# gdonninelli/Navier-Stokes_equations

Hardware: NVIDIA B200
Metric: time-steps/s (higher is better)
Workload: dtype f64 (fp16 operator copy inside the velocity preconditioner)

## Files before the change

navier-stokes_equations_b200/csrc/nsb200.cu:

```cuda
#include "../../include/nsb200.h"

#include <cuda_runtime.h>
#include <dlfcn.h>
#include <nccl.h>

#include <algorithm>
#include <cmath>
#include <cstdlib>
#include <cstring>
#include <map>
#include <memory>
#include <string>
#include <vector>

#include "amg.hpp"
#include "small_eig.hpp"
#include "assemble.cuh"
#include "device.cuh"
#include "linalg.cuh"
#include "structure.hpp"
#include "twolevel.cuh"
#include "velstream.cuh"

using namespace nsb;

namespace {

struct CudaErr {
  std::string msg;
};
#define CK(call)                                                                                   \
  do {                                                                                             \
    cudaError_t e_ = (call);                                                                       \
    if (e_ != cudaSuccess)                                                                         \
      throw CudaErr{std::string(#call) + " failed: " + cudaGetErrorString(e_) + " (" __FILE__ ":" + \
                    std::to_string(__LINE__) + ")"};                                               \
  } while (0)
#define CKN(call)                                                                        \
  do {                                                                                   \
    ncclResult_t r_ = (call);                                                            \
    if (r_ != ncclSuccess)                                                               \
      throw CudaErr{std::string(#call) + " failed: " + g_nccl.GetErrorString(r_)};       \
  } while (0)

struct NcclApi {
  void* handle = nullptr;
  ncclResult_t (*GetUniqueId)(ncclUniqueId*) = nullptr;
  ncclResult_t (*CommInitRank)(ncclComm_t*, int, ncclUniqueId, int) = nullptr;
  ncclResult_t (*CommDestroy)(ncclComm_t) = nullptr;
  ncclResult_t (*AllReduce)(const void*, void*, size_t, ncclDataType_t, ncclRedOp_t, ncclComm_t, cudaStream_t) = nullptr;
  ncclResult_t (*AllGather)(const void*, void*, size_t, ncclDataType_t, ncclComm_t, cudaStream_t) = nullptr;
  ncclResult_t (*Send)(const void*, size_t, ncclDataType_t, int, ncclComm_t, cudaStream_t) = nullptr;
  ncclResult_t (*Recv)(void*, size_t, ncclDataType_t, int, ncclComm_t, cudaStream_t) = nullptr;
  ncclResult_t (*GroupStart)() = nullptr;
  ncclResult_t (*GroupEnd)() = nullptr;
  const char* (*GetErrorString)(ncclResult_t) = nullptr;
  bool load(std::string& err) {
    if (handle) return true;
    for (const char* name : {"libnccl.so.2", "libnccl.so"}) {
      handle = dlopen(name, RTLD_NOW | RTLD_GLOBAL);
      if (handle) break;
    }
    if (!handle) { err = std::string("cannot load NCCL: ") + dlerror(); return false; }
    auto sym = [&](const char* n) { void* p = dlsym(handle, n); if (!p) err = std::string("NCCL symbol missing: ") + n; return p; };
    GetUniqueId = (decltype(GetUniqueId))sym("ncclGetUniqueId");
    CommInitRank = (decltype(CommInitRank))sym("ncclCommInitRank");
    CommDestroy = (decltype(CommDestroy))sym("ncclCommDestroy");
    AllReduce = (decltype(AllReduce))sym("ncclAllReduce");
    AllGather = (decltype(AllGather))sym("ncclAllGather");
    Send = (decltype(Send))sym("ncclSend");
    Recv = (decltype(Recv))sym("ncclRecv");
    GroupStart = (decltype(GroupStart))sym("ncclGroupStart");
    GroupEnd = (decltype(GroupEnd))sym("ncclGroupEnd");
    GetErrorString = (decltype(GetErrorString))sym("ncclGetErrorString");
    return GetUniqueId && CommInitRank && CommDestroy && AllReduce && AllGather && Send && Recv && GroupStart && GroupEnd && GetErrorString;
  }
};
NcclApi g_nccl;

template <typename T> struct DBuf {
  T* p = nullptr;
  size_t n = 0;
  bool owned = true;
  DBuf() = default;
  DBuf(const DBuf&) = delete;
  DBuf& operator=(const DBuf&) = delete;
  ~DBuf() { if (p && owned) cudaFree(p); }
  void alloc(size_t count) {
    if (p && owned) cudaFree(p);
    p = nullptr; owned = true;
    n = count;
    if (count) CK(cudaMalloc(&p, count * sizeof(T)));
  }
  void view(T* ptr, size_t count) {
    if (p && owned) cudaFree(p);
    p = ptr; n = count; owned = false;
  }
  void zero(cudaStream_t s) { if (n) CK(cudaMemsetAsync(p, 0, n * sizeof(T), s)); }
  void upload(const std::vector<T>& v, cudaStream_t s) {
    alloc(v.size());
    if (n) CK(cudaMemcpyAsync(p, v.data(), n * sizeof(T), cudaMemcpyHostToDevice, s));
  }
};

enum ProfCat { PC_ASM_CTX = 0, PC_ASM_ROWS, PC_SPMV, PC_SPMV_VEL, PC_SCHUR, PC_AMG, PC_ORTH, PC_OTHER, PC_ASM_PACK, PC_COARSE, PC_ASM_COARSE, PC_N };
const char* kProfNames[PC_N] = {"asm_context", "asm_rows", "spmv", "spmv_vel", "schur", "amg", "orth", "other", "asm_pack", "coarse", "asm_coarse"};

struct Prof {
  bool on = false;
  std::vector<cudaEvent_t> pool;
  size_t used = 0;
  struct Rec { int cat; size_t e0, e1; };
  std::vector<Rec> recs;
  double ms[PC_N] = {0};
  int64_t cnt[PC_N] = {0};
  cudaEvent_t get() {
    if (used == pool.size()) { cudaEvent_t e; cudaEventCreate(&e); pool.push_back(e); }
    return pool[used++];
  }
  size_t begin(int cat, cudaStream_t s) {
    if (!on) return 0;
    Rec r{cat, used, 0};
    cudaEventRecord(get(), s);
    recs.push_back(r);
    return recs.size() - 1;
  }
  void end(size_t id, cudaStream_t s) {
    if (!on) return;
    recs[id].e1 = used;
    cudaEventRecord(get(), s);
  }
  void collect(cudaStream_t s) {
    if (recs.empty()) return;
    cudaStreamSynchronize(s);
    for (auto& r : recs) {
      float t = 0;
      cudaEventElapsedTime(&t, pool[r.e0], pool[r.e1]);
      ms[r.cat] += t;
      cnt[r.cat]++;
    }
    recs.clear();
    used = 0;
  }
  void reset() { for (int i = 0; i < PC_N; ++i) { ms[i] = 0; cnt[i] = 0; } recs.clear(); used = 0; }
  ~Prof() { for (auto e : pool) cudaEventDestroy(e); }
};

struct DevLevel {
  DevCsr A, P, R;
  DBuf<int> Aptr, Acol, Pptr, Pcol, Rptr, Rcol;
  DBuf<double> Aval, Pval, Rval, dinv;
  DBuf<double> x, x2, b, d, r;
  double lmax = 1.0;
  int n = 0;
};

struct HaloBuf {
  DBuf<double> u, p;
  DBuf<int> uoff, poff;
};

void upload_csr(const HostCsr& H, DBuf<int>& ptr, DBuf<int>& col, DBuf<double>& val, DevCsr& D, cudaStream_t s) {
  ptr.upload(H.ptr, s); col.upload(H.col, s); val.upload(H.val, s);
  D.n = H.n; D.m = H.m; D.ptr = ptr.p; D.col = col.p; D.val = val.p;
}

struct PeerHalo {
  bool on = false;
  DBuf<double> arena;
  size_t stride_f = 0, stride_c = 0, coarse_base = 0;
  int slots_f = 0, slots_c = 0;
  DBuf<unsigned long long> flags;
  DBuf<unsigned int> counter;
  std::vector<void*> opened;
  std::vector<double*> peer_arena;
  std::vector<unsigned long long*> peer_flags;
  DBuf<double*> d_peer_arena;
  DBuf<unsigned long long*> d_peer_flags;
  DBuf<int> d_peer_rank;
  DBuf<int> seg_ptr_f, src_f, seg_ptr_c, src_c;
  DBuf<long long> land_f, land_c;
  unsigned long long seq = 0;
  const double* last_vec = nullptr;
  int total_f_vel = 0, total_f_all = 0, total_c = 0;
  DBuf<int> send_ptr_f, send_ptr_c, list_f, list_c;
  DBuf<int2> send_dst_f, send_dst_c;
  int n_int_f = 0, n_int_c = 0;
  const double* fresh_vec = nullptr;
  unsigned long long fresh_seq = 0;
};

struct VsDev {
  const VsTile* tiles;
  const uint32_t* meta;
  const int* uniq_xoff;
  const unsigned char* vals;
  int n_tiles;
};

struct PolyLevel {
  bool coarse = false;
  int nn = 0;
  long long n = 0, n_tot = 0;
  const double* dinv = nullptr;
  const int64_t* gid = nullptr;
  double *z0 = nullptr, *z1 = nullptr, *zd = nullptr, *poly = nullptr, *pin = nullptr;
  DBuf<double> probe;
  bool probe_init = false;
  std::vector<double> wr, wi;
  double ritz_lo = 0, ritz_hi = 0, ritz_im = 0, ritz_top = 0, probe_res = 1.0;
  std::vector<std::pair<double, double>> roots;
};

struct Coarse {
  DBuf<VsTile> tiles;
  DBuf<uint32_t> meta;
  DBuf<int> uniq_xoff;
  DBuf<unsigned char> vals;
  int n_tiles = 0;
  int64_t total_nq = 0;
  DBuf<long long> nbr_ptr, vedge_ptr;
  DBuf<int> nbr_vxoff, vedge_xoff, ends_xoff, send_xoff;
  DBuf<double> cvals, dinv, rc, z0, z1, zd, poly, pin, send_buf;
  std::vector<int> h_tiles_int, h_tiles_bnd, h_tile_node_ptr;
  std::vector<int64_t> gid, h_nbr_ptr, h_nbr_gid;
  bool built = false, valid = false;
};

}

struct nsb_ctx {
  int dim = 0, device = 0;
  int rank = 0, nranks = 1;
  ncclComm_t comm = nullptr;
  cudaStream_t stream = nullptr;
  std::string err;
  bool have_mesh = false, have_matrix = false, have_pressure = false;
  int64_t launches = 0;
  Prof prof;
  cudaEvent_t t0 = nullptr, t1 = nullptr;

  int64_t n_vertices = 0, n_cells = 0, n_u = 0, n_p = 0;
  std::vector<double> coords;
  std::vector<uint32_t> cell_vertices;
  std::vector<int> g_cell_pid;
  Structure S;
  DevMesh M{};
  DBuf<int> d_cell_xoff, d_cell_poff, d_nbr_xoff, d_pnbr_xoff, d_selfrank, d_node_pid, d_pid_node, d_pselfrank, d_tile_ptr;
  DBuf<double> d_cell_geom;
  DBuf<uint16_t> d_rank_uu, d_rank_up;
  DBuf<long long> d_nbr_ptr, d_pnbr_ptr, d_rowbase, d_prowbase, d_n2c_ptr;
  DBuf<uint32_t> d_n2c;
  DBuf<NodeDesc> d_nd;
  DBuf<FeTables> d_fe;
  int num_sms = 148;
  int n_tiles = 0, tile_smem_bytes = 0;
  DBuf<int> d_stile_ptr, d_suniq_ptr, d_suniq_xoff, d_spuniq_ptr, d_spuniq_xoff;
  DBuf<unsigned short> d_nbr_loc, d_pnbr_loc;
  SpmvTiles stiles{};
  int n_stiles = 0;
  std::vector<int> g2x;
  DBuf<int> d_pid_gid;
  DBuf<int> d_own_gdof;
  DBuf<double> w_tg, w_gather;
  DBuf<double> v_old, v_oldold, v_cur, v_sol, v_rhs;
  DBuf<unsigned char> cflag;
  DBuf<double> cval;
  DBuf<int> c_idx;
  DBuf<double> c_val;
  int n_con = 0;
  nsb_params par{};
  nsb_solver_opts opt{};
  DBuf<double> vals, dinv, ctx, cell_rhs;
  DBuf<double> forcing[2];
  bool forcing_set[2] = {false, false};
  DBuf<unsigned char> vs_vals;
  DBuf<VsTile> d_vs_tiles;
  DBuf<uint32_t> d_vs_meta;
  int64_t vs_total_nq = 0;
  bool vs_valid = false;
  int ctx_stride = 0;
  HostCsr h_Mp, h_Kp;
  DevCsr Mp{};
  DBuf<int> Mp_ptr, Mp_col;
  DBuf<double> Mp_val, Mp_dinv;
  double Mp_lmax = 1.0;
  std::vector<std::unique_ptr<DevLevel>> amg;
  std::vector<std::unique_ptr<HaloBuf>> halo;
  int n_tiles_int = 0, n_tiles_bnd = 0;
  std::vector<int> h_tiles_int, h_tiles_bnd, h_tile_node_ptr;
  bool fused_halo = false;
  double* pin = nullptr;
  DBuf<double> coarse_inv;
  int coarse_n = 0;
  DBuf<double> w_z0, w_z1, w_d, w_t, w_y1, w_m0, w_m1, w_md, w_in, w_tmp, w_pin, w_poly, w_y0, w_u;
  Coarse cg;
  PeerHalo ph;
  PolyLevel lvF, lvC;
  bool two_level = false;
  bool cycle_disabled = false;
  DBuf<double> V;
  int V_cap = 0;
  DBuf<double> partial, d_h, d_nrm;
  int solves = 0;

  void launch_check() {
    ++launches;
#ifdef NSB_DEBUG_SYNC
    CK(cudaStreamSynchronize(stream));
#endif
    CK(cudaGetLastError());
  }
};

namespace {

int fail(nsb_ctx* c, const std::string& m, int code = -1) {
  if (c) c->err = m;
  return code;
}

#define NSB_TRY try {
#define NSB_CATCH(c)                                               \
  }                                                                \
  catch (const CudaErr& e) { return fail(c, e.msg); }              \
  catch (const std::exception& e) { return fail(c, e.what()); }

inline int nblk(long long n, int t) { return (int)((n + t - 1) / t); }

#ifndef NSB_DEFAULT_PRECOND_PRECISION
#define NSB_DEFAULT_PRECOND_PRECISION 16
#endif

size_t vs_vals_bytes(const nsb_ctx* c) {
  if (c->opt.precond_precision == 64) return 0;
  return (size_t)c->vs_total_nq * 4 * c->dim * c->dim * (c->opt.precond_precision == 16 ? 2 : 4);
}

void peer_wait(nsb_ctx* c) {
  PeerHalo& H = c->ph;
  const int np = (int)c->S.peer.size();
  if (np == 0) return;
  k_halo_wait<<<1, 32, 0, c->stream>>>(np, H.d_peer_rank.p, H.flags.p, H.seq);
  c->launch_check();
}

void peer_exchange(nsb_ctx* c, const double* v, int nseg, const DBuf<int>& seg_ptr, const DBuf<int>& src, const DBuf<long long>& land,
                   int total_entries, bool wait = true) {
  PeerHalo& H = c->ph;
  const int np = (int)c->S.peer.size();
  if (np == 0) return;
  const long long vec_off = v - H.arena.p;
  if (vec_off < 0 || (size_t)vec_off >= H.arena.n) throw CudaErr{"halo exchange of a vector outside the symmetric arena"};
  if (v == H.last_vec) {
    k_halo_ack<<<1, 32, 0, c->stream>>>(np, H.d_peer_flags.p, c->nranks, c->rank, H.seq);
    c->launch_check();
    k_halo_wait<<<1, 32, 0, c->stream>>>(np, H.d_peer_rank.p, H.flags.p + c->nranks, H.seq);
    c->launch_check();
  }
  H.last_vec = v;
  H.fresh_vec = nullptr;
  ++H.seq;
  const int grid = std::max(1, std::min(nblk(total_entries, 256), 64));
  k_halo_push<<<grid, 256, 0, c->stream>>>(nseg, np, seg_ptr.p, src.p, land.p, H.d_peer_arena.p, vec_off, v, H.d_peer_flags.p, c->rank,
                                            H.seq, H.counter.p);
  c->launch_check();
  if (wait) peer_wait(c);
}

void halo_exchange(nsb_ctx* c, double* v, bool with_pressure = true) {
  if (c->nranks == 1) return;
  const Structure& S = c->S;
  if (c->ph.on) {
    const int np = (int)S.peer.size();
    const int nseg = with_pressure ? 2 * np : np;
    peer_exchange(c, v, nseg, c->ph.seg_ptr_f, c->ph.src_f, c->ph.land_f, with_pressure ? c->ph.total_f_all : c->ph.total_f_vel);
    return;
  }
  auto& B = c->halo;
  if (B.empty()) {
    auto b = std::make_unique<HaloBuf>();
    std::vector<int> uo, po;
    for (size_t k = 0; k < S.peer.size(); ++k) {
      for (int n : S.send_nodes[k]) uo.push_back((int)S.node_xoff(n));
      for (int q : S.send_pids[k]) po.push_back((int)S.pid_xoff(q));
    }
    b->uoff.upload(uo, c->stream); b->poff.upload(po, c->stream);
    CK(cudaStreamSynchronize(c->stream));
    b->u.alloc(uo.size() * S.dim); b->p.alloc(po.size());
    B.push_back(std::move(b));
  }
  HaloBuf& H = *B[0];
  const long long tu = (long long)H.uoff.n, tp = (long long)H.poff.n;
  if (tu) { k_gather_nodes<<<nblk(tu * S.dim, 256), 256, 0, c->stream>>>((int)tu, S.dim, H.uoff.p, v, H.u.p); c->launch_check(); }
  if (with_pressure && tp) { k_gather<<<nblk(tp, 256), 256, 0, c->stream>>>((int)tp, H.poff.p, v, H.p.p); c->launch_check(); }
  CKN(g_nccl.GroupStart());
  long long uoff = S.n_own_dofs(), poff = S.n_own_dofs() + (long long)S.dim * S.nn_ghost;
  size_t su = 0, sp = 0;
  for (size_t k = 0; k < S.peer.size(); ++k) {
    const int peer = S.peer[k];
    const size_t nu = S.send_nodes[k].size() * S.dim, np = S.send_pids[k].size();
    if (nu) CKN(g_nccl.Send(H.u.p + su, nu, ncclDouble, peer, c->comm, c->stream));
    if (with_pressure && np) CKN(g_nccl.Send(H.p.p + sp, np, ncclDouble, peer, c->comm, c->stream));
    const size_t ru = (size_t)S.recv_node_count[k] * S.dim, rp = (size_t)S.recv_pid_count[k];
    if (ru) CKN(g_nccl.Recv(v + uoff, ru, ncclDouble, peer, c->comm, c->stream));
    if (with_pressure && rp) CKN(g_nccl.Recv(v + poff, rp, ncclDouble, peer, c->comm, c->stream));
    uoff += ru; poff += rp;
    su += nu; sp += np;
  }
  CKN(g_nccl.GroupEnd());
}

void allreduce_sum(nsb_ctx* c, double* dbuf, int n) {
  if (c->nranks == 1) return;
  CKN(g_nccl.AllReduce(dbuf, dbuf, n, ncclDouble, ncclSum, c->comm, c->stream));
}

template <int DIM> void launch_coarse_assemble(nsb_ctx* c);

template <int DIM> void launch_assemble(nsb_ctx* c, bool newton) {
  AsmParams P;
  P.dt = c->par.dt; P.inv_dt = 1.0 / c->par.dt; P.theta = c->par.theta; P.nu = c->par.nu; P.rho = c->par.rho;
  P.use_supg = c->par.use_supg;
  P.gamma = c->par.use_supg ? c->par.gamma : 0.0;
  P.first_order_ustar = c->par.first_order_ustar;
  const int stride = newton ? Ctx<DIM>::N_NEWTON : CtxL<DIM>::N;
  if ((int)c->ctx_stride < stride) {
    c->ctx.alloc((size_t)c->S.nc * stride);
    c->ctx_stride = stride;
  }
  const double* vecA = newton ? c->v_cur.p : c->v_old.p;
  const double* vecB = newton ? c->v_old.p : c->v_oldold.p;
  size_t id = c->prof.begin(PC_ASM_CTX, c->stream);
  const int cgrid = std::min(nblk(c->S.nc, ASM_WARPS), c->num_sms * 8);
  const double *fn = c->forcing[NSB_FORCING_NEW].p, *fo = c->forcing[NSB_FORCING_OLD].p;
  const bool forced = fn != nullptr;
  if (newton && forced)
    k_cell_context<DIM, true, true><<<cgrid, ASM_WARPS * 32, 0, c->stream>>>(c->M, P, c->d_fe.p, vecA, vecB, c->ctx.p, c->cell_rhs.p, fn, fo);
  else if (newton)
    k_cell_context<DIM, true, false><<<cgrid, ASM_WARPS * 32, 0, c->stream>>>(c->M, P, c->d_fe.p, vecA, vecB, c->ctx.p, c->cell_rhs.p, nullptr, nullptr);
  else if (forced)
    k_cell_context<DIM, false, true><<<cgrid, ASM_WARPS * 32, 0, c->stream>>>(c->M, P, c->d_fe.p, vecA, vecB, c->ctx.p, c->cell_rhs.p, fn, fo);
  else
    k_cell_context<DIM, false, false><<<cgrid, ASM_WARPS * 32, 0, c->stream>>>(c->M, P, c->d_fe.p, vecA, vecB, c->ctx.p, c->cell_rhs.p, nullptr, nullptr);
  c->launch_check();
  c->prof.end(id, c->stream);
  RowOut out{c->vals.p, c->v_rhs.p, c->dinv.p};
  id = c->prof.begin(PC_ASM_ROWS, c->stream);
  if (newton)
    k_node_rows<DIM, true><<<c->n_tiles, ASM_WARPS * 32, c->tile_smem_bytes, c->stream>>>(c->M, P, c->ctx.p, c->cell_rhs.p, c->cflag.p, c->cval.p, out, c->d_tile_ptr.p, c->d_fe.p);
  else
    k_node_rows<DIM, false><<<c->n_tiles, ASM_WARPS * 32, c->tile_smem_bytes, c->stream>>>(c->M, P, c->ctx.p, c->cell_rhs.p, c->cflag.p, c->cval.p, out, c->d_tile_ptr.p, c->d_fe.p);
  c->launch_check();
  c->prof.end(id, c->stream);
  c->vs_valid = false;
  if (c->vs_vals.p) {
    id = c->prof.begin(PC_ASM_PACK, c->stream);
    if (c->opt.precond_precision == 16)
      k_vel_pack<DIM, __half><<<c->n_stiles, 256, 0, c->stream>>>(c->M, c->d_vs_tiles.p, c->d_vs_meta.p, c->vals.p, c->dinv.p, reinterpret_cast<__half*>(c->vs_vals.p));
    else
      k_vel_pack<DIM, float><<<c->n_stiles, 256, 0, c->stream>>>(c->M, c->d_vs_tiles.p, c->d_vs_meta.p, c->vals.p, c->dinv.p, reinterpret_cast<float*>(c->vs_vals.p));
    c->launch_check();
    c->prof.end(id, c->stream);
    c->vs_valid = true;
  }
  c->cg.valid = false;
  if (!newton && c->vs_valid && c->cg.built && c->opt.velocity_cycle != 1) launch_coarse_assemble<DIM>(c);
}

template <int DIM> void set_smem_attr(int bytes) {
  CK(cudaFuncSetAttribute(k_node_rows<DIM, false>, cudaFuncAttributeMaxDynamicSharedMemorySize, bytes));
  CK(cudaFuncSetAttribute(k_node_rows<DIM, true>, cudaFuncAttributeMaxDynamicSharedMemorySize, bytes));
}

template <int DIM, typename VT> void set_vs_attr() {
  const int bytes = VsLayout<DIM, VT>::SMEM_BYTES;
  CK(cudaFuncSetAttribute(k_vel_stream<DIM, VT, 2, false>, cudaFuncAttributeMaxDynamicSharedMemorySize, bytes));
  CK(cudaFuncSetAttribute(k_vel_stream<DIM, VT, 3, false>, cudaFuncAttributeMaxDynamicSharedMemorySize, bytes));
  CK(cudaFuncSetAttribute(k_vel_stream<DIM, VT, 3, true>, cudaFuncAttributeMaxDynamicSharedMemorySize, bytes));
  CK(cudaFuncSetAttribute(k_vel_stream<DIM, VT, 4, false>, cudaFuncAttributeMaxDynamicSharedMemorySize, bytes));
  CK(cudaFuncSetAttribute(k_vel_stream<DIM, VT, 4, true>, cudaFuncAttributeMaxDynamicSharedMemorySize, bytes));
}

template <int DIM, typename VT, int MODE, bool HALO>
void launch_vel_stream(nsb_ctx* c, const VsDev& D, int ntiles, const int* list, const double* x, double* y, const double* u, double* poly,
                       PolyCoef pc, const VsHalo& hx) {
  if (ntiles <= 0) return;
  const int grid = std::min(ntiles, c->num_sms);
  k_vel_stream<DIM, VT, MODE, HALO><<<grid, VS_THREADS, VsLayout<DIM, VT>::SMEM_BYTES, c->stream>>>(
      D.tiles, ntiles, list, reinterpret_cast<const VT*>(D.vals), D.meta, D.uniq_xoff, x, y, u, poly, pc, hx);
  c->launch_check();
}
template <int MODE, bool HALO>
void vel_stream(nsb_ctx* c, const VsDev& D, int ntiles, const int* list, const double* x, double* y, const double* u, double* poly, PolyCoef pc,
                const VsHalo& hx = VsHalo{}) {
  const bool h = c->opt.precond_precision == 16;
  if (c->dim == 2) {
    if (h) launch_vel_stream<2, __half, MODE, HALO>(c, D, ntiles, list, x, y, u, poly, pc, hx);
    else launch_vel_stream<2, float, MODE, HALO>(c, D, ntiles, list, x, y, u, poly, pc, hx);
  } else {
    if (h) launch_vel_stream<3, __half, MODE, HALO>(c, D, ntiles, list, x, y, u, poly, pc, hx);
    else launch_vel_stream<3, float, MODE, HALO>(c, D, ntiles, list, x, y, u, poly, pc, hx);
  }
}
VsDev fine_dev(const nsb_ctx* c);

void spmv_full(nsb_ctx* c, const double* x, double* y) {
  size_t id = c->prof.begin(PC_SPMV, c->stream);
  if (c->dim == 2) k_spmv_full<2, double><<<c->n_stiles, SPMV_WARPS * 32, 0, c->stream>>>(c->M, c->stiles, c->vals.p, x, y);
  else k_spmv_full<3, double><<<c->n_stiles, SPMV_WARPS * 32, 0, c->stream>>>(c->M, c->stiles, c->vals.p, x, y);
  c->launch_check();
  c->prof.end(id, c->stream);
}

template <int MODE>
void spmv_vel(nsb_ctx* c, const double* x, double* y, const double* u, double* poly, PolyCoef pc) {
  size_t id = c->prof.begin(PC_SPMV_VEL, c->stream);
  const int g = c->n_stiles;
  if (c->vs_valid && MODE != 0) {
    vel_stream<MODE == 0 ? 2 : MODE, false>(c, fine_dev(c), g, nullptr, x, y, u, poly, pc);
  } else {
    if (c->dim == 2) k_spmv_vel<2, MODE, double><<<g, SPMV_WARPS * 32, 0, c->stream>>>(c->M, c->stiles, c->vals.p, x, y, u, poly, c->dinv.p, pc);
    else k_spmv_vel<3, MODE, double><<<g, SPMV_WARPS * 32, 0, c->stream>>>(c->M, c->stiles, c->vals.p, x, y, u, poly, c->dinv.p, pc);
    c->launch_check();
  }
  c->prof.end(id, c->stream);
}

template <int MODE>
void fused_apply(nsb_ctx* c, bool coarse, const VsDev& D, double* x, double* y, const double* u, double* poly, PolyCoef pc) {
  PeerHalo& H = c->ph;
  const int np = (int)c->S.peer.size();
  VsHalo hx{};
  hx.flags = H.flags.p; hx.peer_rank = H.d_peer_rank.p; hx.npeers = np;
  hx.n_int = coarse ? H.n_int_c : H.n_int_f;
  hx.ghost_start = coarse ? c->dim * c->S.np_own : (int)c->S.n_own_dofs();
  if (x == H.fresh_vec) hx.wait_seq = H.fresh_seq;
  else {
    if (coarse) peer_exchange(c, x, np, H.seg_ptr_c, H.src_c, H.land_c, H.total_c);
    else peer_exchange(c, x, np, H.seg_ptr_f, H.src_f, H.land_f, H.total_f_vel);
    hx.wait_seq = 0;
  }
  hx.send_ptr = coarse ? H.send_ptr_c.p : H.send_ptr_f.p;
  hx.send_dst = coarse ? H.send_dst_c.p : H.send_dst_f.p;
  hx.peer_arena = H.d_peer_arena.p;
  hx.y_off = y - H.arena.p;
  if (hx.y_off < 0 || (size_t)hx.y_off >= H.arena.n) throw CudaErr{"fused halo delivery into a vector outside the symmetric arena"};
  hx.peer_flags = H.d_peer_flags.p; hx.my_rank = c->rank;
  hx.push_seq = ++H.seq;
  hx.counter = H.counter.p;
  const int* list = coarse ? H.list_c.p : H.list_f.p;
  vel_stream<MODE, true>(c, D, D.n_tiles, list, x, y, u, poly, pc, hx);
  H.fresh_vec = y; H.fresh_seq = hx.push_seq;
  H.last_vec = nullptr;
}

void halo_spmv_vel3(nsb_ctx* c, double* x, double* y, const double* u, double* poly, PolyCoef pc) {
  if (c->nranks > 1 && c->ph.on && c->vs_valid && c->fused_halo) {
    size_t id = c->prof.begin(PC_SPMV_VEL, c->stream);
    fused_apply<3>(c, false, fine_dev(c), x, y, u, poly, pc);
    c->prof.end(id, c->stream);
    return;
  }
  halo_exchange(c, x, false);
  spmv_vel<3>(c, x, y, u, poly, pc);
}

void block_scale(nsb_ctx* c, const double* x, double* y) {
  if (c->dim == 2) k_block_scale<2><<<nblk(c->S.nn_own, 256), 256, 0, c->stream>>>(c->S.nn_own, c->dinv.p, x, y);
  else k_block_scale<3><<<nblk(c->S.nn_own, 256), 256, 0, c->stream>>>(c->S.nn_own, c->dinv.p, x, y);
  c->launch_check();
}

double device_norm2(nsb_ctx* c, const double* x, long long n) {
  const int nb = nblk(n, RED_CHUNK);
  k_norm2_partial<<<nb, RED_THREADS, 0, c->stream>>>(x, n, c->partial.p);
  c->launch_check();
  k_reduce_partials<<<1, RED_THREADS, 0, c->stream>>>(nb, c->partial.p, c->d_nrm.p, 0);
  c->launch_check();
  allreduce_sum(c, c->d_nrm.p, 1);
  double v = 0;
  CK(cudaMemcpyAsync(&v, c->d_nrm.p, sizeof(double), cudaMemcpyDeviceToHost, c->stream));
  CK(cudaStreamSynchronize(c->stream));
  return std::sqrt(v);
}

struct Cheb {
  double theta, delta, sigma, rho;
  Cheb(double lmax, double lmin) : theta(0.5 * (lmax + lmin)), delta(0.5 * (lmax - lmin)) {
    sigma = theta / delta;
    rho = 1.0 / sigma;
  }
  void next(double& c1, double& c2) {
    const double rho_new = 1.0 / (2.0 * sigma - rho);
    c1 = rho_new * rho;
    c2 = 2.0 * rho_new / delta;
    rho = rho_new;
  }
};


VsDev fine_dev(const nsb_ctx* c) {
  return VsDev{c->d_vs_tiles.p, c->d_vs_meta.p, c->d_suniq_xoff.p, c->vs_vals.p, c->n_stiles};
}
VsDev coarse_dev(const nsb_ctx* c) {
  return VsDev{c->cg.tiles.p, c->cg.meta.p, c->cg.uniq_xoff.p, c->cg.vals.p, c->cg.n_tiles};
}

void halo_exchange_coarse(nsb_ctx* c, double* v) {
  if (c->nranks == 1) return;
  const Structure& S = c->S;
  if (c->ph.on) {
    peer_exchange(c, v, (int)S.peer.size(), c->ph.seg_ptr_c, c->ph.src_c, c->ph.land_c, c->ph.total_c);
    return;
  }
  Coarse& G = c->cg;
  const int dim = c->dim;
  const long long tp = (long long)G.send_xoff.n;
  if (tp) { k_gather_nodes<<<nblk(tp * dim, 256), 256, 0, c->stream>>>((int)tp, dim, G.send_xoff.p, v, G.send_buf.p); c->launch_check(); }
  CKN(g_nccl.GroupStart());
  long long roff = (long long)dim * S.np_own;
  size_t so = 0;
  for (size_t k = 0; k < S.peer.size(); ++k) {
    const int peer = S.peer[k];
    const size_t ns = S.send_pids[k].size() * dim, nr = (size_t)S.recv_pid_count[k] * dim;
    if (ns) CKN(g_nccl.Send(G.send_buf.p + so, ns, ncclDouble, peer, c->comm, c->stream));
    if (nr) CKN(g_nccl.Recv(v + roff, nr, ncclDouble, peer, c->comm, c->stream));
    so += ns; roff += nr;
  }
  CKN(g_nccl.GroupEnd());
}

void level_halo(nsb_ctx* c, PolyLevel& lv, double* v) {
  if (lv.coarse) halo_exchange_coarse(c, v);
  else halo_exchange(c, v, false);
}

template <int MODE>
void level_apply(nsb_ctx* c, PolyLevel& lv, const double* x, double* y, const double* u, double* poly, PolyCoef pc) {
  if (!lv.coarse) { spmv_vel<MODE>(c, x, y, u, poly, pc); return; }
  size_t id = c->prof.begin(PC_COARSE, c->stream);
  vel_stream<MODE, false>(c, coarse_dev(c), c->cg.n_tiles, nullptr, x, y, u, poly, pc);
  c->prof.end(id, c->stream);
}

void level_root(nsb_ctx* c, PolyLevel& lv, double* x, double* y, const double* u, double* poly, PolyCoef pc) {
  if (!lv.coarse) { halo_spmv_vel3(c, x, y, u, poly, pc); return; }
  if (c->nranks > 1 && c->ph.on && c->fused_halo) {
    size_t id = c->prof.begin(PC_COARSE, c->stream);
    fused_apply<3>(c, true, coarse_dev(c), x, y, u, poly, pc);
    c->prof.end(id, c->stream);
    return;
  }
  halo_exchange_coarse(c, x);
  level_apply<3>(c, lv, x, y, u, poly, pc);
}

void level_block_scale(nsb_ctx* c, PolyLevel& lv, const double* x, double* y) {
  if (c->dim == 2) k_block_scale<2><<<nblk(lv.nn, 256), 256, 0, c->stream>>>(lv.nn, lv.dinv, x, y);
  else k_block_scale<3><<<nblk(lv.nn, 256), 256, 0, c->stream>>>(lv.nn, lv.dinv, x, y);
  c->launch_check();
}

void level_arnoldi(nsb_ctx* c, PolyLevel& lv, int dmax, double target) {
  const long long nl = lv.n;
  const long long ld = c->S.n_own_dofs();
  int d = std::max(1, std::min(dmax, 64));
  if (c->V_cap < d + 1) { c->V.alloc((size_t)(std::max(d + 1, c->V_cap)) * ld); c->V_cap = std::max(d + 1, c->V_cap); }
  const int nb = nblk(nl, RED_CHUNK);
  if (c->partial.n < (size_t)nb * (d + 2)) c->partial.alloc((size_t)nb * (d + 2));
  if (c->d_h.n < (size_t)2 * (d + 2)) c->d_h.alloc(2 * (d + 2));
  if (!lv.probe_init) {
    std::vector<double> h(nl);
    for (int A = 0; A < lv.nn; ++A)
      for (int k = 0; k < c->dim; ++k) {
        uint64_t z = (uint64_t)(lv.gid[A] * c->dim + k) + 0x9E3779B97F4A7C15ull;
        z = (z ^ (z >> 30)) * 0xBF58476D1CE4E5B9ull;
        z = (z ^ (z >> 27)) * 0x94D049BB133111EBull;
        z ^= z >> 31;
        h[(size_t)c->dim * A + k] = (double)(z >> 11) / 9007199254740992.0 - 0.5;
      }
    lv.probe.upload(h, c->stream);
    CK(cudaStreamSynchronize(c->stream));
    lv.probe_init = true;
  }
  const int ldh = d;
  std::vector<double> H((size_t)(d + 1) * d, 0.0), hh(2 * (d + 2)), gcs(d + 1), gsn(d + 1);
  double gres = 1.0;
  double beta = device_norm2(c, lv.probe.p, nl);
  k_axpby<<<nblk(nl, 256), 256, 0, c->stream>>>(nl, 1.0 / beta, lv.probe.p, 0.0, c->V.p);
  c->launch_check();
  int dd = d;
  for (int k = 0; k < d; ++k) {
    double* vk = c->V.p + (size_t)k * ld;
    double* w = c->V.p + (size_t)(k + 1) * ld;
    const double* xin = vk;
    if (c->nranks > 1) {
      double* buf = (k & 1) ? lv.z1 : lv.pin;
      CK(cudaMemcpyAsync(buf, vk, nl * sizeof(double), cudaMemcpyDeviceToDevice, c->stream));
      level_halo(c, lv, buf);
      xin = buf;
    }
    level_apply<2>(c, lv, xin, w, nullptr, nullptr, PolyCoef{});
    for (int pass = 0; pass < 2; ++pass) {
      k_multi_dot<<<nb, RED_THREADS, 0, c->stream>>>(k + 1, c->V.p, ld, w, nl, c->partial.p);
      c->launch_check();
      double* hp = c->d_h.p + pass * (d + 2);
      k_reduce_partials<<<k + 1, RED_THREADS, 0, c->stream>>>(nb, c->partial.p, hp, 0);
      c->launch_check();
      allreduce_sum(c, hp, k + 1);
      k_multi_axpy<<<nb, RED_THREADS, 0, c->stream>>>(k + 1, c->V.p, ld, hp, -1.0, w, nl, pass == 1 ? c->partial.p : nullptr);
      c->launch_check();
    }
    k_reduce_partials<<<1, RED_THREADS, 0, c->stream>>>(nb, c->partial.p, c->d_nrm.p, 0);
    c->launch_check();
    allreduce_sum(c, c->d_nrm.p, 1);
    k_scale_by_inv_norm<<<nblk(nl, 256), 256, 0, c->stream>>>(nl, w, c->d_nrm.p, w);
    c->launch_check();
    double nrm2 = 0;
    CK(cudaMemcpyAsync(hh.data(), c->d_h.p, sizeof(double) * 2 * (d + 2), cudaMemcpyDeviceToHost, c->stream));
    CK(cudaMemcpyAsync(&nrm2, c->d_nrm.p, sizeof(double), cudaMemcpyDeviceToHost, c->stream));
    CK(cudaStreamSynchronize(c->stream));
    for (int i = 0; i <= k; ++i) H[(size_t)i * ldh + k] = hh[i] + hh[(d + 2) + i];
    H[(size_t)(k + 1) * ldh + k] = std::sqrt(nrm2);
    if (!(nrm2 > 1e-28)) { dd = k + 1; break; }
    {
      std::vector<double> col(k + 2);
      for (int i = 0; i <= k + 1; ++i) col[i] = H[(size_t)i * ldh + k];
      for (int i = 0; i < k; ++i) {
        const double t = gcs[i] * col[i] + gsn[i] * col[i + 1];
        col[i + 1] = -gsn[i] * col[i] + gcs[i] * col[i + 1];
        col[i] = t;
      }
      const double r = std::hypot(col[k], col[k + 1]);
      gcs[k] = col[k] / r; gsn[k] = col[k + 1] / r;
      gres *= std::fabs(gsn[k]);
      if (target > 0 && gres <= target && k + 1 >= 2) { dd = k + 1; break; }
    }
  }
  lv.probe_res = gres;
  d = dd;
  std::vector<double> Hd((size_t)d * d), At((size_t)d * d), f(d, 0.0);
  for (int i = 0; i < d; ++i)
    for (int j = 0; j < d; ++j) { Hd[(size_t)i * d + j] = H[(size_t)i * ldh + j]; At[(size_t)j * d + i] = H[(size_t)i * ldh + j]; }
  f[d - 1] = 1.0;
  {
    for (int col = 0; col < d; ++col) {
      int p = col;
      for (int r = col + 1; r < d; ++r) if (std::fabs(At[(size_t)r * d + col]) > std::fabs(At[(size_t)p * d + col])) p = r;
      if (p != col) { for (int k = 0; k < d; ++k) std::swap(At[(size_t)col * d + k], At[(size_t)p * d + k]); std::swap(f[col], f[p]); }
      const double dg = At[(size_t)col * d + col];
      for (int r = col + 1; r < d; ++r) {
        const double m = At[(size_t)r * d + col] / dg;
        if (m == 0.0) continue;
        for (int k = col; k < d; ++k) At[(size_t)r * d + k] -= m * At[(size_t)col * d + k];
        f[r] -= m * f[col];
      }
    }
    for (int r = d - 1; r >= 0; --r) {
      double sum = f[r];
      for (int k = r + 1; k < d; ++k) sum -= At[(size_t)r * d + k] * f[k];
      f[r] = sum / At[(size_t)r * d + r];
    }
  }
  const double hl = H[(size_t)d * ldh + (d - 1)];
  for (int i = 0; i < d; ++i) Hd[(size_t)i * d + (d - 1)] += hl * hl * f[i];
  std::vector<double> H0((size_t)d * d), sr, si;
  for (int i = 0; i < d; ++i)
    for (int j = 0; j < d; ++j) H0[(size_t)i * d + j] = H[(size_t)i * ldh + j];
  if (!hessenberg_eigs(d, Hd, lv.wr, lv.wi)) throw CudaErr{"harmonic Ritz eigenvalue iteration did not converge"};
  if (!hessenberg_eigs(d, H0, sr, si)) throw CudaErr{"Ritz eigenvalue iteration did not converge"};
  lv.ritz_lo = 1e300; lv.ritz_hi = -1e300; lv.ritz_im = 0; lv.ritz_top = -1e300;
  for (int i = 0; i < d; ++i) {
    lv.ritz_lo = std::min(lv.ritz_lo, lv.wr[i]); lv.ritz_hi = std::max(lv.ritz_hi, lv.wr[i]);
    lv.ritz_im = std::max(lv.ritz_im, std::fabs(lv.wi[i]));
    lv.ritz_top = std::max(lv.ritz_top, std::hypot(sr[i], si[i]));
  }
  lv.ritz_top = std::max(lv.ritz_top, lv.ritz_hi);
}

bool level_spectrum_is_real(const PolyLevel& lv, double tol = 0.05) { return lv.ritz_lo > 0 && lv.ritz_im < tol * lv.ritz_hi; }

void set_roots(PolyLevel& lv, std::vector<double> wr, std::vector<double> wi) {
  const int d = (int)wr.size();
  std::vector<std::pair<double, double>> th, out;
  for (int i = 0; i < d; ++i) if (wi[i] >= 0) th.emplace_back(wr[i], wi[i]);
  auto mag = [](const std::pair<double, double>& z) { return std::hypot(z.first, z.second); };
  while (!th.empty()) {
    size_t best = 0;
    double bv = -1e300;
    for (size_t i = 0; i < th.size(); ++i) {
      double v;
      if (out.empty()) v = mag(th[i]);
      else {
        v = 0;
        for (auto& o : out) {
          v += std::log(std::hypot(th[i].first - o.first, th[i].second - o.second) + 1e-300);
          if (o.second != 0) v += std::log(std::hypot(th[i].first - o.first, th[i].second + o.second) + 1e-300);
        }
      }
      if (v > bv) { bv = v; best = i; }
    }
    out.push_back(th[best]);
    th.erase(th.begin() + best);
  }
  lv.roots = out;
}
void set_chebyshev_roots(PolyLevel& lv, int d, double lo, double hi) {
  std::vector<double> wr(d), wi(d, 0.0);
  for (int j = 1; j <= d; ++j) wr[j - 1] = 0.5 * (hi + lo) + 0.5 * (hi - lo) * std::cos(M_PI * (2 * j - 1) / (2.0 * d));
  set_roots(lv, wr, wi);
}

void apply_poly(nsb_ctx* c, PolyLevel& lv) {
  double* prod = lv.z0;
  double* other = lv.z1;
  double* tmp = lv.zd;
  double* poly = lv.poly;
  CK(cudaMemsetAsync(poly, 0, lv.n * sizeof(double), c->stream));
  const auto& R = lv.roots;
  for (size_t k = 0; k < R.size(); ++k) {
    const bool last = (k + 1 == R.size());
    const double a = R[k].first, b = R[k].second;
    if (b == 0.0) {
      if (last) {
        k_axpby<<<nblk(lv.n, 256), 256, 0, c->stream>>>(lv.n, 1.0 / a, prod, 1.0, poly);
        c->launch_check();
      } else {
        level_root(c, lv, prod, other, prod, poly, PolyCoef{1.0, -1.0 / a, 1.0 / a, 0.0});
        std::swap(prod, other);
      }
    } else {
      const double m2 = a * a + b * b;
      level_root(c, lv, prod, tmp, prod, poly, PolyCoef{2.0 * a, -1.0, 0.0, 1.0 / m2});
      if (!last) {
        level_root(c, lv, tmp, other, prod, poly, PolyCoef{1.0, -1.0 / m2, 0.0, 0.0});
        std::swap(prod, other);
      }
    }
  }
}

template <int DIM> void launch_coarse_assemble(nsb_ctx* c) {
  Coarse& G = c->cg;
  FeTables T;
  fill_tables(DIM, T);
  double wsum = 0;
  for (int q = 0; q < T.nq; ++q) wsum += T.w[q];
  const double gamma = c->par.use_supg ? c->par.gamma : 0.0;
  size_t id = c->prof.begin(PC_ASM_COARSE, c->stream);
  k_coarse_rows<DIM><<<nblk(c->S.np_own, CG_WARPS), CG_WARPS * 32, 0, c->stream>>>(c->M, c->ctx.p, gamma, wsum, G.nbr_ptr.p, G.nbr_vxoff.p,
                                                                                     c->cflag.p, G.cvals.p, G.dinv.p);
  c->launch_check();
  if (c->opt.precond_precision == 16)
    k_coarse_pack<DIM, __half><<<G.n_tiles, 256, 0, c->stream>>>(G.tiles.p, G.meta.p, G.nbr_ptr.p, G.cvals.p, G.dinv.p, reinterpret_cast<__half*>(G.vals.p));
  else
    k_coarse_pack<DIM, float><<<G.n_tiles, 256, 0, c->stream>>>(G.tiles.p, G.meta.p, G.nbr_ptr.p, G.cvals.p, G.dinv.p, reinterpret_cast<float*>(G.vals.p));
  c->launch_check();
  c->prof.end(id, c->stream);
  G.valid = true;
}

void setup_velocity_pc(nsb_ctx* c) {
  PolyLevel& F = c->lvF;
  bool two = c->opt.velocity_cycle != 1 && c->cg.valid && c->vs_valid && !c->cycle_disabled;
  if (two) {
    level_arnoldi(c, F, 24, 0.0);
    two = level_spectrum_is_real(F, 0.02);
  }
  c->two_level = two;
  if (!two) {
    level_arnoldi(c, F, c->opt.poly_degree_F, c->opt.poly_target);
    if (c->opt.poly_kind == 1 && level_spectrum_is_real(F)) set_chebyshev_roots(F, (int)F.wr.size(), 0.9 * F.ritz_lo, 1.05 * F.ritz_hi);
    else set_roots(F, F.wr, F.wi);
    return;
  }
  const double hi = c->opt.smoother_hi_factor * F.ritz_top;
  set_chebyshev_roots(F, std::max(1, c->opt.smoother_degree), c->opt.smoother_lo_frac * hi, hi);
  PolyLevel& C = c->lvC;
  level_arnoldi(c, C, std::max(4, std::min(64, c->opt.coarse_degree + 5)), 0.05);
  if (level_spectrum_is_real(C)) set_chebyshev_roots(C, std::max(1, c->opt.coarse_degree), 0.9 * C.ritz_lo, c->opt.smoother_hi_factor * C.ritz_top);
  else set_roots(C, C.wr, C.wi);
}

void apply_velocity_pc(nsb_ctx* c, const double* x) {
  PolyLevel& F = c->lvF;
  const long long nu = F.n;
  if (!c->two_level) {
    level_block_scale(c, F, x, F.z0);
    apply_poly(c, F);
    return;
  }
  PolyLevel& C = c->lvC;
  Coarse& G = c->cg;
  const double* xr = x;
  if (c->nranks > 1) {
    CK(cudaMemcpyAsync(c->w_u.p, x, nu * sizeof(double), cudaMemcpyDeviceToDevice, c->stream));
    halo_exchange(c, c->w_u.p, false);
    xr = c->w_u.p;
  }
  size_t id = c->prof.begin(PC_COARSE, c->stream);
  if (c->dim == 2) k_restrict<2><<<nblk(c->S.np_own, 128), 128, 0, c->stream>>>(c->S.np_own, c->M.pid_node, G.vedge_ptr.p, G.vedge_xoff.p, c->cflag.p, xr, G.rc.p);
  else k_restrict<3><<<nblk(c->S.np_own, 128), 128, 0, c->stream>>>(c->S.np_own, c->M.pid_node, G.vedge_ptr.p, G.vedge_xoff.p, c->cflag.p, xr, G.rc.p);
  c->launch_check();
  c->prof.end(id, c->stream);
  level_block_scale(c, C, G.rc.p, C.z0);
  apply_poly(c, C);
  halo_exchange_coarse(c, C.poly);
  double* y0 = c->w_y0.p;
  id = c->prof.begin(PC_COARSE, c->stream);
  if (c->dim == 2) k_prolong<2><<<nblk(nu, 256), 256, 0, c->stream>>>(c->S.nn_own, G.ends_xoff.p, c->cflag.p, C.poly, y0);
  else k_prolong<3><<<nblk(nu, 256), 256, 0, c->stream>>>(c->S.nn_own, G.ends_xoff.p, c->cflag.p, C.poly, y0);
  c->launch_check();
  c->prof.end(id, c->stream);
  level_block_scale(c, F, x, c->w_u.p);
  if (c->nranks > 1 && c->ph.on && c->fused_halo) {
    size_t idf = c->prof.begin(PC_SPMV_VEL, c->stream);
    fused_apply<4>(c, false, fine_dev(c), y0, F.z0, c->w_u.p, nullptr, PolyCoef{1.0, -1.0, 0.0, 0.0});
    c->prof.end(idf, c->stream);
  } else {
    halo_exchange(c, y0, false);
    level_apply<4>(c, F, y0, F.z0, c->w_u.p, nullptr, PolyCoef{1.0, -1.0, 0.0, 0.0});
  }
  apply_poly(c, F);
  k_axpby<<<nblk(nu, 256), 256, 0, c->stream>>>(nu, 1.0, y0, 1.0, F.poly);
  c->launch_check();
}

void csr_cheb(nsb_ctx* c, const DevCsr& A, const double* dinv, double lmax, double ratio, int degree,
              const double* b, double* x, double* x2, double* d, bool zero_guess, double** result) {
  Cheb ch(1.1 * lmax, 1.1 * lmax / ratio);
  double* cur = x;
  double* oth = x2;
  int k0 = 0;
  const int g8 = nblk((long long)A.n * 8, 256);
  if (zero_guess) {
    k_cheb_first<<<nblk(A.n, 256), 256, 0, c->stream>>>(A.n, dinv, b, d, cur, 1.0 / ch.theta);
    c->launch_check();
    k0 = 1;
  }
  for (int k = k0; k < degree; ++k) {
    double c1, c2;
    if (k == 0) { c1 = 0.0; c2 = 1.0 / ch.theta; }
    else ch.next(c1, c2);
    k_csr<3><<<g8, 256, 0, c->stream>>>(A, cur, oth, b, d, dinv, c1, c2);
    c->launch_check();
    std::swap(cur, oth);
  }
  *result = cur;
}

void amg_vcycle(nsb_ctx* c, int lev) {
  DevLevel& L = *c->amg[lev];
  const int deg = c->opt.amg_smoother_degree;
  if (lev + 1 == (int)c->amg.size()) {
    if (c->coarse_n > 0) {
      k_dense_mv<<<nblk((long long)L.n * 32, 256), 256, 0, c->stream>>>(L.n, c->coarse_inv.p, L.b.p, L.x.p);
      c->launch_check();
    } else {
      double* res;
      csr_cheb(c, L.A, L.dinv.p, L.lmax, 30.0, 12, L.b.p, L.x.p, L.x2.p, L.d.p, true, &res);
      if (res != L.x.p) std::swap(L.x.p, L.x2.p);
    }
    return;
  }
  double* res;
  csr_cheb(c, L.A, L.dinv.p, L.lmax, 20.0, deg, L.b.p, L.x.p, L.x2.p, L.d.p, true, &res);
  if (res != L.x.p) std::swap(L.x.p, L.x2.p);
  const int g8 = nblk((long long)L.n * 8, 256);
  k_csr<1><<<g8, 256, 0, c->stream>>>(L.A, L.x.p, L.r.p, L.b.p, nullptr, nullptr, 0, 0);
  c->launch_check();
  DevLevel& N = *c->amg[lev + 1];
  k_csr<0><<<nblk((long long)N.n * 8, 256), 256, 0, c->stream>>>(L.R, L.r.p, N.b.p, nullptr, nullptr, nullptr, 0, 0);
  c->launch_check();
  amg_vcycle(c, lev + 1);
  k_csr<2><<<g8, 256, 0, c->stream>>>(L.P, N.x.p, L.x.p, nullptr, nullptr, nullptr, 0, 0);
  c->launch_check();
  csr_cheb(c, L.A, L.dinv.p, L.lmax, 20.0, deg, L.b.p, L.x.p, L.x2.p, L.d.p, false, &res);
  if (res != L.x.p) std::swap(L.x.p, L.x2.p);
}

double schur_mass_coeff(const nsb_ctx* c) {
  const double cm = c->opt.schur_mass_coeff;
  return cm >= 0 ? cm : c->par.theta * c->par.nu + (c->par.use_supg ? c->par.gamma : 0.0);
}

void precond_apply(nsb_ctx* c, const double* x, double* y) {
  const Structure& S = c->S;
  const int dim = c->dim;
  const long long nu = (long long)dim * S.nn_own;
  apply_velocity_pc(c, x);
  double* z = c->w_poly.p;
  CK(cudaMemcpyAsync(y, z, nu * sizeof(double), cudaMemcpyDeviceToDevice, c->stream));
  halo_exchange(c, z);
  size_t id = c->prof.begin(PC_SCHUR, c->stream);
  if (dim == 2) k_schur_rhs<2, double><<<nblk(S.np_own, SPMV_WARPS), SPMV_WARPS * 32, 0, c->stream>>>(c->M, c->vals.p, z, x, c->w_t.p);
  else k_schur_rhs<3, double><<<nblk(S.np_own, SPMV_WARPS), SPMV_WARPS * 32, 0, c->stream>>>(c->M, c->vals.p, z, x, c->w_t.p);
  c->launch_check();
  c->prof.end(id, c->stream);
  const double* tg = c->w_t.p;
  if (c->nranks > 1) {
    CK(cudaMemsetAsync(c->w_tg.p, 0, (size_t)c->n_p * sizeof(double), c->stream));
    k_scatter_vals<<<nblk(S.np_own, 256), 256, 0, c->stream>>>(S.np_own, c->d_pid_gid.p, c->w_t.p, c->w_tg.p);
    c->launch_check();
    allreduce_sum(c, c->w_tg.p, (int)c->n_p);
    tg = c->w_tg.p;
  }
  id = c->prof.begin(PC_AMG, c->stream);
  DevLevel& L0 = *c->amg[0];
  CK(cudaMemcpyAsync(L0.b.p, tg, (size_t)L0.n * sizeof(double), cudaMemcpyDeviceToDevice, c->stream));
// ... 15 lines not shown
  const int m = std::max(1, n_tmp - 2);
  if (c->V_cap < m + 1) {
    c->V.alloc((size_t)(m + 1) * n);
    c->V_cap = m + 1;
  }
  const int nb = nblk(n, RED_CHUNK);
  if (c->partial.n < (size_t)nb * (m + 2)) c->partial.alloc((size_t)nb * (m + 2));
  if (c->d_h.n < (size_t)2 * (m + 2)) c->d_h.alloc(2 * (m + 2));
  double* x = c->v_sol.p;
  CK(cudaMemsetAsync(x, 0, S.n_tot_dofs() * sizeof(double), c->stream));
  std::vector<double> H((size_t)(m + 1) * m, 0.0), cs(m), sn(m), g(m + 1), hcol(2 * (m + 2));
  int it = 0;
  double res = 0;
  bool first = true;
  for (;;) {
    double* V0 = c->V.p;
    if (first) {
      precond_apply(c, c->v_rhs.p, c->w_in.p);
    } else {
      halo_exchange(c, x);
      spmv_full(c, x, c->w_tmp.p);
      k_lincomb<<<nblk(n, 256), 256, 0, c->stream>>>(n, 1.0, c->v_rhs.p, -1.0, c->w_tmp.p, c->w_tmp.p);
      c->launch_check();
      precond_apply(c, c->w_tmp.p, c->w_in.p);
    }
    const double beta = device_norm2(c, c->w_in.p, n);
    res = beta;
    if (first && beta <= tol_abs) { *iterations = 0; *residual = beta; return 0; }
    first = false;
    if (!(beta > 0)) { *iterations = it; *residual = beta; return 0; }
    k_axpby<<<nblk(n, 256), 256, 0, c->stream>>>(n, 1.0 / beta, c->w_in.p, 0.0, V0);
    c->launch_check();
    std::fill(g.begin(), g.end(), 0.0);
    g[0] = beta;
    int kused = 0;
    bool converged = false;
    for (int k = 0; k < m; ++k) {
      double* vk = c->V.p + (size_t)k * n;
      double* w = c->V.p + (size_t)(k + 1) * n;
      const double* xin = vk;
      if (c->nranks > 1) {
        CK(cudaMemcpyAsync(c->w_pin.p, vk, n * sizeof(double), cudaMemcpyDeviceToDevice, c->stream));
        halo_exchange(c, c->w_pin.p);
        xin = c->w_pin.p;
      }
      spmv_full(c, xin, c->w_tmp.p);
      precond_apply(c, c->w_tmp.p, w);
      size_t id = c->prof.begin(PC_ORTH, c->stream);
      const int mode = c->opt.reorthogonalize;
      int passes = 1;
      double nrm2 = 0, nrm2_before = 0;
      for (int pass = 0; pass < 2; ++pass) {
        const int nv = k + 1 + (pass == 0 ? 1 : 0);
        k_multi_dot<<<nb, RED_THREADS, 0, c->stream>>>(nv, c->V.p, n, w, n, c->partial.p);
        c->launch_check();
        double* hp = c->d_h.p + pass * (m + 2);
        k_reduce_partials<<<nv, RED_THREADS, 0, c->stream>>>(nb, c->partial.p, hp, 0);
        c->launch_check();
        allreduce_sum(c, hp, nv);
        k_multi_axpy<<<nb, RED_THREADS, 0, c->stream>>>(k + 1, c->V.p, n, hp, -1.0, w, n, c->partial.p);
        c->launch_check();
        k_reduce_partials<<<1, RED_THREADS, 0, c->stream>>>(nb, c->partial.p, c->d_nrm.p, 0);
        c->launch_check();
        allreduce_sum(c, c->d_nrm.p, 1);
        passes = pass + 1;
        if (pass == 1 || mode < 0) break;
        if (mode != 2) {
          CK(cudaMemcpyAsync(&nrm2_before, hp + k + 1, sizeof(double), cudaMemcpyDeviceToHost, c->stream));
          CK(cudaMemcpyAsync(&nrm2, c->d_nrm.p, sizeof(double), cudaMemcpyDeviceToHost, c->stream));
          CK(cudaStreamSynchronize(c->stream));
          if (nrm2 > 0.5 * nrm2_before) break;
        }
      }
      k_scale_by_inv_norm<<<nblk(n, 256), 256, 0, c->stream>>>(n, w, c->d_nrm.p, w);
      c->launch_check();
      c->prof.end(id, c->stream);
      CK(cudaMemcpyAsync(hcol.data(), c->d_h.p, sizeof(double) * 2 * (m + 2), cudaMemcpyDeviceToHost, c->stream));
      CK(cudaMemcpyAsync(&nrm2, c->d_nrm.p, sizeof(double), cudaMemcpyDeviceToHost, c->stream));
      CK(cudaStreamSynchronize(c->stream));
      for (int i = 0; i <= k; ++i) H[(size_t)i * m + k] = hcol[i] + (passes == 2 ? hcol[(m + 2) + i] : 0.0);
      H[(size_t)(k + 1) * m + k] = std::sqrt(nrm2);
      for (int i = 0; i < k; ++i) {
        const double t = cs[i] * H[(size_t)i * m + k] + sn[i] * H[(size_t)(i + 1) * m + k];
        H[(size_t)(i + 1) * m + k] = -sn[i] * H[(size_t)i * m + k] + cs[i] * H[(size_t)(i + 1) * m + k];
        H[(size_t)i * m + k] = t;
      }
      const double a = H[(size_t)k * m + k], b = H[(size_t)(k + 1) * m + k];
      const double dd = std::hypot(a, b);
      cs[k] = a / dd; sn[k] = b / dd;
      H[(size_t)k * m + k] = dd;
      H[(size_t)(k + 1) * m + k] = 0.0;
      g[k + 1] = -sn[k] * g[k];
      g[k] = cs[k] * g[k];
      res = std::fabs(g[k + 1]);
      ++it;
      kused = k + 1;
      if (res <= tol_abs) { converged = true; break; }
      if (it >= max_it) break;
      if (!(nrm2 > 0)) break;
    }
    std::vector<double> yv(kused);
    for (int i = kused - 1; i >= 0; --i) {
      double s = g[i];
      for (int j = i + 1; j < kused; ++j) s -= H[(size_t)i * m + j] * yv[j];
      yv[i] = s / H[(size_t)i * m + i];
    }
    CK(cudaMemcpyAsync(c->d_h.p, yv.data(), sizeof(double) * kused, cudaMemcpyHostToDevice, c->stream));
    k_multi_axpy<<<nb, RED_THREADS, 0, c->stream>>>(kused, c->V.p, n, c->d_h.p, 1.0, x, n, nullptr);
    c->launch_check();
    CK(cudaStreamSynchronize(c->stream));
    if (converged || it >= max_it) {
      *iterations = it;
      *residual = res;
      return converged ? 0 : 1;
    }
  }
}

void build_tiles(nsb_ctx* c) {
  const Structure& S = c->S;
  int dev_max = 0;
  CK(cudaDeviceGetAttribute(&dev_max, cudaDevAttrMaxSharedMemoryPerBlockOptin, c->device));
  const int stat = 24 * 1024;
  int budget = std::max(S.max_node_smem_doubles, 5 * 1024);
  if ((long long)budget * 8 + stat > dev_max)
    throw CudaErr{"a node's rows do not fit in shared memory (valence too high)"};
  std::vector<int> tp;
  tp.push_back(0);
  int sum = 0, cnt = 0;
  for (int A = 0; A < S.nn_own; ++A) {
    const int need = (S.dim + (S.node_pid[A] >= 0 ? 1 : 0)) * S.row_len(A);
    if (cnt > 0 && (sum + need > budget || cnt >= 64)) { tp.push_back(A); sum = 0; cnt = 0; }
    sum += need; ++cnt;
  }
  tp.push_back(S.nn_own);
  c->n_tiles = (int)tp.size() - 1;
  c->tile_smem_bytes = budget * 8;
  c->d_tile_ptr.upload(tp, c->stream);
  {
    TilePlan P;
    const TileLimits L{TILE_MAX_NODES, TILE_MAX_IDX, TILE_MAX_UNIQ, TILE_MAX_PUNIQ, VS_MAX_BLOCKS};
    const std::string err = build_tile_plan(S, L, P);
    if (!err.empty()) throw CudaErr{err};
    VsPlan V;
    const std::string err2 = build_vel_stream(S, P, V);
    if (!err2.empty()) throw CudaErr{err2};
    c->n_stiles = P.n_tiles();
    c->d_stile_ptr.upload(P.node_ptr, c->stream);
    c->n_tiles_int = (int)P.tiles_int.size(); c->n_tiles_bnd = (int)P.tiles_bnd.size();
    c->h_tiles_int = P.tiles_int; c->h_tiles_bnd = P.tiles_bnd; c->h_tile_node_ptr = P.node_ptr;
    c->d_suniq_ptr.upload(P.uniq_ptr, c->stream); c->d_suniq_xoff.upload(P.uniq_xoff, c->stream);
    c->d_spuniq_ptr.upload(P.puniq_ptr, c->stream); c->d_spuniq_xoff.upload(P.puniq_xoff, c->stream);
    c->d_nbr_loc.upload(P.nbr_loc, c->stream); c->d_pnbr_loc.upload(P.pnbr_loc, c->stream);
    c->d_vs_tiles.upload(V.tiles, c->stream); c->d_vs_meta.upload(V.meta, c->stream);
    c->vs_total_nq = V.total_nq;
    CK(cudaStreamSynchronize(c->stream));
    c->stiles.node_ptr = c->d_stile_ptr.p;
    c->stiles.uniq_ptr = c->d_suniq_ptr.p; c->stiles.uniq_xoff = c->d_suniq_xoff.p;
    c->stiles.puniq_ptr = c->d_spuniq_ptr.p; c->stiles.puniq_xoff = c->d_spuniq_xoff.p;
    c->stiles.nbr_loc = c->d_nbr_loc.p; c->stiles.pnbr_loc = c->d_pnbr_loc.p;
  }
  c->vs_vals.alloc(vs_vals_bytes(c));
  c->vs_valid = false;
  CK(cudaStreamSynchronize(c->stream));
  if (c->dim == 2) { set_smem_attr<2>(c->tile_smem_bytes); set_vs_attr<2, float>(); set_vs_attr<2, __half>(); }
  else { set_smem_attr<3>(c->tile_smem_bytes); set_vs_attr<3, float>(); set_vs_attr<3, __half>(); }
}

void close_peer_halo(nsb_ctx* c) {
  PeerHalo& H = c->ph;
  for (void* q : H.opened) cudaIpcCloseMemHandle(q);
  H.opened.clear(); H.peer_arena.clear(); H.peer_flags.clear();
  H.on = false;
}

void nccl_barrier(nsb_ctx* c) {
  if (c->nranks == 1 || !c->comm) return;
  CKN(g_nccl.AllReduce(c->d_nrm.p + 2, c->d_nrm.p + 2, 1, ncclDouble, ncclSum, c->comm, c->stream));
  CK(cudaStreamSynchronize(c->stream));
}

void setup_peer_halo(nsb_ctx* c, std::vector<DBuf<double>*> fine, std::vector<DBuf<double>*> coarse, size_t nt, size_t nct) {
  PeerHalo& H = c->ph;
  const Structure& S = c->S;
  const int R = c->nranks, dim = c->dim, np = (int)S.peer.size();
  cudaStream_t st = c->stream;
  close_peer_halo(c);
  nccl_barrier(c);
  long long hs[2] = {(long long)nt, (long long)nct};
  DBuf<long long> ds;
  ds.alloc(2);
  CK(cudaMemcpyAsync(ds.p, hs, sizeof(hs), cudaMemcpyHostToDevice, st));
  CKN(g_nccl.AllReduce(ds.p, ds.p, 2, ncclInt64, ncclMax, c->comm, st));
  CK(cudaMemcpyAsync(hs, ds.p, sizeof(hs), cudaMemcpyDeviceToHost, st));
  CK(cudaStreamSynchronize(st));
  H.stride_f = ((size_t)hs[0] + 31) / 32 * 32;
  H.stride_c = ((size_t)hs[1] + 31) / 32 * 32;
  H.slots_f = (int)fine.size(); H.slots_c = (int)coarse.size();
  H.coarse_base = H.stride_f * H.slots_f;
  H.arena.alloc(H.coarse_base + H.stride_c * H.slots_c);
  H.arena.zero(st);
  for (size_t i = 0; i < fine.size(); ++i) fine[i]->view(H.arena.p + i * H.stride_f, nt);
  for (size_t i = 0; i < coarse.size(); ++i) coarse[i]->view(H.arena.p + H.coarse_base + i * H.stride_c, nct);
  H.flags.alloc(2 * (size_t)R); H.flags.zero(st);
  H.counter.alloc(1); H.counter.zero(st);
  H.seq = 0; H.last_vec = nullptr;
  const char* mode = std::getenv("NSB200_HALO");
  const bool want = !(mode && std::string(mode) == "nccl");
  std::vector<long long> mine((size_t)R * 3, -1), all((size_t)R * R * 3, -1);
  {
    long long uoff = S.n_own_dofs(), poff = S.n_own_dofs() + (long long)dim * S.nn_ghost, coff = (long long)dim * S.np_own;
    for (int k = 0; k < np; ++k) {
      mine[(size_t)S.peer[k] * 3 + 0] = uoff; mine[(size_t)S.peer[k] * 3 + 1] = poff; mine[(size_t)S.peer[k] * 3 + 2] = coff;
      uoff += (long long)S.recv_node_count[k] * dim; poff += S.recv_pid_count[k]; coff += (long long)S.recv_pid_count[k] * dim;
    }
  }
  struct Handles { cudaIpcMemHandle_t arena, flags; };
  Handles hm;
  std::vector<Handles> hall(R);
  bool ok = want;
  if (ok) ok = cudaIpcGetMemHandle(&hm.arena, H.arena.p) == cudaSuccess && cudaIpcGetMemHandle(&hm.flags, H.flags.p) == cudaSuccess;
  if (!ok) { std::memset(&hm, 0, sizeof(hm)); cudaGetLastError(); }
  {
    DBuf<unsigned char> g0, g1;
    DBuf<long long> t0, t1;
    g0.alloc(sizeof(Handles) + 8); g1.alloc((sizeof(Handles) + 8) * R);
    t0.alloc(mine.size()); t1.alloc(all.size());
    unsigned char pack[sizeof(Handles) + 8] = {0};
    std::memcpy(pack, &hm, sizeof(hm));
    pack[sizeof(Handles)] = ok ? 1 : 0;
    CK(cudaMemcpyAsync(g0.p, pack, sizeof(pack), cudaMemcpyHostToDevice, st));
    CK(cudaMemcpyAsync(t0.p, mine.data(), mine.size() * sizeof(long long), cudaMemcpyHostToDevice, st));
    CKN(g_nccl.AllGather(g0.p, g1.p, sizeof(pack), ncclChar, c->comm, st));
    CKN(g_nccl.AllGather(t0.p, t1.p, mine.size(), ncclInt64, c->comm, st));
    std::vector<unsigned char> back((sizeof(Handles) + 8) * R);
    CK(cudaMemcpyAsync(back.data(), g1.p, back.size(), cudaMemcpyDeviceToHost, st));
    CK(cudaMemcpyAsync(all.data(), t1.p, all.size() * sizeof(long long), cudaMemcpyDeviceToHost, st));
    CK(cudaStreamSynchronize(st));
    for (int r = 0; r < R; ++r) {
      std::memcpy(&hall[r], back.data() + (sizeof(Handles) + 8) * r, sizeof(Handles));
      ok = ok && back[(sizeof(Handles) + 8) * r + sizeof(Handles)] == 1;
    }
  }
  if (ok) {
    for (int k = 0; k < np && ok; ++k) {
      void *pa = nullptr, *pf = nullptr;
      ok = cudaIpcOpenMemHandle(&pa, hall[S.peer[k]].arena, cudaIpcMemLazyEnablePeerAccess) == cudaSuccess;
      if (ok) { H.opened.push_back(pa); ok = cudaIpcOpenMemHandle(&pf, hall[S.peer[k]].flags, cudaIpcMemLazyEnablePeerAccess) == cudaSuccess; }
      if (ok) H.opened.push_back(pf);
      H.peer_arena.push_back((double*)pa); H.peer_flags.push_back((unsigned long long*)pf);
    }
    if (!ok) cudaGetLastError();
  }
  {
    DBuf<long long> d;
    d.alloc(1);
    long long v = ok ? 1 : 0;
    CK(cudaMemcpyAsync(d.p, &v, sizeof(v), cudaMemcpyHostToDevice, st));
    CKN(g_nccl.AllReduce(d.p, d.p, 1, ncclInt64, ncclMin, c->comm, st));
    CK(cudaMemcpyAsync(&v, d.p, sizeof(v), cudaMemcpyDeviceToHost, st));
    CK(cudaStreamSynchronize(st));
    ok = v == 1;
  }
  if (!ok) {
    if (want && c->rank == 0) std::fprintf(stderr, "nsb200: peer-store halo unavailable (CUDA IPC), using NCCL send/recv\n");
    close_peer_halo(c);
    return;
  }
  std::vector<int> sp(1, 0), src, spc(1, 0), srcc, pr(np);
  std::vector<long long> land(2 * (size_t)np), landc(np);
  for (int k = 0; k < np; ++k) {
    pr[k] = S.peer[k];
    for (int n : S.send_nodes[k]) for (int cc = 0; cc < dim; ++cc) src.push_back((int)S.node_xoff(n) + cc);
    sp.push_back((int)src.size());
    land[k] = all[((size_t)S.peer[k] * R + c->rank) * 3 + 0];
  }
  H.total_f_vel = (int)src.size();
  for (int k = 0; k < np; ++k) {
    for (int q : S.send_pids[k]) src.push_back((int)S.pid_xoff(q));
    sp.push_back((int)src.size());
    land[np + k] = all[((size_t)S.peer[k] * R + c->rank) * 3 + 1];
    for (int q : S.send_pids[k]) for (int cc = 0; cc < dim; ++cc) srcc.push_back(dim * q + cc);
    spc.push_back((int)srcc.size());
    landc[k] = all[((size_t)S.peer[k] * R + c->rank) * 3 + 2];
  }
  H.total_f_all = (int)src.size(); H.total_c = (int)srcc.size();
  for (int k = 0; k < np; ++k)
    if (land[k] < 0 || land[np + k] < 0 || landc[k] < 0) throw CudaErr{"halo plan mismatch: a peer does not expect data from this rank"};
  H.seg_ptr_f.upload(sp, st); H.src_f.upload(src, st); H.land_f.upload(land, st);
  H.seg_ptr_c.upload(spc, st); H.src_c.upload(srcc, st); H.land_c.upload(landc, st);
  H.d_peer_arena.upload(H.peer_arena, st); H.d_peer_flags.upload(H.peer_flags, st); H.d_peer_rank.upload(pr, st);
  auto fused_tables = [&](int n_own, const std::vector<std::vector<int>>& send, const std::vector<long long>& landing, const std::vector<int>& ,
                          const std::vector<int>& t_bnd, const std::vector<int>& node_ptr, DBuf<int>& d_ptr, DBuf<int2>& d_dst, DBuf<int>& d_list,
                          int& n_int) {
    std::vector<int> cnt(n_own + 1, 0);
    for (int k = 0; k < np; ++k) for (int n : send[k]) cnt[n + 1]++;
    for (int n = 0; n < n_own; ++n) cnt[n + 1] += cnt[n];
    std::vector<int2> dst(cnt[n_own]);
    std::vector<int> fill(cnt.begin(), cnt.end() - 1);
    for (int k = 0; k < np; ++k)
      for (size_t i = 0; i < send[k].size(); ++i) dst[fill[send[k][i]]++] = make_int2(k, (int)(landing[k] + (long long)i * dim));
    std::vector<char> back(node_ptr.size() - 1, 0);
    for (int t : t_bnd) back[t] = 1;
    for (size_t t = 0; t + 1 < node_ptr.size(); ++t)
      for (int n = node_ptr[t]; n < node_ptr[t + 1] && !back[t]; ++n)
        if (cnt[n + 1] != cnt[n]) back[t] = 1;
    std::vector<int> list;
    for (size_t t = 0; t + 1 < node_ptr.size(); ++t) if (!back[t]) list.push_back((int)t);
    n_int = (int)list.size();
    for (size_t t = 0; t + 1 < node_ptr.size(); ++t) if (back[t]) list.push_back((int)t);
    for (auto& d : dst) if (d.y < 0) throw CudaErr{"halo plan: negative landing offset"};
    d_ptr.upload(cnt, st); d_dst.upload(dst, st); d_list.upload(list, st);
    CK(cudaStreamSynchronize(st));
  };
  {
    std::vector<long long> lf(land.begin(), land.begin() + np);
    fused_tables(S.nn_own, S.send_nodes, lf, c->h_tiles_int, c->h_tiles_bnd, c->h_tile_node_ptr, H.send_ptr_f, H.send_dst_f, H.list_f, H.n_int_f);
    fused_tables(S.np_own, S.send_pids, landc, c->cg.h_tiles_int, c->cg.h_tiles_bnd, c->cg.h_tile_node_ptr, H.send_ptr_c, H.send_dst_c, H.list_c, H.n_int_c);
  }
  H.fresh_vec = nullptr; H.fresh_seq = 0;
  CK(cudaStreamSynchronize(st));
  nccl_barrier(c);
  H.on = true;
}

void build_coarse_level(nsb_ctx* c) {
  const Structure& S = c->S;
  Coarse& G = c->cg;
  G.built = false; G.valid = false;
  CoarseLevel CL;
  const std::string e = build_coarse(S, CL);
  if (!e.empty()) throw CudaErr{e};
  const Structure& Sc = CL.Sc;
  for (int P = 0; P < S.np_own; ++P)
    if (Sc.nbr_ptr[P + 1] - Sc.nbr_ptr[P] > CG_MAX_NB) throw CudaErr{"a vertex has more P1 neighbours than the coarse row kernel can accumulate"};
  TilePlan P;
  const TileLimits L{TILE_MAX_NODES, TILE_MAX_IDX, TILE_MAX_UNIQ, TILE_MAX_PUNIQ, VS_MAX_BLOCKS};
  const std::string e1 = build_tile_plan(Sc, L, P);
  if (!e1.empty()) throw CudaErr{e1};
  VsPlan V;
  const std::string e2 = build_vel_stream(Sc, P, V);
  if (!e2.empty()) throw CudaErr{e2};
  cudaStream_t st = c->stream;
  const int dim = c->dim;
  G.n_tiles = P.n_tiles();
  G.total_nq = V.total_nq;
  G.h_tiles_int = P.tiles_int; G.h_tiles_bnd = P.tiles_bnd; G.h_tile_node_ptr = P.node_ptr;
  G.tiles.upload(V.tiles, st); G.meta.upload(V.meta, st); G.uniq_xoff.upload(P.uniq_xoff, st);
  std::vector<long long> t64(Sc.nbr_ptr.begin(), Sc.nbr_ptr.end()), v64(CL.vedge_ptr.begin(), CL.vedge_ptr.end());
  G.nbr_ptr.upload(t64, st); G.vedge_ptr.upload(v64, st);
  std::vector<int> vx(Sc.nbr.size()), ex(CL.vedge.size()), en(CL.node_ends.size()), sx;
  for (size_t i = 0; i < vx.size(); ++i) vx[i] = (int)S.node_xoff(S.pid_node[Sc.nbr[i]]);
  for (size_t i = 0; i < ex.size(); ++i) ex[i] = (int)S.node_xoff(CL.vedge[i]);
  for (size_t i = 0; i < en.size(); ++i) en[i] = (int)Sc.node_xoff(CL.node_ends[i]);
  for (size_t k = 0; k < S.peer.size(); ++k)
    for (int q : S.send_pids[k]) sx.push_back((int)Sc.node_xoff(q));
  G.nbr_vxoff.upload(vx, st); G.vedge_xoff.upload(ex, st); G.ends_xoff.upload(en, st); G.send_xoff.upload(sx, st);
  G.send_buf.alloc(sx.size() * dim);
  G.gid.assign(S.pid_gid.begin(), S.pid_gid.begin() + S.np_own);
  G.h_nbr_ptr.assign(Sc.nbr_ptr.begin(), Sc.nbr_ptr.end());
  G.h_nbr_gid.resize(Sc.nbr.size());
  for (size_t i = 0; i < Sc.nbr.size(); ++i) G.h_nbr_gid[i] = S.pid_gid[Sc.nbr[i]];
  CK(cudaStreamSynchronize(st));
  const size_t nct = (size_t)Sc.n_tot_dofs();
  G.cvals.alloc(Sc.nbr.size() * dim * dim);
  G.dinv.alloc((size_t)S.np_own * dim * dim);
  if (c->nranks == 1) {
    for (DBuf<double>* v : {&G.rc, &G.z0, &G.z1, &G.zd, &G.poly, &G.pin}) { v->alloc(nct); v->zero(st); }
  } else {
    setup_peer_halo(c, {&c->v_old, &c->v_oldold, &c->v_cur, &c->v_sol, &c->v_rhs, &c->cval, &c->w_z0, &c->w_z1, &c->w_d, &c->w_in, &c->w_tmp,
                        &c->w_pin, &c->w_poly, &c->w_y0, &c->w_u},
                    {&G.rc, &G.z0, &G.z1, &G.zd, &G.poly, &G.pin}, (size_t)S.n_tot_dofs(), nct);
  }
  CK(cudaStreamSynchronize(st));
  PolyLevel& C = c->lvC;
  C.coarse = true; C.nn = S.np_own; C.n = (long long)dim * S.np_own; C.n_tot = (long long)nct;
  C.dinv = G.dinv.p; C.gid = G.gid.data();
  C.z0 = G.z0.p; C.z1 = G.z1.p; C.zd = G.zd.p; C.poly = G.poly.p; C.pin = G.pin.p;
  C.probe_init = false; C.roots.clear();
  G.built = true;
}

size_t coarse_vals_bytes(const nsb_ctx* c) {
  if (c->opt.precond_precision == 64) return 0;
  return (size_t)c->cg.total_nq * 4 * c->dim * c->dim * (c->opt.precond_precision == 16 ? 2 : 4);
}

void bind_fine_level(nsb_ctx* c) {
  PolyLevel& F = c->lvF;
  F.coarse = false; F.nn = c->S.nn_own; F.n = (long long)c->dim * c->S.nn_own; F.n_tot = c->S.n_tot_dofs();
  F.dinv = c->dinv.p; F.gid = c->S.node_gid.data();
  F.z0 = c->w_z0.p; F.z1 = c->w_z1.p; F.zd = c->w_d.p; F.poly = c->w_poly.p; F.pin = c->w_pin.p;
}

void host_pressure_matrices(nsb_ctx* c, const std::vector<unsigned char>& pflag) {
  const int dim = c->dim, NV = dim + 1;
  const int64_t np = c->n_p, C = c->n_cells;
  FeTables T;
  fill_tables(dim, T);
  double wsum = 0;
  for (int q = 0; q < T.nq; ++q) wsum += T.w[q];
  std::vector<std::vector<int>> adj(np);
  for (int64_t cc = 0; cc < C; ++cc)
    for (int i = 0; i < NV; ++i)
      for (int j = 0; j < NV; ++j) adj[c->g_cell_pid[cc * NV + i]].push_back(c->g_cell_pid[cc * NV + j]);
  HostCsr Mp, Kp;
  Mp.n = Mp.m = (int)np;
  Mp.ptr.assign(np + 1, 0);
  for (int64_t i = 0; i < np; ++i) {
    auto& a = adj[i];
    std::sort(a.begin(), a.end());
    a.erase(std::unique(a.begin(), a.end()), a.end());
    Mp.ptr[i + 1] = Mp.ptr[i] + (int)a.size();
  }
  Mp.col.resize(Mp.ptr[np]);
  for (int64_t i = 0; i < np; ++i) std::copy(adj[i].begin(), adj[i].end(), Mp.col.begin() + Mp.ptr[i]);
  Mp.val.assign(Mp.col.size(), 0.0);
  Kp = Mp;
  auto find = [&](int r, int col) {
    const int* b = Mp.col.data() + Mp.ptr[r];
    const int* e = Mp.col.data() + Mp.ptr[r + 1];
    return (int)(std::lower_bound(b, e, col) - Mp.col.data());
  };
  for (int64_t cc = 0; cc < C; ++cc) {
    const uint32_t* cv = c->cell_vertices.data() + cc * NV;
    double X[4][3] = {{0}};
    for (int v = 0; v < NV; ++v)
      for (int k = 0; k < dim; ++k) X[v][k] = c->coords[(size_t)cv[v] * dim + k];
    double gl[4][3] = {{0}}, det;
    if (dim == 2) {
      const double a = X[1][0] - X[0][0], b = X[2][0] - X[0][0], cq = X[1][1] - X[0][1], d = X[2][1] - X[0][1];
      det = a * d - b * cq;
      gl[1][0] = d / det; gl[1][1] = -b / det; gl[2][0] = -cq / det; gl[2][1] = a / det;
      for (int k = 0; k < 2; ++k) gl[0][k] = -(gl[1][k] + gl[2][k]);
    } else {
      double J[3][3];
      for (int r = 0; r < 3; ++r)
        for (int k = 0; k < 3; ++k) J[r][k] = X[k + 1][r] - X[0][r];
      const double c00 = J[1][1] * J[2][2] - J[1][2] * J[2][1], c01 = J[1][2] * J[2][0] - J[1][0] * J[2][2],
                   c02 = J[1][0] * J[2][1] - J[1][1] * J[2][0];
      det = J[0][0] * c00 + J[0][1] * c01 + J[0][2] * c02;
      const double id = 1.0 / det;
      gl[1][0] = c00 * id; gl[1][1] = (J[0][2] * J[2][1] - J[0][1] * J[2][2]) * id; gl[1][2] = (J[0][1] * J[1][2] - J[0][2] * J[1][1]) * id;
      gl[2][0] = c01 * id; gl[2][1] = (J[0][0] * J[2][2] - J[0][2] * J[2][0]) * id; gl[2][2] = (J[0][2] * J[1][0] - J[0][0] * J[1][2]) * id;
      gl[3][0] = c02 * id; gl[3][1] = (J[0][1] * J[2][0] - J[0][0] * J[2][1]) * id; gl[3][2] = (J[0][0] * J[1][1] - J[0][1] * J[1][0]) * id;
      for (int k = 0; k < 3; ++k) gl[0][k] = -((gl[1][k] + gl[2][k]) + gl[3][k]);
    }
    const double absJ = std::fabs(det);
    const int* pid = c->g_cell_pid.data() + cc * NV;
    for (int i = 0; i < NV; ++i) {
      const bool ci = pflag[pid[i]] != 0;
      for (int j = 0; j < NV; ++j) {
        const bool cj = pflag[pid[j]] != 0;
        double gg = 0;
        for (int k = 0; k < dim; ++k) gg += gl[i][k] * gl[j][k];
        double m = absJ * T.MPhat[i][j], kk = absJ * wsum * gg;
        if (ci || cj) {
          if (i == j) { m = std::fabs(m); kk = std::fabs(kk); }
          else { m = 0; kk = 0; }
        }
        const int p = find(pid[i], pid[j]);
        Mp.val[p] += m;
        Kp.val[p] += kk;
      }
    }
  }
  for (size_t k = 0; k < Kp.val.size(); ++k) Kp.val[k] += 1e-6 * Mp.val[k];
  c->h_Mp = std::move(Mp);
  c->h_Kp = std::move(Kp);
}

double* vec_ptr(nsb_ctx* c, int which) {
  switch (which) {
    case NSB_SOLUTION_OLD: return c->v_old.p;
    case NSB_SOLUTION_OLD_OLD: return c->v_oldold.p;
    case NSB_CURRENT_SOLUTION: return c->v_cur.p;
    case NSB_SOLUTION: return c->v_sol.p;
    case NSB_RHS: return c->v_rhs.p;
  }
  return nullptr;
}

PolyLevel& level_of(nsb_ctx* c, int level) { return level == 0 ? c->lvF : c->lvC; }

void level_upload(nsb_ctx* c, int level, const double* g, double* d) {
  const Structure& S = c->S;
  const int dim = c->dim;
  const int nn = level == 0 ? S.nn_own + S.nn_ghost : S.np_own;
  std::vector<double> loc(level == 0 ? (size_t)S.n_tot_dofs() : (size_t)dim * nn, 0.0);
  for (int A = 0; A < nn; ++A) {
    const int64_t off = level == 0 ? S.node_xoff(A) : (int64_t)dim * A;
    const int64_t gid = level == 0 ? S.node_gid[A] : S.pid_gid[A];
    for (int k = 0; k < dim; ++k) loc[off + k] = g[gid * dim + k];
  }
  CK(cudaMemcpyAsync(d, loc.data(), loc.size() * sizeof(double), cudaMemcpyHostToDevice, c->stream));
  CK(cudaStreamSynchronize(c->stream));
}

void level_download(nsb_ctx* c, int level, const double* d, double* g) {
  const Structure& S = c->S;
  const int dim = c->dim;
  const int nn = level == 0 ? S.nn_own : S.np_own;
  std::vector<double> out((size_t)dim * nn);
  CK(cudaMemcpyAsync(out.data(), d, out.size() * sizeof(double), cudaMemcpyDeviceToHost, c->stream));
  CK(cudaStreamSynchronize(c->stream));
  for (int A = 0; A < nn; ++A) {
    const int64_t gid = level == 0 ? S.node_gid[A] : S.pid_gid[A];
    for (int k = 0; k < dim; ++k) g[gid * dim + k] = out[(size_t)dim * A + k];
  }
}

void velocity_operator_apply(nsb_ctx* c, int level, int mode, const double* coef, const double* xg, const double* ug, double* yg,
                             double* pg) {
  PolyLevel& lv = level_of(c, level);
  double* x = level == 0 ? c->w_pin.p : c->cg.pin.p;
  double* u = level == 0 ? c->w_u.p : c->cg.z0.p;
  double* y = level == 0 ? c->w_tmp.p : c->cg.z1.p;
  double* p = level == 0 ? c->w_poly.p : c->cg.poly.p;
  level_upload(c, level, xg, x);
  if (mode >= 3) level_upload(c, level, ug, u);
  if (mode == 3) level_upload(c, level, pg, p);
  const PolyCoef pc = coef ? PolyCoef{coef[0], coef[1], coef[2], coef[3]} : PolyCoef{};
  if (mode == 2) level_apply<2>(c, lv, x, y, nullptr, nullptr, pc);
  else if (mode == 3) level_apply<3>(c, lv, x, y, u, p, pc);
  else level_apply<4>(c, lv, x, y, u, nullptr, pc);
  level_download(c, level, y, yg);
  if (mode == 3) level_download(c, level, p, pg);
}

template <typename VT>
void unpack_level(nsb_ctx* c, const VsDev& D, int64_t total_nq, size_t n_uniq, std::vector<int>& node, std::vector<int>& nbr,
                  std::vector<double>& val) {
  const int dim = c->dim, PL = dim * dim;
  std::vector<VsTile> tiles(D.n_tiles);
  std::vector<uint32_t> meta((size_t)total_nq * 4);
  std::vector<int> uniq(n_uniq);
  std::vector<VT> v((size_t)total_nq * 4 * PL);
  CK(cudaMemcpyAsync(tiles.data(), D.tiles, tiles.size() * sizeof(VsTile), cudaMemcpyDeviceToHost, c->stream));
  CK(cudaMemcpyAsync(meta.data(), D.meta, meta.size() * sizeof(uint32_t), cudaMemcpyDeviceToHost, c->stream));
  CK(cudaMemcpyAsync(uniq.data(), D.uniq_xoff, uniq.size() * sizeof(int), cudaMemcpyDeviceToHost, c->stream));
  CK(cudaMemcpyAsync(v.data(), D.vals, v.size() * sizeof(VT), cudaMemcpyDeviceToHost, c->stream));
  CK(cudaStreamSynchronize(c->stream));
  for (const VsTile& T : tiles) {
    const uint32_t* m = meta.data() + (size_t)T.nq_off * 4;
    const VT* tv = v.data() + (size_t)T.nq_off * 4 * PL;
    for (int q = 0; q < T.nquad; ++q) {
      const uint32_t* mq = m + 4 * q;
      if (mq[2] == 0xffffu) continue;
      const int cnt = (int)(mq[3] >> 16);
      for (int e = 0; e < cnt; ++e) {
        const int loc = (int)(((e < 2 ? mq[0] : mq[1]) >> (16 * (e & 1))) & 0xffffu);
        node.push_back(T.n0 + (int)mq[2]);
        nbr.push_back(uniq[T.u0 + loc] / dim);
        for (int rc = 0; rc < PL; ++rc) val.push_back((double)(float)tv[((size_t)rc * T.NQ + q) * 4 + e]);
      }
    }
  }
}

}

extern "C" {

int nsb_create(int dim, int device, nsb_handle* out) {
  if (!out) return -1;
  *out = nullptr;
  if (dim != 2 && dim != 3) return -1;
  nsb_ctx* c = new nsb_ctx();
  c->dim = dim; c->device = device;
  *out = c;
  NSB_TRY
  int ndev = 0;
  CK(cudaGetDeviceCount(&ndev));
  if (device < 0 || device >= ndev) throw CudaErr{"no such CUDA device (the product path has no CPU fallback)"};
  CK(cudaSetDevice(device));
  cudaDeviceProp prop;
  CK(cudaGetDeviceProperties(&prop, device));
  if (prop.major < 10) throw CudaErr{"nsb200 is built for sm_100a (B200) only"};
  CK(cudaStreamCreateWithFlags(&c->stream, cudaStreamNonBlocking));
  CK(cudaEventCreate(&c->t0));
  CK(cudaEventCreate(&c->t1));
  FeTables T2, T3;
  fill_tables(2, T2);
  fill_tables(3, T3);
  {
    std::vector<FeTables> tv(1, dim == 2 ? T2 : T3);
    c->d_fe.upload(tv, c->stream);
    CK(cudaStreamSynchronize(c->stream));
  }
  CK(cudaDeviceGetAttribute(&c->num_sms, cudaDevAttrMultiProcessorCount, device));
  c->opt.poly_degree_F = 64; c->opt.poly_refresh = 1; c->opt.poly_target = 0.08; c->opt.poly_kind = 1; c->opt.cheb_degree_Mp = 3;
  c->opt.amg_smoother_degree = 2; c->opt.schur_mass_coeff = -1.0; c->opt.reorthogonalize = 1;
  c->opt.precond_precision = NSB_DEFAULT_PRECOND_PRECISION;
  c->opt.precond_operator = 1;
  c->opt.velocity_cycle = 2; c->opt.smoother_degree = 14; c->opt.smoother_lo_frac = 0.012; c->opt.coarse_degree = 15; c->opt.smoother_hi_factor = 1.1;
  c->par.dt = 0.01; c->par.theta = 1.0; c->par.nu = 1e-3; c->par.rho = 1.0; c->par.gamma = 0.1;
  c->d_nrm.alloc(4);
  return 0;
  NSB_CATCH(c)
}

int nsb_destroy(nsb_handle c) {
  if (!c) return 0;
  cudaSetDevice(c->device);
  if (c->stream) cudaStreamSynchronize(c->stream);
  if (c->ph.on) {
    try { close_peer_halo(c); nccl_barrier(c); } catch (...) {}
  }
  if (c->pin) cudaFreeHost(c->pin);
  if (c->comm) g_nccl.CommDestroy(c->comm);
  if (c->t0) cudaEventDestroy(c->t0);
  if (c->t1) cudaEventDestroy(c->t1);
  cudaStream_t s = c->stream;
  delete c;
  if (s) cudaStreamDestroy(s);
  return 0;
}

const char* nsb_last_error(nsb_handle c) { return c ? c->err.c_str() : "null handle"; }

int nsb_comm_unique_id(void* out128) {
  ncclUniqueId id;
  std::string err;
  if (!g_nccl.load(err)) { std::fprintf(stderr, "nsb200: %s\n", err.c_str()); return -1; }
  if (g_nccl.GetUniqueId(&id) != ncclSuccess) return -1;
  std::memcpy(out128, &id, sizeof(id));
  return 0;
}

int nsb_comm_init(nsb_handle c, int rank, int nranks, const void* uid) {
  if (!c) return -1;
  NSB_TRY
  CK(cudaSetDevice(c->device));
  if (c->have_mesh) throw CudaErr{"nsb_comm_init must precede nsb_upload_mesh"};
  if (nranks > 1) {
    std::string err;
    if (!g_nccl.load(err)) throw CudaErr{err};
    if (!uid) throw CudaErr{"nccl_unique_id is required with more than one rank"};
    ncclUniqueId id;
    std::memcpy(&id, uid, sizeof(id));
    CKN(g_nccl.CommInitRank(&c->comm, nranks, id, rank));
    const char* fh = std::getenv("NSB200_FUSED_HALO");
    c->fused_halo = fh && fh[0] == '1';
  }
  c->rank = rank; c->nranks = nranks;
  return 0;
  NSB_CATCH(c)
}

int nsb_upload_mesh(nsb_handle c, int64_t n_vertices, const double* coords, int64_t n_cells,
                    const uint32_t* cell_vertices, const uint32_t* cell_dofs, int64_t n_u, int64_t n_p,
                    const int32_t* cell_part) {
  if (!c) return -1;
  NSB_TRY
  CK(cudaSetDevice(c->device));
  for (auto& b : c->forcing) b.alloc(0);
  c->forcing_set[0] = c->forcing_set[1] = false;
  const int dim = c->dim, NV = dim + 1;
  std::string e = build_structure(dim, n_vertices, coords, n_cells, cell_vertices, cell_dofs, n_u, n_p,
                                  c->nranks > 1 ? cell_part : nullptr, c->rank, c->nranks, c->S);
  if (!e.empty()) return fail(c, e);
  if (c->nranks > 1 && !cell_part) return fail(c, "cell_part is required with more than one rank");
  Structure& S = c->S;
  c->n_vertices = n_vertices; c->n_cells = n_cells; c->n_u = n_u; c->n_p = n_p;
  c->coords.assign(coords, coords + n_vertices * dim);
  c->cell_vertices.assign(cell_vertices, cell_vertices + n_cells * NV);
  c->g_cell_pid.resize(n_cells * NV);
  const int DPC = S.DPC;
  for (int64_t cc = 0; cc < n_cells; ++cc)
    for (int v = 0; v < NV; ++v) c->g_cell_pid[cc * NV + v] = (int)(cell_dofs[cc * DPC + v * (dim + 1) + dim] - n_u);
  if (S.n_tot_dofs() >= (int64_t)INT32_MAX) return fail(c, "local vector too long for 32-bit offsets");
  c->g2x.assign(n_u + n_p, -1);
  for (int A = 0; A < S.nn_own + S.nn_ghost; ++A)
    for (int k = 0; k < dim; ++k) c->g2x[S.node_gid[A] * dim + k] = (int)S.node_xoff(A) + k;
  for (int P = 0; P < S.np_own + S.np_ghost; ++P) c->g2x[n_u + S.pid_gid[P]] = (int)S.pid_xoff(P);
  cudaStream_t st = c->stream;
  std::vector<int> cx(S.cell_nodes.size()), cp(S.cell_pids.size());
  for (size_t i = 0; i < cx.size(); ++i) cx[i] = (int)S.node_xoff(S.cell_nodes[i]);
  for (size_t i = 0; i < cp.size(); ++i) cp[i] = (int)S.pid_xoff(S.cell_pids[i]);
  c->d_cell_xoff.upload(cx, st); c->d_cell_poff.upload(cp, st);
  c->d_cell_geom.upload(S.cell_geom, st);
  c->d_rank_uu.upload(S.rank_uu, st); c->d_rank_up.upload(S.rank_up, st);
  std::vector<int> nx(S.nbr.size()), px(S.pnbr.size());
  for (size_t i = 0; i < nx.size(); ++i) nx[i] = (int)S.node_xoff(S.nbr[i]);
  for (size_t i = 0; i < px.size(); ++i) px[i] = (int)S.pid_xoff(S.pnbr[i]);
  c->d_nbr_xoff.upload(nx, st); c->d_pnbr_xoff.upload(px, st);
  std::vector<long long> t64;
  auto up64 = [&](const std::vector<int64_t>& v, DBuf<long long>& d) {
    t64.assign(v.begin(), v.end());
    d.upload(t64, st);
    CK(cudaStreamSynchronize(st));
  };
  up64(S.nbr_ptr, c->d_nbr_ptr); up64(S.pnbr_ptr, c->d_pnbr_ptr);
  up64(S.rowbase, c->d_rowbase); up64(S.prowbase, c->d_prowbase); up64(S.n2c_ptr, c->d_n2c_ptr);
  c->d_selfrank.upload(S.selfrank, st);
  std::vector<int> npid(S.node_pid.begin(), S.node_pid.begin() + S.nn_own);
  c->d_node_pid.upload(npid, st);
  std::vector<int> pnode(S.pid_node.begin(), S.pid_node.begin() + S.np_own);
  c->d_pid_node.upload(pnode, st);
  c->d_pselfrank.upload(S.pselfrank, st);
  c->d_n2c.upload(S.n2c, st);
  if (S.nbr.size() >= (size_t)INT32_MAX) return fail(c, "neighbour lists too long for 32-bit offsets");
  std::vector<NodeDesc> nd(S.nn_own);
  for (int A = 0; A < S.nn_own; ++A) {
    NodeDesc& d = nd[A];
    d.rowbase = S.rowbase[A];
// ... 552 lines not shown
  apply_velocity_pc(c, c->w_tmp.p);
  CK(cudaMemcpyAsync(yg, c->w_poly.p, nu * sizeof(double), cudaMemcpyDeviceToHost, c->stream));
  CK(cudaStreamSynchronize(c->stream));
  return 0;
  NSB_CATCH(c)
}

int nsb_apply_preconditioner(nsb_handle c, const double* xg, double* yg) {
  if (int rc = pc_entry_check(c, "nsb_apply_preconditioner")) return rc;
  NSB_TRY
  CK(cudaSetDevice(c->device));
  const size_t n = (size_t)c->S.n_own_dofs();
  CK(cudaMemcpyAsync(c->w_tmp.p, xg, n * sizeof(double), cudaMemcpyHostToDevice, c->stream));
  precond_apply(c, c->w_tmp.p, c->w_in.p);
  CK(cudaMemcpyAsync(yg, c->w_in.p, n * sizeof(double), cudaMemcpyDeviceToHost, c->stream));
  CK(cudaStreamSynchronize(c->stream));
  return 0;
  NSB_CATCH(c)
}

int nsb_pressure_pc_info(nsb_handle c, double* mp_lambda_max, double* mass_coeff) {
  if (!c || !c->have_pressure) return fail(c, "pressure matrices not assembled");
  if (mp_lambda_max) *mp_lambda_max = c->Mp_lmax;
  if (mass_coeff) *mass_coeff = schur_mass_coeff(c);
  return 0;
}

int nsb_timer_start(nsb_handle c) {
  if (!c) return -1;
  cudaSetDevice(c->device);
  return cudaEventRecord(c->t0, c->stream) == cudaSuccess ? 0 : -1;
}
int nsb_timer_stop(nsb_handle c, double* ms) {
  if (!c) return -1;
  cudaSetDevice(c->device);
  cudaEventRecord(c->t1, c->stream);
  cudaEventSynchronize(c->t1);
  float t = 0;
  cudaEventElapsedTime(&t, c->t0, c->t1);
  if (ms) *ms = t;
  return 0;
}
int nsb_synchronize(nsb_handle c) {
  if (!c) return -1;
  cudaSetDevice(c->device);
  return cudaStreamSynchronize(c->stream) == cudaSuccess ? 0 : fail(c, "stream synchronize failed");
}
int nsb_profile_enable(nsb_handle c, int on) {
  if (!c) return -1;
  c->prof.collect(c->stream);
  c->prof.on = on != 0;
  return 0;
}
int nsb_profile_reset(nsb_handle c) {
  if (!c) return -1;
  c->prof.collect(c->stream);
  c->prof.reset();
  return 0;
}
int nsb_profile_get(nsb_handle c, const char* name, double* total_ms, int64_t* launches) {
  if (!c) return -1;
  c->prof.collect(c->stream);
  for (int i = 0; i < PC_N; ++i)
    if (std::strcmp(name, kProfNames[i]) == 0) {
      if (total_ms) *total_ms = c->prof.ms[i];
      if (launches) *launches = c->prof.cnt[i];
      return 0;
    }
  return fail(c, "unknown profile class");
}
int nsb_test_build_pattern(int dim, int64_t n_vertices, const double* coords, int64_t n_cells,
                           const uint32_t* cell_vertices, const uint32_t* cell_dofs, int64_t n_u, int64_t n_p,
                           const int32_t* cell_part, int rank, int nranks, int64_t* n_rows, int64_t* nnz,
                           int64_t* rowptr, uint32_t* col, int64_t* row_gids, int64_t* n_ghost_dofs,
                           int64_t* n_send_dofs, int64_t* n_local_cells) {
  Structure S;
  const std::string e = build_structure(dim, n_vertices, coords, n_cells, cell_vertices, cell_dofs, n_u, n_p, cell_part, rank, nranks, S);
  if (!e.empty()) { std::fprintf(stderr, "nsb_test_build_pattern: %s\n", e.c_str()); return -1; }
  if (n_rows) *n_rows = S.n_own_dofs();
  if (nnz) *nnz = S.nnz_local;
  if (n_ghost_dofs) *n_ghost_dofs = S.n_tot_dofs() - S.n_own_dofs();
  if (n_local_cells) *n_local_cells = S.nc;
  if (n_send_dofs) {
    int64_t t = 0;
    for (size_t k = 0; k < S.peer.size(); ++k) t += (int64_t)S.send_nodes[k].size() * dim + (int64_t)S.send_pids[k].size();
    *n_send_dofs = t;
  }
  if (rowptr && col) {
    std::vector<int64_t> rp;
    std::vector<uint32_t> cl;
    export_pattern(S, rp, cl);
    std::copy(rp.begin(), rp.end(), rowptr);
    std::copy(cl.begin(), cl.end(), col);
  }
  if (row_gids) {
    std::vector<int64_t> g;
    export_row_gids(S, g);
    std::copy(g.begin(), g.end(), row_gids);
  }
  return 0;
}

int nsb_test_halo_plan(int dim, int64_t n_vertices, const double* coords, int64_t n_cells, const uint32_t* cell_vertices,
                       const uint32_t* cell_dofs, int64_t n_u, int64_t n_p, const int32_t* cell_part, int rank, int nranks,
                       int64_t* n_ghost, int64_t* ghost_gdof, int32_t* n_peers, int32_t* peers, int64_t* send_u_ptr,
                       int64_t* send_u_gdof, int64_t* send_p_ptr, int64_t* send_p_gdof, int64_t* recv_u_count,
                       int64_t* recv_p_count) {
  Structure S;
  const std::string e = build_structure(dim, n_vertices, coords, n_cells, cell_vertices, cell_dofs, n_u, n_p, cell_part, rank, nranks, S);
  if (!e.empty()) { std::fprintf(stderr, "nsb_test_halo_plan: %s\n", e.c_str()); return -1; }
  if (n_ghost) *n_ghost = S.n_tot_dofs() - S.n_own_dofs();
  if (n_peers) *n_peers = (int32_t)S.peer.size();
  if (ghost_gdof) {
    int64_t k = 0;
    for (int A = S.nn_own; A < S.nn_own + S.nn_ghost; ++A)
      for (int c = 0; c < dim; ++c) ghost_gdof[k++] = S.node_gid[A] * dim + c;
    for (int P = S.np_own; P < S.np_own + S.np_ghost; ++P) ghost_gdof[k++] = n_u + S.pid_gid[P];
  }
  int64_t su = 0, sp = 0;
  for (size_t k = 0; k < S.peer.size(); ++k) {
    if (peers) peers[k] = S.peer[k];
    if (send_u_ptr) send_u_ptr[k] = su;
    if (send_p_ptr) send_p_ptr[k] = sp;
    for (int A : S.send_nodes[k])
      for (int c = 0; c < dim; ++c) { if (send_u_gdof) send_u_gdof[su] = S.node_gid[A] * dim + c; ++su; }
    for (int P : S.send_pids[k]) { if (send_p_gdof) send_p_gdof[sp] = n_u + S.pid_gid[P]; ++sp; }
    if (recv_u_count) recv_u_count[k] = (int64_t)S.recv_node_count[k] * dim;
    if (recv_p_count) recv_p_count[k] = S.recv_pid_count[k];
  }
  if (send_u_ptr) send_u_ptr[S.peer.size()] = su;
  if (send_p_ptr) send_p_ptr[S.peer.size()] = sp;
  return 0;
}

int nsb_test_tile_plan(int dim, int64_t n_vertices, const double* coords, int64_t n_cells, const uint32_t* cell_vertices,
                       const uint32_t* cell_dofs, int64_t n_u, int64_t n_p, const int32_t* cell_part, int rank, int nranks,
                       int64_t* out5) {
  Structure S;
  const std::string e = build_structure(dim, n_vertices, coords, n_cells, cell_vertices, cell_dofs, n_u, n_p,
                                        nranks > 1 ? cell_part : nullptr, rank, nranks, S);
  if (!e.empty()) { std::fprintf(stderr, "nsb_test_tile_plan: %s\n", e.c_str()); return -1; }
  TilePlan P;
  const TileLimits L{TILE_MAX_NODES, TILE_MAX_IDX, TILE_MAX_UNIQ, TILE_MAX_PUNIQ, VS_MAX_BLOCKS};
  const std::string e2 = build_tile_plan(S, L, P);
  if (!e2.empty()) { std::fprintf(stderr, "nsb_test_tile_plan: %s\n", e2.c_str()); return -1; }
  VsPlan V;
  const std::string e3 = build_vel_stream(S, P, V);
  if (!e3.empty()) { std::fprintf(stderr, "nsb_test_tile_plan: %s\n", e3.c_str()); return -1; }
  out5[0] = P.n_tiles(); out5[1] = (int64_t)P.tiles_int.size(); out5[2] = (int64_t)P.tiles_bnd.size();
  out5[3] = 4 * V.total_nq; out5[4] = verify_tile_plan(S, L, P) + verify_vel_stream(S, P, V);
  return 0;
}

int nsb_test_coarse_level(int dim, int64_t n_vertices, const double* coords, int64_t n_cells, const uint32_t* cell_vertices,
                          const uint32_t* cell_dofs, int64_t n_u, int64_t n_p, const int32_t* cell_part, int rank, int nranks,
                          int64_t* sizes4, int64_t* node_gid, int64_t* ends_gid, int64_t* vedge_pairs, int64_t* vertex_gid,
                          int64_t* cnbr_ptr, int64_t* cnbr_gid) {
  Structure S;
  const std::string e = build_structure(dim, n_vertices, coords, n_cells, cell_vertices, cell_dofs, n_u, n_p,
                                        nranks > 1 ? cell_part : nullptr, rank, nranks, S);
  if (!e.empty()) { std::fprintf(stderr, "nsb_test_coarse_level: %s\n", e.c_str()); return -1; }
  CoarseLevel C;
  const std::string e2 = build_coarse(S, C);
  if (!e2.empty()) { std::fprintf(stderr, "nsb_test_coarse_level: %s\n", e2.c_str()); return -1; }
  sizes4[0] = S.nn_own; sizes4[1] = (int64_t)C.vedge.size(); sizes4[2] = S.np_own; sizes4[3] = (int64_t)C.Sc.nbr.size();
  if (node_gid) for (int A = 0; A < S.nn_own; ++A) node_gid[A] = S.node_gid[A];
  if (ends_gid) for (size_t i = 0; i < C.node_ends.size(); ++i) ends_gid[i] = S.pid_gid[C.node_ends[i]];
  if (vedge_pairs)
    for (int P = 0; P < S.np_own; ++P)
      for (int64_t k = C.vedge_ptr[P]; k < C.vedge_ptr[P + 1]; ++k) { vedge_pairs[2 * k] = S.pid_gid[P]; vedge_pairs[2 * k + 1] = S.node_gid[C.vedge[k]]; }
  if (vertex_gid) for (int P = 0; P < S.np_own; ++P) vertex_gid[P] = S.pid_gid[P];
  if (cnbr_ptr) std::copy(C.Sc.nbr_ptr.begin(), C.Sc.nbr_ptr.end(), cnbr_ptr);
  if (cnbr_gid) for (size_t i = 0; i < C.Sc.nbr.size(); ++i) cnbr_gid[i] = S.pid_gid[C.Sc.nbr[i]];
  return 0;
}

int nsb_test_hessenberg_eigs(int n, const double* a, double* wr, double* wi) {
  std::vector<double> A(a, a + (size_t)n * n), r, i;
  if (!hessenberg_eigs(n, A, r, i)) return 1;
  std::copy(r.begin(), r.end(), wr);
  std::copy(i.begin(), i.end(), wi);
  return 0;
}

int nsb_solver_info(nsb_handle c, int* poly_degree, double* poly_probe_residual, int* amg_levels) {
  if (!c) return -1;
  if (poly_degree) {
    int d = 0;
    for (auto& r : c->lvF.roots) d += (r.second != 0.0) ? 2 : 1;
    *poly_degree = d;
  }
  if (poly_probe_residual) *poly_probe_residual = c->lvF.probe_res;
  if (amg_levels) *amg_levels = (int)c->amg.size();
  return 0;
}

int nsb_velocity_operator_info(nsb_handle c, int* precision, int64_t* value_bytes, int64_t* index_bytes, int64_t* tiles,
                               int64_t* blocks) {
  if (!c || !c->have_mesh) return fail(c, "no mesh uploaded");
  if (precision) *precision = c->opt.precond_precision;
  if (value_bytes) *value_bytes = (int64_t)vs_vals_bytes(c);
  if (index_bytes) *index_bytes = 16 * c->vs_total_nq + 64 * (int64_t)c->n_stiles + 4 * (int64_t)c->d_suniq_xoff.n;
  if (tiles) *tiles = c->n_stiles;
  if (blocks) *blocks = (int64_t)c->S.nbr.size();
  return 0;
}

int nsb_comm_info(nsb_handle c, int* nranks, int* halo_mode, int64_t* halo_doubles_per_exchange) {
  if (!c) return -1;
  if (nranks) *nranks = c->nranks;
  if (halo_mode) *halo_mode = c->nranks == 1 ? 0 : !c->ph.on ? 1 : c->fused_halo ? 3 : 2;
  if (halo_doubles_per_exchange) {
    int64_t t = 0;
    for (size_t k = 0; k < c->S.peer.size(); ++k) t += (int64_t)c->S.send_nodes[k].size() * c->dim;
    *halo_doubles_per_exchange = t;
  }
  return 0;
}

int nsb_get_coarse_operator(nsb_handle c, int64_t* n_rows, int64_t* n_blocks, int64_t* row_gid, int64_t* rowptr, int64_t* col_gid,
                            double* vals) {
  if (!c || !c->have_mesh || !c->cg.built) return fail(c, "no coarse level");
  NSB_TRY
  CK(cudaSetDevice(c->device));
  const Coarse& G = c->cg;
  if (n_rows) *n_rows = (int64_t)G.gid.size();
  if (n_blocks) *n_blocks = (int64_t)G.h_nbr_gid.size();
  if (row_gid) std::copy(G.gid.begin(), G.gid.end(), row_gid);
  if (rowptr) std::copy(G.h_nbr_ptr.begin(), G.h_nbr_ptr.end(), rowptr);
  if (col_gid) std::copy(G.h_nbr_gid.begin(), G.h_nbr_gid.end(), col_gid);
  if (vals) {
    if (!G.valid) return fail(c, "the coarse operator has not been assembled (linearised systems with velocity_cycle = 2 only)");
    CK(cudaMemcpyAsync(vals, G.cvals.p, G.cvals.n * sizeof(double), cudaMemcpyDeviceToHost, c->stream));
    CK(cudaStreamSynchronize(c->stream));
  }
  return 0;
  NSB_CATCH(c)
}

int nsb_velocity_pc_info(nsb_handle c, int* two_level, int* smoother_degree, int* coarse_degree, int64_t* coarse_rows,
                         int64_t* coarse_value_bytes, double* fine_lambda_max) {
  if (!c) return -1;
  if (two_level) *two_level = c->two_level ? 1 : 0;
  if (smoother_degree) *smoother_degree = (int)c->lvF.roots.size();
  if (coarse_degree) *coarse_degree = c->two_level ? (int)c->lvC.roots.size() : 0;
  if (coarse_rows) *coarse_rows = c->lvC.n;
  if (coarse_value_bytes) *coarse_value_bytes = (int64_t)coarse_vals_bytes(c);
  if (fine_lambda_max) *fine_lambda_max = c->lvF.ritz_top;
  return 0;
}

int nsb_get_solver_opts(nsb_handle c, nsb_solver_opts* o) {
  if (!c || !o) return -1;
  *o = c->opt;
  return 0;
}

int nsb_launch_count(nsb_handle c, int64_t* n) {
  if (!c) return -1;
  *n = c->launches;
  return 0;
}

}
```

navier-stokes_equations_b200/csrc/structure.cpp:

```cpp
#include "structure.hpp"

#include <algorithm>
#include <cstring>
#include <climits>
#include <cmath>
#include <numeric>

namespace nsb {

namespace {
struct Layout {
  int dim, NV, NN, DPC;
  int udof(int a, int c) const { return a < NV ? a * (dim + 1) + c : NV * (dim + 1) + (a - NV) * dim + c; }
  int pdof(int v) const { return v * (dim + 1) + dim; }
};
}

std::string build_structure(int dim, int64_t n_vertices, const double* coords, int64_t n_cells,
                            const uint32_t* cell_vertices, const uint32_t* cell_dofs, int64_t n_u,
                            int64_t n_p, const int32_t* cell_part, int rank, int nranks, Structure& S) {
  if (dim != 2 && dim != 3) return "dim must be 2 or 3";
  Layout L{dim, dim + 1, (dim == 2) ? 6 : 10, 0};
  L.DPC = dim * L.NN + L.NV;
  const int NV = L.NV, NN = L.NN, DPC = L.DPC;
// ... 251 lines not shown
      const double id = 1.0 / det;
      gl[1][0] = c00 * id;
      gl[1][1] = (J[0][2] * J[2][1] - J[0][1] * J[2][2]) * id;
      gl[1][2] = (J[0][1] * J[1][2] - J[0][2] * J[1][1]) * id;
      gl[2][0] = c01 * id;
      gl[2][1] = (J[0][0] * J[2][2] - J[0][2] * J[2][0]) * id;
      gl[2][2] = (J[0][2] * J[1][0] - J[0][0] * J[1][2]) * id;
      gl[3][0] = c02 * id;
      gl[3][1] = (J[0][1] * J[2][0] - J[0][0] * J[2][1]) * id;
      gl[3][2] = (J[0][0] * J[1][1] - J[0][1] * J[1][0]) * id;
      for (int k = 0; k < 3; ++k) gl[0][k] = -((gl[1][k] + gl[2][k]) + gl[3][k]);
    }
    if (!(det > 0)) ++negative;
    double h = 0;
    for (int v = 0; v < NV; ++v)
      for (int w = v + 1; w < NV; ++w) {
        double s = 0;
        for (int k = 0; k < dim; ++k) s += (X[v][k] - X[w][k]) * (X[v][k] - X[w][k]);
        h = std::max(h, std::sqrt(s));
      }
    for (int v = 0; v < NV; ++v)
      for (int k = 0; k < dim; ++k) g[v * dim + k] = gl[v][k];
    g[12] = det;
    g[13] = h;
    g[14] = 1.0 / h;
  }
  if (negative) return "mesh has cells with non-positive measure";
  (void)n_vertices;

  if (nranks > 1) {
    std::vector<std::vector<int64_t>> send_to(nranks);
    std::vector<char> seen(nranks);
    for (int64_t c = 0; c < n_cells; ++c) {
      int os[10], no = 0;
      for (int a = 0; a < NN; ++a) {
        const int o = owner[cn[(size_t)c * NN + a]];
        bool dup = false;
        for (int k = 0; k < no; ++k) dup |= (os[k] == o);
        if (!dup) os[no++] = o;
      }
      if (no == 1) continue;
      for (int a = 0; a < NN; ++a) {
        const int n = cn[(size_t)c * NN + a];
        if (owner[n] != rank) continue;
        for (int k = 0; k < no; ++k)
          if (os[k] != rank) send_to[os[k]].push_back(n);
      }
    }
    std::vector<int64_t> recv_cnt(nranks, 0), recv_pcnt(nranks, 0);
    for (int k = 0; k < nn_ghost; ++k) {
      recv_cnt[owner[ghosts[k]]]++;
      if (node_pid_glob[ghosts[k]] >= 0) recv_pcnt[owner[ghosts[k]]]++;
    }
    for (int s = 0; s < nranks; ++s) {
      auto& v = send_to[s];
      std::sort(v.begin(), v.end());
      v.erase(std::unique(v.begin(), v.end()), v.end());
      if (v.empty() && recv_cnt[s] == 0) continue;
      S.peer.push_back(s);
      std::vector<int> sn, sp;
      for (int64_t n : v) {
        sn.push_back(g2l[n]);
        if (node_pid_glob[n] >= 0) sp.push_back(pg2l[node_pid_glob[n]]);
      }
      S.send_nodes.push_back(sn);
      S.send_pids.push_back(sp);
      S.recv_node_count.push_back((int)recv_cnt[s]);
      S.recv_pid_count.push_back((int)recv_pcnt[s]);
    }
  }
  return "";
}

void export_pattern(const Structure& S, std::vector<int64_t>& rowptr, std::vector<uint32_t>& col) {
  const int dim = S.dim;
  const int64_t nrows = S.n_own_dofs();
  rowptr.assign(nrows + 1, 0);
  col.resize(S.nnz_local);
  auto fill_row = [&](int A, uint32_t* out) {
    int64_t k = 0;
    for (int64_t j = S.nbr_ptr[A]; j < S.nbr_ptr[A + 1]; ++j)
      for (int d = 0; d < dim; ++d) out[k++] = (uint32_t)(S.node_gid[S.nbr[j]] * dim + d);
    for (int64_t j = S.pnbr_ptr[A]; j < S.pnbr_ptr[A + 1]; ++j)
      out[k++] = (uint32_t)(S.n_u_glob + S.pid_gid[S.pnbr[j]]);
  };
  for (int A = 0; A < S.nn_own; ++A) {
    const int len = S.row_len(A);
    for (int c = 0; c < dim; ++c) {
      rowptr[(int64_t)dim * A + c] = S.rowbase[A] + (int64_t)c * len;
      fill_row(A, col.data() + S.rowbase[A] + (int64_t)c * len);
    }
  }
  for (int P = 0; P < S.np_own; ++P) {
    rowptr[(int64_t)dim * S.nn_own + P] = S.prowbase[P];
    fill_row(S.pid_node[P], col.data() + S.prowbase[P]);
  }
  rowptr[nrows] = S.nnz_local;
}

void export_row_gids(const Structure& S, std::vector<int64_t>& gid) {
  gid.resize(S.n_own_dofs());
  for (int A = 0; A < S.nn_own; ++A)
    for (int c = 0; c < S.dim; ++c) gid[(int64_t)S.dim * A + c] = S.node_gid[A] * S.dim + c;
  for (int P = 0; P < S.np_own; ++P) gid[(int64_t)S.dim * S.nn_own + P] = S.n_u_glob + S.pid_gid[P];
}

std::string build_tile_plan(const Structure& S, const TileLimits& L, TilePlan& P) {
  P = TilePlan();
  const int ntot = S.nn_own + S.nn_ghost, ptot = S.np_own + S.np_ghost;
  P.nbr_loc.assign(S.nbr.size(), 0);
  P.pnbr_loc.assign(S.pnbr.size(), 0);
  std::vector<int> stamp(ntot, -1), pstamp(ptot, -1), posn(ntot, 0), posp(ptot, 0);
  P.node_ptr.push_back(0); P.uniq_ptr.push_back(0); P.puniq_ptr.push_back(0);
  int A = 0, tile = 0;
  std::vector<int> U, PU;
  while (A < S.nn_own) {
    U.clear(); PU.clear();
    int idx = 0, cn = 0, vblk = 0;
    const int start = A;
    while (A < S.nn_own && cn < L.max_nodes) {
      const int nb = (int)(S.nbr_ptr[A + 1] - S.nbr_ptr[A]), np = (int)(S.pnbr_ptr[A + 1] - S.pnbr_ptr[A]);
      if (nb + np > L.max_idx || nb > L.max_uniq || np > L.max_puniq || (L.max_vel_blocks && (nb + 3) / 4 * 4 > L.max_vel_blocks))
        return "a node has more neighbours than one SpMV tile can stage";
      if (idx + nb + np > L.max_idx) break;
      if (L.max_vel_blocks && vblk + (nb + 3) / 4 * 4 > L.max_vel_blocks) break;
      vblk += (nb + 3) / 4 * 4;
      int newu = 0, newp = 0;
      for (int64_t k = S.nbr_ptr[A]; k < S.nbr_ptr[A + 1]; ++k) newu += stamp[S.nbr[k]] != tile;
      for (int64_t k = S.pnbr_ptr[A]; k < S.pnbr_ptr[A + 1]; ++k) newp += pstamp[S.pnbr[k]] != tile;
      if ((int)U.size() + newu > L.max_uniq || (int)PU.size() + newp > L.max_puniq) break;
      for (int64_t k = S.nbr_ptr[A]; k < S.nbr_ptr[A + 1]; ++k)
        if (stamp[S.nbr[k]] != tile) { stamp[S.nbr[k]] = tile; U.push_back(S.nbr[k]); }
      for (int64_t k = S.pnbr_ptr[A]; k < S.pnbr_ptr[A + 1]; ++k)
        if (pstamp[S.pnbr[k]] != tile) { pstamp[S.pnbr[k]] = tile; PU.push_back(S.pnbr[k]); }
      idx += nb + np; ++cn; ++A;
    }
    std::sort(U.begin(), U.end(), [&](int a, int b) { return S.node_xoff(a) < S.node_xoff(b); });
    std::sort(PU.begin(), PU.end(), [&](int a, int b) { return S.pid_xoff(a) < S.pid_xoff(b); });
    for (size_t i = 0; i < U.size(); ++i) { posn[U[i]] = (int)i; P.uniq_xoff.push_back((int)S.node_xoff(U[i])); }
    for (size_t i = 0; i < PU.size(); ++i) { posp[PU[i]] = (int)i; P.puniq_xoff.push_back((int)S.pid_xoff(PU[i])); }
    for (int B = start; B < A; ++B) {
      for (int64_t k = S.nbr_ptr[B]; k < S.nbr_ptr[B + 1]; ++k) P.nbr_loc[k] = (unsigned short)posn[S.nbr[k]];
      for (int64_t k = S.pnbr_ptr[B]; k < S.pnbr_ptr[B + 1]; ++k) P.pnbr_loc[k] = (unsigned short)posp[S.pnbr[k]];
    }
    bool reads_ghost = false;
    for (int n : U) reads_ghost |= (n >= S.nn_own);
    (reads_ghost ? P.tiles_bnd : P.tiles_int).push_back(tile);
    P.node_ptr.push_back(A); P.uniq_ptr.push_back((int)P.uniq_xoff.size()); P.puniq_ptr.push_back((int)P.puniq_xoff.size());
    ++tile;
  }
  return "";
}

std::string build_vel_stream(const Structure& S, const TilePlan& P, VsPlan& V) {
  V = VsPlan();
  const int nt = P.n_tiles();
  V.tiles.resize(nt);
  auto quads = [&](int A) { return (int)((S.nbr_ptr[A + 1] - S.nbr_ptr[A] + 3) / 4); };
  int64_t off = 0;
  std::vector<int> qstart;
  for (int t = 0; t < nt; ++t) {
    VsTile& T = V.tiles[t];
    std::memset(&T, 0, sizeof(T));
    T.n0 = P.node_ptr[t]; T.nn = P.node_ptr[t + 1] - T.n0;
    qstart.assign(T.nn + 1, 0);
    for (int a = 0; a < T.nn; ++a) qstart[a + 1] = qstart[a] + quads(T.n0 + a);
    if (qstart[T.nn] > VS_MAX_QUADS) return "an SpMV tile holds more velocity blocks than the streamed operator can stage";
    T.nquad = qstart[T.nn];
    T.NQ = (T.nquad + 31) / 32 * 32;
    if ((off + T.NQ) * 4 >= (int64_t)INT32_MAX) return "too many velocity blocks for 32-bit tile offsets";
    T.nq_off = (int)off;
    T.u0 = P.uniq_ptr[t]; T.nuq = P.uniq_ptr[t + 1] - T.u0;
    int a = 0;
    for (int w = 0; w <= VS_CONSUMERS; ++w) {
      const int target = (int)((int64_t)T.nquad * w / VS_CONSUMERS);
      while (a < T.nn && qstart[a] < target) ++a;
      T.split[w] = (unsigned short)qstart[a];
    }
    T.split[VS_CONSUMERS] = (unsigned short)T.nquad;
    off += T.NQ;
  }
  V.total_nq = off;
  V.meta.assign((size_t)off * 4, 0u);
#pragma omp parallel for schedule(static)
  for (int t = 0; t < nt; ++t) {
    const VsTile& T = V.tiles[t];
    uint32_t* m = V.meta.data() + (size_t)T.nq_off * 4;
    int q = 0;
    for (int a = 0; a < T.nn; ++a) {
      const int64_t k0 = S.nbr_ptr[T.n0 + a], k1 = S.nbr_ptr[T.n0 + a + 1];
      for (int64_t k = k0; k < k1; k += 4, ++q) {
        uint32_t loc[4];
        const int cnt = (int)std::min<int64_t>(4, k1 - k);
        for (int e = 0; e < 4; ++e) loc[e] = P.nbr_loc[k + (e < cnt ? e : 0)];
        m[4 * q + 0] = loc[0] | (loc[1] << 16);
        m[4 * q + 1] = loc[2] | (loc[3] << 16);
        m[4 * q + 2] = (uint32_t)a;
        m[4 * q + 3] = (uint32_t)(k - k0) | ((uint32_t)cnt << 16);
      }
    }
    for (; q < T.NQ; ++q) { m[4 * q + 0] = 0; m[4 * q + 1] = 0; m[4 * q + 2] = 0xffffu; m[4 * q + 3] = 0; }
  }
  return "";
}

int64_t verify_vel_stream(const Structure& S, const TilePlan& P, const VsPlan& V) {
  int64_t bad = 0;
  const int nt = P.n_tiles();
  if ((int)V.tiles.size() != nt) return 1;
  int64_t off = 0;
  int next_node = 0;
  for (int t = 0; t < nt; ++t) {
    const VsTile& T = V.tiles[t];
    if (T.n0 != next_node || T.nn <= 0 || T.nn > 64) ++bad;
    next_node = T.n0 + T.nn;
    if (T.nq_off != off || T.NQ % 32 || T.NQ < T.nquad || T.NQ > VS_MAX_QUADS) ++bad;
    if (T.u0 != P.uniq_ptr[t] || T.nuq != P.uniq_ptr[t + 1] - P.uniq_ptr[t]) ++bad;
    const uint32_t* m = V.meta.data() + (size_t)off * 4;
    int q = 0;
    std::vector<int> qstart(1, 0);
    for (int a = 0; a < T.nn; ++a) {
      const int64_t k0 = S.nbr_ptr[T.n0 + a], k1 = S.nbr_ptr[T.n0 + a + 1];
      for (int64_t k = k0; k < k1; k += 4, ++q) {
        const int cnt = (int)(m[4 * q + 3] >> 16), first = (int)(m[4 * q + 3] & 0xffffu);
        if ((int)m[4 * q + 2] != a || first != (int)(k - k0) || cnt != (int)std::min<int64_t>(4, k1 - k)) ++bad;
        for (int e = 0; e < 4; ++e) {
          const int loc = (int)((m[4 * q + e / 2] >> (16 * (e & 1))) & 0xffffu);
          if (loc >= T.nuq) { ++bad; continue; }
          if (e < cnt && P.uniq_xoff[T.u0 + loc] != (int)S.node_xoff(S.nbr[k + e])) ++bad;
        }
      }
      qstart.push_back(q);
    }
    if (q != T.nquad) ++bad;
    for (; q < T.NQ; ++q) if (m[4 * q + 2] != 0xffffu) ++bad;
    if (T.split[0] != 0 || T.split[VS_CONSUMERS] != T.nquad) ++bad;
    for (int w = 0; w < VS_CONSUMERS; ++w) {
      if (T.split[w] > T.split[w + 1]) ++bad;
      if (!std::binary_search(qstart.begin(), qstart.end(), (int)T.split[w])) ++bad;
    }
    off += T.NQ;
  }
  if (next_node != S.nn_own || off != V.total_nq) ++bad;
  return bad;
}

std::string build_coarse(const Structure& S, CoarseLevel& C) {
  C = CoarseLevel();
  static const int lines2[3][2] = {{0, 1}, {1, 2}, {2, 0}};
  static const int lines3[6][2] = {{0, 1}, {1, 2}, {2, 0}, {0, 3}, {1, 3}, {2, 3}};
  const int dim = S.dim, NV = S.NV, NN = S.NN, NL = NN - NV;
  Structure& Sc = C.Sc;
  Sc.dim = dim; Sc.NV = NV; Sc.NN = NN; Sc.DPC = S.DPC;
  Sc.rank = S.rank; Sc.nranks = S.nranks;
  Sc.nn_own = S.np_own; Sc.nn_ghost = S.np_ghost; Sc.np_own = 0; Sc.np_ghost = 0; Sc.nc = 0;
  Sc.node_gid = S.pid_gid;
  Sc.nbr_ptr.assign(S.np_own + 1, 0);
  for (int P = 0; P < S.np_own; ++P) {
    const int A = S.pid_node[P];
    Sc.nbr_ptr[P + 1] = Sc.nbr_ptr[P] + (S.pnbr_ptr[A + 1] - S.pnbr_ptr[A]);
  }
  Sc.nbr.resize((size_t)Sc.nbr_ptr[S.np_own]);
  Sc.selfrank.assign(S.np_own, 0);
  for (int P = 0; P < S.np_own; ++P) {
    const int A = S.pid_node[P];
    std::copy(S.pnbr.begin() + S.pnbr_ptr[A], S.pnbr.begin() + S.pnbr_ptr[A + 1], Sc.nbr.begin() + Sc.nbr_ptr[P]);
    Sc.selfrank[P] = S.pselfrank[P];
  }
  Sc.pnbr_ptr.assign(S.np_own + 1, 0);
  Sc.node_pid.assign(S.np_own + S.np_ghost, -1);
  Sc.peer = S.peer;
  Sc.send_nodes = S.send_pids;
  Sc.send_pids.assign(S.peer.size(), std::vector<int>());
  Sc.recv_node_count = S.recv_pid_count;
  Sc.recv_pid_count.assign(S.peer.size(), 0);
  std::vector<std::pair<int, int>> ve;
  C.node_ends.assign((size_t)S.nn_own * 2, -1);
  for (int c = 0; c < S.nc; ++c) {
    const int* cn = S.cell_nodes.data() + (size_t)c * NN;
    const int* cp = S.cell_pids.data() + (size_t)c * NV;
    for (int v = 0; v < NV; ++v)
      if (cn[v] < S.nn_own) { C.node_ends[2 * (size_t)cn[v]] = cp[v]; C.node_ends[2 * (size_t)cn[v] + 1] = cp[v]; }
    for (int l = 0; l < NL; ++l) {
      const int i = dim == 2 ? lines2[l][0] : lines3[l][0], j = dim == 2 ? lines2[l][1] : lines3[l][1];
      const int e = cn[NV + l];
      if (e < S.nn_own) { C.node_ends[2 * (size_t)e] = cp[i]; C.node_ends[2 * (size_t)e + 1] = cp[j]; }
      if (cp[i] < S.np_own) ve.emplace_back(cp[i], e);
      if (cp[j] < S.np_own) ve.emplace_back(cp[j], e);
    }
  }
  for (int A = 0; A < S.nn_own; ++A)
    if (C.node_ends[2 * (size_t)A] < 0) return "an owned node belongs to no local cell";
  std::sort(ve.begin(), ve.end());
  ve.erase(std::unique(ve.begin(), ve.end()), ve.end());
  C.vedge_ptr.assign(S.np_own + 1, 0);
  for (auto& pr : ve) C.vedge_ptr[pr.first + 1]++;
  for (int P = 0; P < S.np_own; ++P) C.vedge_ptr[P + 1] += C.vedge_ptr[P];
  C.vedge.resize(ve.size());
  for (size_t k = 0; k < ve.size(); ++k) C.vedge[k] = ve[k].second;
  return "";
}

int64_t verify_tile_plan(const Structure& S, const TileLimits& L, const TilePlan& P) {
  int64_t bad = 0;
  const int nt = P.n_tiles();
  if (nt < 0 || P.node_ptr.empty() || P.node_ptr.front() != 0 || P.node_ptr.back() != S.nn_own) return 1;
  if ((int)P.uniq_ptr.size() != nt + 1 || (int)P.puniq_ptr.size() != nt + 1) return 1;
  std::vector<char> seen(nt, 0);
  for (int t : P.tiles_int) { if (t < 0 || t >= nt || seen[t]) ++bad; else seen[t] = 1; }
  for (int t : P.tiles_bnd) { if (t < 0 || t >= nt || seen[t]) ++bad; else seen[t] = 2; }
  for (int t = 0; t < nt; ++t) if (!seen[t]) ++bad;
  if (bad) return bad;
  for (int t = 0; t < nt; ++t) {
    const int n0 = P.node_ptr[t], n1 = P.node_ptr[t + 1];
    const int u0 = P.uniq_ptr[t], nu = P.uniq_ptr[t + 1] - u0, q0 = P.puniq_ptr[t], nq = P.puniq_ptr[t + 1] - q0;
    if (n1 <= n0 || n1 - n0 > L.max_nodes || nu > L.max_uniq || nq > L.max_puniq) ++bad;
    int64_t idx = 0;
    bool ghost = false;
    for (int i = 1; i < nu; ++i) if (P.uniq_xoff[u0 + i] <= P.uniq_xoff[u0 + i - 1]) ++bad;
    for (int i = 1; i < nq; ++i) if (P.puniq_xoff[q0 + i] <= P.puniq_xoff[q0 + i - 1]) ++bad;
    for (int i = 0; i < nu; ++i) ghost |= P.uniq_xoff[u0 + i] >= S.n_own_dofs();
    if ((seen[t] == 2) != ghost) ++bad;
    for (int A = n0; A < n1; ++A) {
      idx += (S.nbr_ptr[A + 1] - S.nbr_ptr[A]) + (S.pnbr_ptr[A + 1] - S.pnbr_ptr[A]);
      for (int64_t k = S.nbr_ptr[A]; k < S.nbr_ptr[A + 1]; ++k) {
        const int loc = P.nbr_loc[k];
        if (loc >= nu || P.uniq_xoff[u0 + loc] != (int)S.node_xoff(S.nbr[k])) ++bad;
      }
      for (int64_t k = S.pnbr_ptr[A]; k < S.pnbr_ptr[A + 1]; ++k) {
        const int loc = P.pnbr_loc[k];
        if (loc >= nq || P.puniq_xoff[q0 + loc] != (int)S.pid_xoff(S.pnbr[k])) ++bad;
      }
    }
    if (idx > L.max_idx) ++bad;
  }
  return bad;
}

}
```

navier-stokes_equations_b200/csrc/structure.hpp:

```cpp
#pragma once
#include <cstdint>
#include <string>
#include <vector>

namespace nsb {

struct Structure {
  int dim = 0, NV = 0, NN = 0, DPC = 0;
  int rank = 0, nranks = 1;
  int64_t n_u_glob = 0, n_p_glob = 0, n_cells_glob = 0;
  int nn_own = 0, nn_ghost = 0, np_own = 0, np_ghost = 0, nc = 0;
  std::vector<int64_t> node_gid;
  std::vector<int64_t> pid_gid;
  std::vector<int> cell_gid;
  std::vector<int> cell_nodes;
  std::vector<int> cell_pids;
  std::vector<int> node_pid;
  std::vector<int> pid_node;
  std::vector<int64_t> nbr_ptr;
  std::vector<int> nbr;
  std::vector<int64_t> pnbr_ptr;
  std::vector<int> pnbr;
  std::vector<int> selfrank;
  std::vector<int> pselfrank;
  std::vector<int64_t> rowbase;
  std::vector<int64_t> prowbase;
  int64_t nnz_local = 0;
  std::vector<int64_t> n2c_ptr;
  std::vector<uint32_t> n2c;
  std::vector<uint16_t> rank_uu;
  std::vector<uint16_t> rank_up;
  std::vector<double> cell_geom;
  std::vector<int> peer;
  std::vector<std::vector<int>> send_nodes;
  std::vector<std::vector<int>> send_pids;
  std::vector<int> recv_node_count, recv_pid_count;
  int max_row_len = 0, max_node_smem_doubles = 0;

  int64_t n_own_dofs() const { return (int64_t)dim * nn_own + np_own; }
  int64_t n_tot_dofs() const { return (int64_t)dim * (nn_own + nn_ghost) + np_own + np_ghost; }
  int64_t node_xoff(int A) const {
    return A < nn_own ? (int64_t)dim * A : n_own_dofs() + (int64_t)dim * (A - nn_own);
  }
  int64_t pid_xoff(int P) const {
    return P < np_own ? (int64_t)dim * nn_own + P
                      : n_own_dofs() + (int64_t)dim * nn_ghost + (P - np_own);
  }
  int row_len(int A) const {
    return dim * (int)(nbr_ptr[A + 1] - nbr_ptr[A]) + (int)(pnbr_ptr[A + 1] - pnbr_ptr[A]);
  }
};

std::string build_structure(int dim, int64_t n_vertices, const double* coords, int64_t n_cells,
                            const uint32_t* cell_vertices, const uint32_t* cell_dofs, int64_t n_u,
                            int64_t n_p, const int32_t* cell_part, int rank, int nranks, Structure& S);

struct TileLimits {
  int max_nodes, max_idx, max_uniq, max_puniq;
  int max_vel_blocks = 0;
};
struct TilePlan {
  std::vector<int> node_ptr;
  std::vector<int> uniq_ptr, uniq_xoff;
  std::vector<int> puniq_ptr, puniq_xoff;
  std::vector<unsigned short> nbr_loc;
  std::vector<unsigned short> pnbr_loc;
  std::vector<int> tiles_int, tiles_bnd;
  int n_tiles() const { return (int)node_ptr.size() - 1; }
};
std::string build_tile_plan(const Structure& S, const TileLimits& L, TilePlan& P);
int64_t verify_tile_plan(const Structure& S, const TileLimits& L, const TilePlan& P);

constexpr int VS_CONSUMERS = 8;
constexpr int VS_MAX_BLOCKS = 2048;
constexpr int VS_MAX_QUADS = VS_MAX_BLOCKS / 4;
struct alignas(16) VsTile {
  int n0, nn;
  int nquad, NQ;
  int nq_off;
  int u0, nuq;
  int pad0;
  unsigned short split[VS_CONSUMERS + 1];
  unsigned short pad1[32 - 16 - (VS_CONSUMERS + 1)];
};
static_assert(sizeof(VsTile) == 64, "VsTile is one 64-byte TMA bulk copy");
struct VsPlan {
  std::vector<VsTile> tiles;
  std::vector<uint32_t> meta;
  int64_t total_nq = 0;
};
std::string build_vel_stream(const Structure& S, const TilePlan& P, VsPlan& V);
int64_t verify_vel_stream(const Structure& S, const TilePlan& P, const VsPlan& V);

struct CoarseLevel {
  Structure Sc;
  std::vector<int64_t> vedge_ptr;
  std::vector<int> vedge;
  std::vector<int> node_ends;
};
std::string build_coarse(const Structure& S, CoarseLevel& C);

void export_pattern(const Structure& S, std::vector<int64_t>& rowptr, std::vector<uint32_t>& col);

void export_row_gids(const Structure& S, std::vector<int64_t>& gid);

}
```

navier-stokes_equations_b200/csrc/twolevel.cuh:

```cuda
#pragma once
#include "assemble.cuh"
#include "velstream.cuh"

namespace nsb {

constexpr int CG_WARPS = 4;
constexpr int CG_MAX_NB = 64;

template <int DIM>
__global__ void __launch_bounds__(CG_WARPS * 32)
k_coarse_rows(DevMesh M, const double* __restrict__ ctx, double gamma, double wsum, const long long* __restrict__ cnbr_ptr,
              const int* __restrict__ cnbr_vxoff, const unsigned char* __restrict__ cflag, double* __restrict__ cvals,
              double* __restrict__ cdinv) {
  constexpr int NV = DIM + 1, NN = Fe<DIM>::NN, PL = DIM * DIM;
  using CL = CtxL<DIM>;
  __shared__ double sacc[CG_WARPS][CG_MAX_NB * PL];
  const int lane = threadIdx.x & 31, wid = threadIdx.x >> 5;
  const int P = blockIdx.x * CG_WARPS + wid;
  if (P >= M.np_own) return;
  double* acc = sacc[wid];
  const int A = M.pid_node[P];
  const long long q0 = cnbr_ptr[P];
  const int nbc = (int)(cnbr_ptr[P + 1] - q0);
  for (int k = lane; k < nbc * PL; k += 32) acc[k] = 0.0;
  __syncwarp();
  const long long kc0 = M.n2c_ptr[A];
  const int ncell = (int)(M.n2c_ptr[A + 1] - kc0);
  for (int ic = 0; ic < ncell; ++ic) {
    const uint32_t pk = __ldg(M.n2c + kc0 + ic);
    const size_t cell = pk >> 4;
    const int a = (int)(pk & 15u);
    const double* cx = ctx + cell * CL::N;
    double t = 0.0;
    if (lane < NN) {
      t = cx[CL::S + a * NN + lane];
#pragma unroll
      for (int e = NV; e < NN; ++e)
        if (node_i<DIM>(e) == a || node_j<DIM>(e) == a) t += 0.5 * cx[CL::S + e * NN + lane];
    }
    double s = 0.0;
#pragma unroll
    for (int f = 0; f < NN; ++f) {
      const double tf = __shfl_sync(NSB_FULL, t, f);
      if (lane < NV) {
        if (f == lane) s += tf;
        else if (f >= NV && (node_i<DIM>(f) == lane || node_j<DIM>(f) == lane)) s += 0.5 * tf;
      }
    }
    if (lane < NV) {
      const int j = lane;
      const int rp = M.rank_up[(cell * NN + a) * NV + j];
      const double vol = gamma * wsum * cx[CL::ABSJ];
      double ga[DIM], gj[DIM];
#pragma unroll
      for (int k = 0; k < DIM; ++k) { ga[k] = cx[CL::GL + a * DIM + k]; gj[k] = cx[CL::GL + j * DIM + k]; }
#pragma unroll
      for (int c = 0; c < DIM; ++c)
#pragma unroll
        for (int d = 0; d < DIM; ++d) acc[rp * PL + c * DIM + d] += ((c == d) ? s : 0.0) + vol * ga[c] * gj[d];
    }
    __syncwarp();
  }
  const int self = M.pselfrank[P];
  const int xA = DIM * A;
  for (int k = lane; k < nbc * PL; k += 32) {
    const int Q = k / PL, c = (k % PL) / DIM, d = k % DIM;
    const bool crow = cflag[xA + c] != 0;
    const bool ccol = cflag[__ldg(cnbr_vxoff + q0 + Q) + d] != 0;
    double v = acc[k];
    if (crow || ccol) v = (Q == self && c == d && crow) ? 1.0 : 0.0;
    acc[k] = v;
    cvals[(q0 + Q) * PL + k % PL] = v;
  }
  __syncwarp();
  if (lane == 0) {
    double Dm[DIM][DIM];
#pragma unroll
    for (int c = 0; c < DIM; ++c)
#pragma unroll
      for (int e = 0; e < DIM; ++e) Dm[c][e] = acc[self * PL + c * DIM + e];
    double* o = cdinv + (size_t)P * PL;
    if (DIM == 2) {
      const double id = 1.0 / (Dm[0][0] * Dm[1][1] - Dm[0][1] * Dm[1][0]);
      o[0] = Dm[1][1] * id; o[1] = -Dm[0][1] * id; o[2] = -Dm[1][0] * id; o[3] = Dm[0][0] * id;
    } else {
      const double c00 = Dm[1][1] * Dm[2][2] - Dm[1][2] * Dm[2][1];
      const double c01 = Dm[1][2] * Dm[2][0] - Dm[1][0] * Dm[2][2];
      const double c02 = Dm[1][0] * Dm[2][1] - Dm[1][1] * Dm[2][0];
      const double id = 1.0 / (Dm[0][0] * c00 + Dm[0][1] * c01 + Dm[0][2] * c02);
      o[0] = c00 * id;
      o[1] = (Dm[0][2] * Dm[2][1] - Dm[0][1] * Dm[2][2]) * id;
      o[2] = (Dm[0][1] * Dm[1][2] - Dm[0][2] * Dm[1][1]) * id;
      o[3] = c01 * id;
      o[4] = (Dm[0][0] * Dm[2][2] - Dm[0][2] * Dm[2][0]) * id;
      o[5] = (Dm[0][2] * Dm[1][0] - Dm[0][0] * Dm[1][2]) * id;
      o[6] = c02 * id;
      o[7] = (Dm[0][1] * Dm[2][0] - Dm[0][0] * Dm[2][1]) * id;
      o[8] = (Dm[0][0] * Dm[1][1] - Dm[0][1] * Dm[1][0]) * id;
    }
  }
}

template <int DIM, typename VT>
__global__ void __launch_bounds__(256)
k_coarse_pack(const VsTile* __restrict__ tiles, const uint32_t* __restrict__ meta, const long long* __restrict__ cnbr_ptr,
              const double* __restrict__ cvals, const double* __restrict__ cdinv, VT* __restrict__ out) {
  constexpr int PL = DIM * DIM;
  const VsTile hd = tiles[blockIdx.x];
  VT* o = out + (long long)PL * 4 * hd.nq_off;
  const uint4* mt = reinterpret_cast<const uint4*>(meta) + hd.nq_off;
  for (int jb = threadIdx.x; jb < 4 * hd.NQ; jb += blockDim.x) {
    const int q = jb >> 2, e = jb & 3;
    double b[DIM][DIM];
#pragma unroll
    for (int r = 0; r < DIM; ++r)
#pragma unroll
      for (int c = 0; c < DIM; ++c) b[r][c] = 0.0;
    const uint4 m = __ldg(mt + q);
    if (m.z != 0xffffu && e < (int)(m.w >> 16)) {
      const int P = hd.n0 + (int)m.z;
      const long long blk = cnbr_ptr[P] + (int)(m.w & 0xffffu) + e;
#pragma unroll
      for (int r = 0; r < DIM; ++r)
#pragma unroll
        for (int c = 0; c < DIM; ++c)
#pragma unroll
          for (int ee = 0; ee < DIM; ++ee) b[r][c] += __ldg(cdinv + (size_t)P * PL + r * DIM + ee) * __ldg(cvals + blk * PL + ee * DIM + c);
    }
#pragma unroll
    for (int r = 0; r < DIM; ++r)
#pragma unroll
      for (int c = 0; c < DIM; ++c) o[((size_t)(r * DIM + c) * hd.NQ + q) * 4 + e] = vs_from_double<DIM, VT>(b[r][c]);
  }
}

template <int DIM>
__global__ void k_restrict(int np_own, const int* __restrict__ pid_node, const long long* __restrict__ vedge_ptr,
                           const int* __restrict__ vedge_xoff, const unsigned char* __restrict__ cflag,
                           const double* __restrict__ r, double* __restrict__ rc) {
  const int P = blockIdx.x * blockDim.x + threadIdx.x;
  if (P >= np_own) return;
  const int xA = DIM * __ldg(pid_node + P);
  double s[DIM];
#pragma unroll
  for (int c = 0; c < DIM; ++c) s[c] = r[xA + c];
  for (long long k = vedge_ptr[P]; k < vedge_ptr[P + 1]; ++k) {
    const int xo = __ldg(vedge_xoff + k);
#pragma unroll
    for (int c = 0; c < DIM; ++c) s[c] += 0.5 * r[xo + c];
  }
#pragma unroll
  for (int c = 0; c < DIM; ++c) rc[DIM * P + c] = cflag[xA + c] ? 0.0 : s[c];
}

template <int DIM>
__global__ void k_prolong(int nn_own, const int* __restrict__ ends_xoff, const unsigned char* __restrict__ cflag,
                          const double* __restrict__ ec, double* __restrict__ y) {
  const int i = blockIdx.x * blockDim.x + threadIdx.x;
  if (i >= nn_own * DIM) return;
  const int A = i / DIM, c = i % DIM;
  const int e0 = __ldg(ends_xoff + 2 * A), e1 = __ldg(ends_xoff + 2 * A + 1);
  y[i] = cflag[i] ? 0.0 : 0.5 * (ec[e0 + c] + ec[e1 + c]);
}

}
```

navier-stokes_equations_b200/csrc/velstream.cuh:

```cuda
#pragma once
#include <cuda_fp16.h>

#include "device.cuh"
#include "linalg.cuh"
#include "structure.hpp"

namespace nsb {

constexpr int VS_GROUPS = 2;
constexpr int VS_THREADS = (VS_GROUPS * VS_CONSUMERS + 1) * 32;
constexpr int VS_MAX_UNIQ = TILE_MAX_UNIQ;

template <int DIM, typename VT> struct VsLayout {
  static constexpr int PL = DIM * DIM;
  static constexpr int VAL_BYTES = PL * VS_MAX_BLOCKS * (int)sizeof(VT);
  static constexpr int META_BYTES = VS_MAX_QUADS * 16;
  static constexpr int XS_BYTES = VS_MAX_UNIQ * DIM * 8;
  static constexpr int YS_BYTES = TILE_MAX_NODES * DIM * 8;
  static constexpr int HDR_BYTES = 64;
  static constexpr int OFF_VAL = 0;
  static constexpr int OFF_META = OFF_VAL + VAL_BYTES;
  static constexpr int OFF_XS = OFF_META + META_BYTES;
  static constexpr int OFF_YS = OFF_XS + XS_BYTES;
  static constexpr int OFF_HDR = OFF_YS + YS_BYTES;
  static constexpr int STAGE_BYTES = ((OFF_HDR + HDR_BYTES + 127) / 128) * 128;
  static constexpr int STAGES = (227 * 1024 - 256) / STAGE_BYTES >= 3 ? 3 : 2;
  static constexpr int SMEM_BYTES = STAGES * STAGE_BYTES + 256;
};

__device__ __forceinline__ uint32_t smem_u32(const void* p) { return (uint32_t)__cvta_generic_to_shared(p); }
__device__ __forceinline__ void mbar_init(uint64_t* bar, uint32_t count) {
  asm volatile("mbarrier.init.shared::cta.b64 [%0], %1;" ::"r"(smem_u32(bar)), "r"(count) : "memory");
}
__device__ __forceinline__ void mbar_expect_tx(uint64_t* bar, uint32_t bytes) {
  asm volatile("mbarrier.arrive.expect_tx.shared::cta.b64 _, [%0], %1;" ::"r"(smem_u32(bar)), "r"(bytes) : "memory");
}
__device__ __forceinline__ void mbar_arrive(uint64_t* bar) {
  asm volatile("mbarrier.arrive.shared::cta.b64 _, [%0];" ::"r"(smem_u32(bar)) : "memory");
}
__device__ __forceinline__ void mbar_wait(uint64_t* bar, uint32_t parity) {
  asm volatile(
      "{\n\t.reg .pred p;\n\t"
      "WAIT_%=:\n\t"
      "mbarrier.try_wait.parity.shared::cta.b64 p, [%0], %1;\n\t"
      "@p bra DONE_%=;\n\t"
      "bra WAIT_%=;\n\t"
      "DONE_%=:\n\t}" ::"r"(smem_u32(bar)), "r"(parity) : "memory");
}
__device__ __forceinline__ void tma_bulk_g2s(void* dst, const void* src, uint32_t bytes, uint64_t* bar) {
  asm volatile("cp.async.bulk.shared::cluster.global.mbarrier::complete_tx::bytes [%0], [%1], %2, [%3];" ::"r"(smem_u32(dst)),
               "l"(src), "r"(bytes), "r"(smem_u32(bar))
               : "memory");
}
__device__ __forceinline__ void cp_async_8(void* dst, const void* src) {
  asm volatile("cp.async.ca.shared.global [%0], [%1], 8;" ::"r"(smem_u32(dst)), "l"(src) : "memory");
}
__device__ __forceinline__ void cp_async_arrive_noinc(uint64_t* bar) {
  asm volatile("cp.async.mbarrier.arrive.noinc.shared::cta.b64 [%0];" ::"r"(smem_u32(bar)) : "memory");
}

struct VsHalo;
template <int DIM> __device__ __forceinline__ void vs_deliver(const VsHalo& hx, int node, int comp, double v);

__device__ __forceinline__ void vs_load4(const float* p, double (&v)[4]) {
  const float4 f = *reinterpret_cast<const float4*>(p);
  v[0] = (double)f.x; v[1] = (double)f.y; v[2] = (double)f.z; v[3] = (double)f.w;
}
__device__ __forceinline__ void vs_load4(const __half* p, double (&v)[4]) {
  const uint2 r = *reinterpret_cast<const uint2*>(p);
  const float2 a = __half22float2(*reinterpret_cast<const __half2*>(&r.x)), b = __half22float2(*reinterpret_cast<const __half2*>(&r.y));
  v[0] = (double)a.x; v[1] = (double)a.y; v[2] = (double)b.x; v[3] = (double)b.y;
}

struct VsHalo {
  const unsigned long long* flags;
  const int* peer_rank;
  int npeers;
  int n_int;
  unsigned long long wait_seq;
  int ghost_start;
  const int* send_ptr;
  const int2* send_dst;
  double* const* peer_arena;
  long long y_off;
  unsigned long long* const* peer_flags;
  int my_rank;
  unsigned long long push_seq;
  unsigned int* counter;
};

template <int DIM, typename VT, int MODE, bool HALO>
__global__ void __launch_bounds__(VS_THREADS, 1)
k_vel_stream(const VsTile* __restrict__ tiles, int n_tiles, const int* __restrict__ tile_list, const VT* __restrict__ vals,
             const uint32_t* __restrict__ meta, const int* __restrict__ uniq_xoff, const double* __restrict__ x,
             double* __restrict__ y, const double* __restrict__ u, double* __restrict__ poly, PolyCoef pc, VsHalo hx) {
  using L = VsLayout<DIM, VT>;
  constexpr int PL = L::PL;
  constexpr int S = L::STAGES;
  extern __shared__ __align__(128) unsigned char vs_smem[];
  uint64_t* full = reinterpret_cast<uint64_t*>(vs_smem + S * L::STAGE_BYTES);
  uint64_t* empty = full + S;
  const int warp = threadIdx.x >> 5, lane = threadIdx.x & 31;
  if (threadIdx.x == 0) {
    for (int s = 0; s < S; ++s) {
      mbar_init(full + s, 1 + 32);
      mbar_init(empty + s, VS_CONSUMERS);
    }
    asm volatile("fence.mbarrier_init.release.cluster;" ::: "memory");
  }
  __syncthreads();
  const int my_tiles = (n_tiles - (int)blockIdx.x + (int)gridDim.x - 1) / (int)gridDim.x;

  if (warp == 0) {
    bool waited = false;
    for (int it = 0; it < my_tiles; ++it) {
      const int s = it % S;
      const uint32_t ph = (uint32_t)(it / S) & 1u;
      if (it >= S) mbar_wait(empty + s, ph ^ 1u);
      int t = (int)blockIdx.x + it * (int)gridDim.x;
      bool ghosts = false;
      if (HALO) {
        ghosts = t >= hx.n_int;
        if (ghosts && !waited) {
          if (hx.wait_seq && lane < hx.npeers) {
            const volatile unsigned long long* f = hx.flags + hx.peer_rank[lane];
            while (*f < hx.wait_seq) { }
          }
          __threadfence_system();
          __syncwarp();
          waited = true;
        }
        t = __ldg(tile_list + t);
      }
      const VsTile* hd = tiles + t;
      const int NQ = __ldg(&hd->NQ), nq_off = __ldg(&hd->nq_off), u0 = __ldg(&hd->u0), nuq = __ldg(&hd->nuq);
      unsigned char* st = vs_smem + s * L::STAGE_BYTES;
      if (lane == 0) {
        const uint32_t vb = (uint32_t)(PL * 4 * NQ * (int)sizeof(VT)), mb = (uint32_t)(NQ * 16);
        mbar_expect_tx(full + s, vb + mb + (uint32_t)L::HDR_BYTES);
        tma_bulk_g2s(st + L::OFF_HDR, hd, L::HDR_BYTES, full + s);
        tma_bulk_g2s(st + L::OFF_VAL, vals + (long long)PL * 4 * nq_off, vb, full + s);
        tma_bulk_g2s(st + L::OFF_META, meta + (long long)4 * nq_off, mb, full + s);
      }
      double* xs = reinterpret_cast<double*>(st + L::OFF_XS);
      constexpr int PER_LANE = VS_MAX_UNIQ / 32;
      int xo[PER_LANE];
#pragma unroll
      for (int q = 0; q < PER_LANE; ++q) {
        const int i = lane + 32 * q;
        xo[q] = i < nuq ? __ldg(uniq_xoff + u0 + i) : -1;
      }
      if (HALO && ghosts) {
#pragma unroll
        for (int q0 = 0; q0 < PER_LANE; q0 += 4) {
          double gv[4][DIM];
#pragma unroll
          for (int q = q0; q < q0 + 4; ++q)
            if (xo[q] >= hx.ghost_start) {
#pragma unroll
              for (int c = 0; c < DIM; ++c) gv[q - q0][c] = __ldcg(x + xo[q] + c);
            }
#pragma unroll
          for (int q = q0; q < q0 + 4; ++q) {
            const int i = lane + 32 * q;
            if (xo[q] >= hx.ghost_start) {
#pragma unroll
              for (int c = 0; c < DIM; ++c) xs[i * DIM + c] = gv[q - q0][c];
            } else if (xo[q] >= 0) {
#pragma unroll
              for (int c = 0; c < DIM; ++c) cp_async_8(xs + i * DIM + c, x + xo[q] + c);
            }
          }
        }
        __threadfence_block();
        cp_async_arrive_noinc(full + s);
      } else {
#pragma unroll
        for (int q = 0; q < PER_LANE; ++q) {
          if (xo[q] >= 0) {
            const int i = lane + 32 * q;
#pragma unroll
            for (int c = 0; c < DIM; ++c) cp_async_8(xs + i * DIM + c, x + xo[q] + c);
          }
        }
        cp_async_arrive_noinc(full + s);
      }
    }
    return;
  }

  const int grp = (warp - 1) / VS_CONSUMERS;
  const int cw = (warp - 1) % VS_CONSUMERS;
  for (int it = grp; it < my_tiles; it += VS_GROUPS) {
    const int s = it % S;
    const uint32_t ph = (uint32_t)(it / S) & 1u;
    mbar_wait(full + s, ph);
    unsigned char* st = vs_smem + s * L::STAGE_BYTES;
    const VsTile* hd = reinterpret_cast<const VsTile*>(st + L::OFF_HDR);
    const VT* sv = reinterpret_cast<const VT*>(st + L::OFF_VAL);
    const uint4* sm = reinterpret_cast<const uint4*>(st + L::OFF_META);
    const double* xs = reinterpret_cast<const double*>(st + L::OFF_XS);
    double* ys = reinterpret_cast<double*>(st + L::OFF_YS);
    const int NQ = hd->NQ, nn = hd->nn, n0 = hd->n0, nquad = hd->nquad;
    const int b0 = hd->split[cw], b1 = hd->split[cw + 1];
    const int na = b0 < b1 ? (int)sm[b0].z : 0;
    const int nb_ = b0 < b1 ? (b1 < nquad ? (int)sm[b1].z : nn) : 0;
    const int r0 = DIM * na, r1 = DIM * nb_;
    const long long rowg0 = (long long)DIM * n0;
    double pu[2], pp[2];
#pragma unroll
    for (int q = 0; q < 2; ++q) {
      const int i = r0 + lane + 32 * q;
      pu[q] = 0.0; pp[q] = 0.0;
      if (MODE >= 3 && i < r1) { pu[q] = u[rowg0 + i]; if (MODE == 3) pp[q] = poly[rowg0 + i]; }
    }
    int carry_row = -1;
    double carry[DIM];
#pragma unroll
    for (int r = 0; r < DIM; ++r) carry[r] = 0.0;
    for (int base = b0; base < b1; base += 32) {
      const int j = base + lane;
      const bool ok = j < b1;
      double acc[DIM];
#pragma unroll
      for (int r = 0; r < DIM; ++r) acc[r] = 0.0;
      int row = 0xffff;
      if (ok) {
        const uint4 m = sm[j];
        row = (int)m.z;
        double xv[4][DIM];
#pragma unroll
        for (int e = 0; e < 4; ++e) {
          const int loc = (int)(((e < 2 ? m.x : m.y) >> (16 * (e & 1))) & 0xffffu);
#pragma unroll
          for (int c = 0; c < DIM; ++c) xv[e][c] = xs[loc * DIM + c];
        }
#pragma unroll
        for (int r = 0; r < DIM; ++r)
#pragma unroll
          for (int c = 0; c < DIM; ++c) {
            double v[4];
            vs_load4(sv + ((size_t)(r * DIM + c) * NQ + j) * 4, v);
#pragma unroll
            for (int e = 0; e < 4; ++e) acc[r] += v[e] * xv[e][c];
          }
      }
      const int row0 = __shfl_sync(NSB_FULL, row, 0);
      if (lane == 0 && carry_row >= 0) {
        if (carry_row == row0) {
#pragma unroll
          for (int r = 0; r < DIM; ++r) acc[r] += carry[r];
        } else {
#pragma unroll
          for (int r = 0; r < DIM; ++r) ys[carry_row * DIM + r] = carry[r];
        }
      }
      const int prev = __shfl_up_sync(NSB_FULL, row, 1);
      const unsigned heads = __ballot_sync(NSB_FULL, lane == 0 || prev != row);
      const int pos = lane - (31 - __clz(heads & (0xffffffffu >> (31 - lane))));
#pragma unroll
      for (int d = 1; d < 32; d <<= 1) {
#pragma unroll
        for (int r = 0; r < DIM; ++r) {
          const double o = __shfl_up_sync(NSB_FULL, acc[r], d);
          if (pos >= d) acc[r] += o;
        }
      }
      const bool last_of_seg = (lane == 31) || ((heads >> (lane + 1)) & 1u);
      if (last_of_seg && lane < 31 && row < nn) {
#pragma unroll
        for (int r = 0; r < DIM; ++r) ys[row * DIM + r] = acc[r];
      }
      carry_row = __shfl_sync(NSB_FULL, row, 31);
      if (carry_row >= nn) carry_row = -1;
#pragma unroll
      for (int r = 0; r < DIM; ++r) carry[r] = __shfl_sync(NSB_FULL, acc[r], 31);
    }
    if (lane == 0 && carry_row >= 0) {
#pragma unroll
      for (int r = 0; r < DIM; ++r) ys[carry_row * DIM + r] = carry[r];
    }
    __syncwarp();
    const bool deliver = HALO && hx.push_seq && ((int)blockIdx.x + it * (int)gridDim.x) >= hx.n_int;
    for (int i = r0 + lane, q = 0; i < r1; i += 32, ++q) {
      const double t = ys[i];
      if (MODE == 2) {
        y[rowg0 + i] = t;
        if (deliver) vs_deliver<DIM>(hx, n0 + i / DIM, i % DIM, t);
      } else {
        const double uv = q == 0 ? pu[0] : q == 1 ? pu[1] : u[rowg0 + i];
        const double pv = MODE != 3 ? 0.0 : q == 0 ? pp[0] : q == 1 ? pp[1] : poly[rowg0 + i];
        const double yv = pc.cu * uv + pc.ct * t;
        y[rowg0 + i] = yv;
        if (deliver) vs_deliver<DIM>(hx, n0 + i / DIM, i % DIM, yv);
        if (MODE == 3) poly[rowg0 + i] = pv + pc.cpu * uv + pc.cpy * yv;
      }
    }
    __syncwarp();
    if (lane == 0) mbar_arrive(empty + s);
  }
  if (HALO && hx.push_seq) {
    __threadfence_system();
    __syncwarp();
    unsigned int prev = 0;
    if (lane == 0) prev = atomicAdd(hx.counter, 1u);
    prev = __shfl_sync(NSB_FULL, prev, 0);
    if (prev == gridDim.x * (VS_GROUPS * VS_CONSUMERS) - 1) {
      __threadfence_system();
      if (lane < hx.npeers) {
        volatile unsigned long long* f = hx.peer_flags[lane] + hx.my_rank;
        *f = hx.push_seq;
      }
      if (lane == 0) *hx.counter = 0;
      __threadfence_system();
    }
  }
}

template <int DIM> __device__ __forceinline__ void vs_deliver(const VsHalo& hx, int node, int comp, double v) {
  for (int k = __ldg(hx.send_ptr + node); k < __ldg(hx.send_ptr + node + 1); ++k) {
    const int2 d = __ldg(hx.send_dst + k);
    hx.peer_arena[d.x][hx.y_off + d.y + comp] = v;
  }
}

template <int DIM, typename VT> __device__ __forceinline__ VT vs_from_double(double v);
template <> __device__ __forceinline__ float vs_from_double<2, float>(double v) { return (float)v; }
template <> __device__ __forceinline__ float vs_from_double<3, float>(double v) { return (float)v; }
template <> __device__ __forceinline__ __half vs_from_double<2, __half>(double v) { return __float2half_rn((float)v); }
template <> __device__ __forceinline__ __half vs_from_double<3, __half>(double v) { return __float2half_rn((float)v); }

template <int DIM, typename VT>
__global__ void __launch_bounds__(256)
k_vel_pack(DevMesh M, const VsTile* __restrict__ tiles, const uint32_t* __restrict__ meta, const double* __restrict__ vals,
           const double* __restrict__ dinv, VT* __restrict__ out) {
  constexpr int PL = DIM * DIM;
  const VsTile hd = tiles[blockIdx.x];
  VT* o = out + (long long)PL * 4 * hd.nq_off;
  const uint4* mt = reinterpret_cast<const uint4*>(meta) + hd.nq_off;
  for (int jb = threadIdx.x; jb < 4 * hd.NQ; jb += blockDim.x) {
    const int q = jb >> 2, e = jb & 3;
    double b[DIM][DIM];
#pragma unroll
    for (int r = 0; r < DIM; ++r)
#pragma unroll
      for (int c = 0; c < DIM; ++c) b[r][c] = 0.0;
    const uint4 m = __ldg(mt + q);
    if (m.z != 0xffffu && e < (int)(m.w >> 16)) {
      const int A = hd.n0 + (int)m.z;
      const NodeDesc d = load_desc(M.nd + A);
      const int k = (int)(m.w & 0xffffu) + e, len = DIM * d.nb + d.np;
      double f[DIM][DIM], di[DIM][DIM];
#pragma unroll
      for (int r = 0; r < DIM; ++r)
#pragma unroll
        for (int c = 0; c < DIM; ++c) {
          f[r][c] = __ldcs(vals + d.rowbase + (long long)r * len + DIM * k + c);
          di[r][c] = __ldg(dinv + (size_t)A * PL + r * DIM + c);
        }
#pragma unroll
      for (int r = 0; r < DIM; ++r)
#pragma unroll
        for (int c = 0; c < DIM; ++c)
#pragma unroll
          for (int ee = 0; ee < DIM; ++ee) b[r][c] += di[r][ee] * f[ee][c];
    }
#pragma unroll
    for (int r = 0; r < DIM; ++r)
#pragma unroll
      for (int c = 0; c < DIM; ++c) o[((size_t)(r * DIM + c) * hd.NQ + q) * 4 + e] = vs_from_double<DIM, VT>(b[r][c]);
  }
}

}
```

Baseline: 0.4627.

## Compress velocity-stream quad descriptors and assign bank-aware x slots in shared memory

Shrinks the per-quad metadata streamed by TMA from 16 to 8 bytes by packing three 10-bit slot indices plus a node index into two words. The block offset and count move to a separate array that only the pack kernels read. A host-side greedy assigner places each tile's unique neighbours into shared-memory x slots so that the 16-lane groups gathering x hit fewer bank conflicts. The segmented scan also exits early once the longest run is covered. In exchange the host setup is more complex and there is an extra per-lane slot load when staging x.

Result: slower. 0.3688, median of 6 (-20.3%).

```diff
diff --git a/navier-stokes_equations_b200/csrc/nsb200.cu b/navier-stokes_equations_b200/csrc/nsb200.cu
--- a/navier-stokes_equations_b200/csrc/nsb200.cu
+++ b/navier-stokes_equations_b200/csrc/nsb200.cu
@@ -5,6 +5,7 @@
 #include <nccl.h>
 
 #include <algorithm>
+#include <chrono>
 #include <cmath>
 #include <cstdlib>
 #include <cstring>
@@ -193,7 +194,9 @@
 struct VsDev {
   const VsTile* tiles;
   const uint32_t* meta;
+  const uint32_t* qpack;
   const int* uniq_xoff;
+  const uint16_t* uniq_slot;
   const unsigned char* vals;
   int n_tiles;
 };
@@ -214,8 +217,9 @@
 
 struct Coarse {
   DBuf<VsTile> tiles;
-  DBuf<uint32_t> meta;
+  DBuf<uint32_t> meta, qpack;
   DBuf<int> uniq_xoff;
+  DBuf<uint16_t> uniq_slot;
   DBuf<unsigned char> vals;
   int n_tiles = 0;
   int64_t total_nq = 0;
@@ -276,7 +280,8 @@
   bool forcing_set[2] = {false, false};
   DBuf<unsigned char> vs_vals;
   DBuf<VsTile> d_vs_tiles;
-  DBuf<uint32_t> d_vs_meta;
+  DBuf<uint32_t> d_vs_meta, d_vs_qpack;
+  DBuf<uint16_t> d_vs_uslot;
   int64_t vs_total_nq = 0;
   bool vs_valid = false;
   int ctx_stride = 0;
@@ -457,9 +462,9 @@
   if (c->vs_vals.p) {
     id = c->prof.begin(PC_ASM_PACK, c->stream);
     if (c->opt.precond_precision == 16)
-      k_vel_pack<DIM, __half><<<c->n_stiles, 256, 0, c->stream>>>(c->M, c->d_vs_tiles.p, c->d_vs_meta.p, c->vals.p, c->dinv.p, reinterpret_cast<__half*>(c->vs_vals.p));
+      k_vel_pack<DIM, __half><<<c->n_stiles, 256, 0, c->stream>>>(c->M, c->d_vs_tiles.p, c->d_vs_meta.p, c->d_vs_qpack.p, c->vals.p, c->dinv.p, reinterpret_cast<__half*>(c->vs_vals.p));
     else
-      k_vel_pack<DIM, float><<<c->n_stiles, 256, 0, c->stream>>>(c->M, c->d_vs_tiles.p, c->d_vs_meta.p, c->vals.p, c->dinv.p, reinterpret_cast<float*>(c->vs_vals.p));
+      k_vel_pack<DIM, float><<<c->n_stiles, 256, 0, c->stream>>>(c->M, c->d_vs_tiles.p, c->d_vs_meta.p, c->d_vs_qpack.p, c->vals.p, c->dinv.p, reinterpret_cast<float*>(c->vs_vals.p));
     c->launch_check();
     c->prof.end(id, c->stream);
     c->vs_valid = true;
@@ -488,7 +493,7 @@
   if (ntiles <= 0) return;
   const int grid = std::min(ntiles, c->num_sms);
   k_vel_stream<DIM, VT, MODE, HALO><<<grid, VS_THREADS, VsLayout<DIM, VT>::SMEM_BYTES, c->stream>>>(
-      D.tiles, ntiles, list, reinterpret_cast<const VT*>(D.vals), D.meta, D.uniq_xoff, x, y, u, poly, pc, hx);
+      D.tiles, ntiles, list, reinterpret_cast<const VT*>(D.vals), D.meta, D.uniq_xoff, D.uniq_slot, x, y, u, poly, pc, hx);
   c->launch_check();
 }
 template <int MODE, bool HALO>
@@ -601,10 +606,10 @@
 
 
 VsDev fine_dev(const nsb_ctx* c) {
-  return VsDev{c->d_vs_tiles.p, c->d_vs_meta.p, c->d_suniq_xoff.p, c->vs_vals.p, c->n_stiles};
+  return VsDev{c->d_vs_tiles.p, c->d_vs_meta.p, c->d_vs_qpack.p, c->d_suniq_xoff.p, c->d_vs_uslot.p, c->vs_vals.p, c->n_stiles};
 }
 VsDev coarse_dev(const nsb_ctx* c) {
-  return VsDev{c->cg.tiles.p, c->cg.meta.p, c->cg.uniq_xoff.p, c->cg.vals.p, c->cg.n_tiles};
+  return VsDev{c->cg.tiles.p, c->cg.meta.p, c->cg.qpack.p, c->cg.uniq_xoff.p, c->cg.uniq_slot.p, c->cg.vals.p, c->cg.n_tiles};
 }
 
 void halo_exchange_coarse(nsb_ctx* c, double* v) {
@@ -853,9 +858,9 @@
                                                                                      c->cflag.p, G.cvals.p, G.dinv.p);
   c->launch_check();
   if (c->opt.precond_precision == 16)
-    k_coarse_pack<DIM, __half><<<G.n_tiles, 256, 0, c->stream>>>(G.tiles.p, G.meta.p, G.nbr_ptr.p, G.cvals.p, G.dinv.p, reinterpret_cast<__half*>(G.vals.p));
+    k_coarse_pack<DIM, __half><<<G.n_tiles, 256, 0, c->stream>>>(G.tiles.p, G.meta.p, G.qpack.p, G.nbr_ptr.p, G.cvals.p, G.dinv.p, reinterpret_cast<__half*>(G.vals.p));
   else
-    k_coarse_pack<DIM, float><<<G.n_tiles, 256, 0, c->stream>>>(G.tiles.p, G.meta.p, G.nbr_ptr.p, G.cvals.p, G.dinv.p, reinterpret_cast<float*>(G.vals.p));
+    k_coarse_pack<DIM, float><<<G.n_tiles, 256, 0, c->stream>>>(G.tiles.p, G.meta.p, G.qpack.p, G.nbr_ptr.p, G.cvals.p, G.dinv.p, reinterpret_cast<float*>(G.vals.p));
   c->launch_check();
   c->prof.end(id, c->stream);
   G.valid = true;
@@ -1177,7 +1182,8 @@
     c->d_suniq_ptr.upload(P.uniq_ptr, c->stream); c->d_suniq_xoff.upload(P.uniq_xoff, c->stream);
     c->d_spuniq_ptr.upload(P.puniq_ptr, c->stream); c->d_spuniq_xoff.upload(P.puniq_xoff, c->stream);
     c->d_nbr_loc.upload(P.nbr_loc, c->stream); c->d_pnbr_loc.upload(P.pnbr_loc, c->stream);
-    c->d_vs_tiles.upload(V.tiles, c->stream); c->d_vs_meta.upload(V.meta, c->stream);
+    c->d_vs_tiles.upload(V.tiles, c->stream); c->d_vs_meta.upload(V.meta, c->stream); c->d_vs_qpack.upload(V.qpack, c->stream);
+    c->d_vs_uslot.upload(V.uniq_slot, c->stream);
     c->vs_total_nq = V.total_nq;
     CK(cudaStreamSynchronize(c->stream));
     c->stiles.node_ptr = c->d_stile_ptr.p;
@@ -1371,7 +1377,8 @@
   G.n_tiles = P.n_tiles();
   G.total_nq = V.total_nq;
   G.h_tiles_int = P.tiles_int; G.h_tiles_bnd = P.tiles_bnd; G.h_tile_node_ptr = P.node_ptr;
-  G.tiles.upload(V.tiles, st); G.meta.upload(V.meta, st); G.uniq_xoff.upload(P.uniq_xoff, st);
+  G.tiles.upload(V.tiles, st); G.meta.upload(V.meta, st); G.qpack.upload(V.qpack, st);
+  G.uniq_xoff.upload(P.uniq_xoff, st); G.uniq_slot.upload(V.uniq_slot, st);
   std::vector<long long> t64(Sc.nbr_ptr.begin(), Sc.nbr_ptr.end()), v64(CL.vedge_ptr.begin(), CL.vedge_ptr.end());
   G.nbr_ptr.upload(t64, st); G.vedge_ptr.upload(v64, st);
   std::vector<int> vx(Sc.nbr.size()), ex(CL.vedge.size()), en(CL.node_ends.size()), sx;
@@ -1558,25 +1565,30 @@
                   std::vector<double>& val) {
   const int dim = c->dim, PL = dim * dim;
   std::vector<VsTile> tiles(D.n_tiles);
-  std::vector<uint32_t> meta((size_t)total_nq * 4);
+  std::vector<uint32_t> meta((size_t)total_nq * 2), qpack((size_t)total_nq);
   std::vector<int> uniq(n_uniq);
+  std::vector<uint16_t> slot(n_uniq);
   std::vector<VT> v((size_t)total_nq * 4 * PL);
   CK(cudaMemcpyAsync(tiles.data(), D.tiles, tiles.size() * sizeof(VsTile), cudaMemcpyDeviceToHost, c->stream));
   CK(cudaMemcpyAsync(meta.data(), D.meta, meta.size() * sizeof(uint32_t), cudaMemcpyDeviceToHost, c->stream));
+  CK(cudaMemcpyAsync(qpack.data(), D.qpack, qpack.size() * sizeof(uint32_t), cudaMemcpyDeviceToHost, c->stream));
   CK(cudaMemcpyAsync(uniq.data(), D.uniq_xoff, uniq.size() * sizeof(int), cudaMemcpyDeviceToHost, c->stream));
+  CK(cudaMemcpyAsync(slot.data(), D.uniq_slot, slot.size() * sizeof(uint16_t), cudaMemcpyDeviceToHost, c->stream));
   CK(cudaMemcpyAsync(v.data(), D.vals, v.size() * sizeof(VT), cudaMemcpyDeviceToHost, c->stream));
   CK(cudaStreamSynchronize(c->stream));
+  std::vector<int> pos_of(VS_MAX_UNIQ);
   for (const VsTile& T : tiles) {
-    const uint32_t* m = meta.data() + (size_t)T.nq_off * 4;
+    const uint32_t* m = meta.data() + (size_t)T.nq_off * 2;
     const VT* tv = v.data() + (size_t)T.nq_off * 4 * PL;
+    for (int i = 0; i < T.nuq; ++i) pos_of[slot[T.u0 + i]] = i;
     for (int q = 0; q < T.nquad; ++q) {
-      const uint32_t* mq = m + 4 * q;
-      if (mq[2] == 0xffffu) continue;
-      const int cnt = (int)(mq[3] >> 16);
+      const uint32_t a = m[2 * q + 1] >> VS_SLOT_BITS;
+      if (a == VS_PAD_NODE) continue;
+      const int cnt = (int)(qpack[T.nq_off + q] >> 16);
       for (int e = 0; e < cnt; ++e) {
-        const int loc = (int)(((e < 2 ? mq[0] : mq[1]) >> (16 * (e & 1))) & 0xffffu);
-        node.push_back(T.n0 + (int)mq[2]);
-        nbr.push_back(uniq[T.u0 + loc] / dim);
+        const int s = (int)((e < 3 ? m[2 * q] >> (VS_SLOT_BITS * e) : m[2 * q + 1]) & VS_SLOT_MASK);
+        node.push_back(T.n0 + (int)a);
+        nbr.push_back(uniq[T.u0 + pos_of[s]] / dim);
         for (int rc = 0; rc < PL; ++rc) val.push_back((double)(float)tv[((size_t)rc * T.NQ + q) * 4 + e]);
       }
     }
@@ -2435,6 +2447,28 @@
   return 0;
 }
 
+int nsb_test_vel_stream_banks(int dim, int64_t n_vertices, const double* coords, int64_t n_cells, const uint32_t* cell_vertices,
+                              const uint32_t* cell_dofs, int64_t n_u, int64_t n_p, const int32_t* cell_part, int rank, int nranks,
+                              int bank_aware, double* out3) {
+  Structure S;
+  const std::string e = build_structure(dim, n_vertices, coords, n_cells, cell_vertices, cell_dofs, n_u, n_p,
+                                        nranks > 1 ? cell_part : nullptr, rank, nranks, S);
+  if (!e.empty()) { std::fprintf(stderr, "nsb_test_vel_stream_banks: %s\n", e.c_str()); return -1; }
+  TilePlan P;
+  const TileLimits L{TILE_MAX_NODES, TILE_MAX_IDX, TILE_MAX_UNIQ, TILE_MAX_PUNIQ, VS_MAX_BLOCKS};
+  const std::string e2 = build_tile_plan(S, L, P);
+  if (!e2.empty()) { std::fprintf(stderr, "nsb_test_vel_stream_banks: %s\n", e2.c_str()); return -1; }
+  VsPlan V;
+  const auto t0 = std::chrono::steady_clock::now();
+  const std::string e3 = build_vel_stream(S, P, V, bank_aware != 0);
+  const double secs = std::chrono::duration<double>(std::chrono::steady_clock::now() - t0).count();
+  if (!e3.empty()) { std::fprintf(stderr, "nsb_test_vel_stream_banks: %s\n", e3.c_str()); return -1; }
+  out3[0] = vel_stream_x_wavefronts(S, V);
+  out3[1] = secs;
+  out3[2] = (double)verify_vel_stream(S, P, V);
+  return 0;
+}
+
 int nsb_test_coarse_level(int dim, int64_t n_vertices, const double* coords, int64_t n_cells, const uint32_t* cell_vertices,
                           const uint32_t* cell_dofs, int64_t n_u, int64_t n_p, const int32_t* cell_part, int rank, int nranks,
                           int64_t* sizes4, int64_t* node_gid, int64_t* ends_gid, int64_t* vedge_pairs, int64_t* vertex_gid,
@@ -2483,7 +2517,7 @@
   if (!c || !c->have_mesh) return fail(c, "no mesh uploaded");
   if (precision) *precision = c->opt.precond_precision;
   if (value_bytes) *value_bytes = (int64_t)vs_vals_bytes(c);
-  if (index_bytes) *index_bytes = 16 * c->vs_total_nq + 64 * (int64_t)c->n_stiles + 4 * (int64_t)c->d_suniq_xoff.n;
+  if (index_bytes) *index_bytes = 8 * c->vs_total_nq + 64 * (int64_t)c->n_stiles + 6 * (int64_t)c->d_suniq_xoff.n;
   if (tiles) *tiles = c->n_stiles;
   if (blocks) *blocks = (int64_t)c->S.nbr.size();
   return 0;
diff --git a/navier-stokes_equations_b200/csrc/structure.cpp b/navier-stokes_equations_b200/csrc/structure.cpp
--- a/navier-stokes_equations_b200/csrc/structure.cpp
+++ b/navier-stokes_equations_b200/csrc/structure.cpp
@@ -427,7 +427,58 @@
   return "";
 }
 
-std::string build_vel_stream(const Structure& S, const TilePlan& P, VsPlan& V) {
+namespace {
+constexpr int VS_BANKS = 16;
+int vs_bank_classes(int dim) { return VS_BANKS / std::gcd(dim, VS_BANKS); }
+
+template <typename F> void vs_for_each_group(const VsTile& T, F&& f) {
+  for (int w = 0; w < VS_CONSUMERS; ++w)
+    for (int base = T.split[w]; base < T.split[w + 1]; base += 32)
+      for (int h = 0; h < 2; ++h) {
+        const int j0 = base + 16 * h, j1 = std::min<int>(j0 + 16, T.split[w + 1]);
+        if (j0 < j1)
+          for (int e = 0; e < 4; ++e) f(j0, j1, e);
+      }
+}
+
+void assign_slots(int dim, const VsTile& T, const uint32_t* locq, uint16_t* slot) {
+  const int M = vs_bank_classes(dim), cap = VS_MAX_UNIQ / M, nu = T.nuq;
+  std::vector<std::vector<int>> groups(nu);
+  int ng = 0;
+  vs_for_each_group(T, [&](int j0, int j1, int e) {
+    for (int j = j0; j < j1; ++j) {
+      const int p = (int)locq[4 * j + e];
+      if (groups[p].empty() || groups[p].back() != ng) groups[p].push_back(ng);
+    }
+    ++ng;
+  });
+  std::vector<int> load((size_t)ng * M, 0), gmax(ng, 0), fill(M, 0), order(nu);
+  std::iota(order.begin(), order.end(), 0);
+  std::stable_sort(order.begin(), order.end(), [&](int a, int b) { return groups[a].size() > groups[b].size(); });
+  for (int p : order) {
+    int best = -1;
+    int64_t best_cost = 0;
+    for (int r = 0; r < M; ++r) {
+      if (fill[r] >= cap) continue;
+      int added = 0, sum = 0;
+      for (int g : groups[p]) {
+        const int l = load[(size_t)g * M + r];
+        added += l + 1 > gmax[g];
+        sum += l;
+      }
+      const int64_t cost = ((int64_t)added << 40) | ((int64_t)sum << 20) | fill[r];
+      if (best < 0 || cost < best_cost) { best = r; best_cost = cost; }
+    }
+    for (int g : groups[p]) {
+      int& l = load[(size_t)g * M + best];
+      gmax[g] = std::max(gmax[g], ++l);
+    }
+    slot[p] = (uint16_t)(best + M * fill[best]++);
+  }
+}
+}
+
+std::string build_vel_stream(const Structure& S, const TilePlan& P, VsPlan& V, bool bank_aware) {
   V = VsPlan();
   const int nt = P.n_tiles();
   V.tiles.resize(nt);
@@ -446,6 +497,7 @@
     if ((off + T.NQ) * 4 >= (int64_t)INT32_MAX) return "too many velocity blocks for 32-bit tile offsets";
     T.nq_off = (int)off;
     T.u0 = P.uniq_ptr[t]; T.nuq = P.uniq_ptr[t + 1] - T.u0;
+    if (T.nn >= (int)VS_PAD_NODE || T.nuq > VS_MAX_UNIQ) return "an SpMV tile has more nodes or neighbours than the streamed operator's quad descriptors can address";
     int a = 0;
     for (int w = 0; w <= VS_CONSUMERS; ++w) {
       const int target = (int)((int64_t)T.nquad * w / VS_CONSUMERS);
@@ -456,33 +508,73 @@
     off += T.NQ;
   }
   V.total_nq = off;
-  V.meta.assign((size_t)off * 4, 0u);
-#pragma omp parallel for schedule(static)
-  for (int t = 0; t < nt; ++t) {
+  V.meta.assign((size_t)off * 2, 0u);
+  V.qpack.assign((size_t)off, 0u);
+  V.uniq_slot.assign(P.uniq_xoff.size(), 0);
+#pragma omp parallel
+  {
+    std::vector<uint32_t> locq;
+#pragma omp for schedule(dynamic, 64)
+    for (int t = 0; t < nt; ++t) {
+      const VsTile& T = V.tiles[t];
+      locq.assign((size_t)4 * T.nquad, 0u);
+      uint32_t* pk = V.qpack.data() + T.nq_off;
+      int q = 0;
+      for (int a = 0; a < T.nn; ++a) {
+        const int64_t k0 = S.nbr_ptr[T.n0 + a], k1 = S.nbr_ptr[T.n0 + a + 1];
+        for (int64_t k = k0; k < k1; k += 4, ++q) {
+          const int cnt = (int)std::min<int64_t>(4, k1 - k);
+          for (int e = 0; e < 4; ++e) locq[4 * q + e] = P.nbr_loc[k + (e < cnt ? e : 0)];
+          pk[q] = (uint32_t)(k - k0) | ((uint32_t)cnt << 16);
+        }
+      }
+      uint16_t* sl = V.uniq_slot.data() + T.u0;
+      if (bank_aware) assign_slots(S.dim, T, locq.data(), sl);
+      else std::iota(sl, sl + T.nuq, (uint16_t)0);
+      uint32_t* m = V.meta.data() + (size_t)T.nq_off * 2;
+      q = 0;
+      for (int a = 0; a < T.nn; ++a)
+        for (int64_t k = S.nbr_ptr[T.n0 + a]; k < S.nbr_ptr[T.n0 + a + 1]; k += 4, ++q) {
+          const uint32_t* l = locq.data() + 4 * q;
+          m[2 * q] = sl[l[0]] | ((uint32_t)sl[l[1]] << VS_SLOT_BITS) | ((uint32_t)sl[l[2]] << (2 * VS_SLOT_BITS));
+          m[2 * q + 1] = sl[l[3]] | ((uint32_t)a << VS_SLOT_BITS);
+        }
+      for (; q < T.NQ; ++q) { m[2 * q] = 0; m[2 * q + 1] = VS_PAD_NODE << VS_SLOT_BITS; }
+    }
+  }
+  return "";
+}
+
+double vel_stream_x_wavefronts(const Structure& S, const VsPlan& V) {
+  int64_t groups = 0, waves = 0;
+#pragma omp parallel for schedule(dynamic, 64) reduction(+ : groups, waves)
+  for (size_t t = 0; t < V.tiles.size(); ++t) {
     const VsTile& T = V.tiles[t];
-    uint32_t* m = V.meta.data() + (size_t)T.nq_off * 4;
-    int q = 0;
-    for (int a = 0; a < T.nn; ++a) {
-      const int64_t k0 = S.nbr_ptr[T.n0 + a], k1 = S.nbr_ptr[T.n0 + a + 1];
-      for (int64_t k = k0; k < k1; k += 4, ++q) {
-        uint32_t loc[4];
-        const int cnt = (int)std::min<int64_t>(4, k1 - k);
-        for (int e = 0; e < 4; ++e) loc[e] = P.nbr_loc[k + (e < cnt ? e : 0)];
-        m[4 * q + 0] = loc[0] | (loc[1] << 16);
-        m[4 * q + 1] = loc[2] | (loc[3] << 16);
-        m[4 * q + 2] = (uint32_t)a;
-        m[4 * q + 3] = (uint32_t)(k - k0) | ((uint32_t)cnt << 16);
-      }
-    }
-    for (; q < T.NQ; ++q) { m[4 * q + 0] = 0; m[4 * q + 1] = 0; m[4 * q + 2] = 0xffffu; m[4 * q + 3] = 0; }
-  }
-  return "";
+    const uint32_t* m = V.meta.data() + (size_t)T.nq_off * 2;
+    vs_for_each_group(T, [&](int j0, int j1, int e) {
+      for (int c = 0; c < S.dim; ++c) {
+        std::vector<uint32_t> words;
+        for (int j = j0; j < j1; ++j) {
+          const uint32_t s = (e < 3 ? m[2 * j] >> (VS_SLOT_BITS * e) : m[2 * j + 1]) & VS_SLOT_MASK;
+          words.push_back((uint32_t)S.dim * s + (uint32_t)c);
+        }
+        std::sort(words.begin(), words.end());
+        words.erase(std::unique(words.begin(), words.end()), words.end());
+        int per_bank[VS_BANKS] = {0}, most = 0;
+        for (uint32_t w : words) most = std::max(most, ++per_bank[w % VS_BANKS]);
+        waves += most;
+        ++groups;
+      }
+    });
+  }
+  return groups ? (double)waves / (double)groups : 0.0;
 }
 
 int64_t verify_vel_stream(const Structure& S, const TilePlan& P, const VsPlan& V) {
   int64_t bad = 0;
   const int nt = P.n_tiles();
   if ((int)V.tiles.size() != nt) return 1;
+  if ((int64_t)V.meta.size() != 2 * V.total_nq || (int64_t)V.qpack.size() != V.total_nq || V.uniq_slot.size() != P.uniq_xoff.size()) return 1;
   int64_t off = 0;
   int next_node = 0;
   for (int t = 0; t < nt; ++t) {
@@ -490,25 +582,35 @@
     if (T.n0 != next_node || T.nn <= 0 || T.nn > 64) ++bad;
     next_node = T.n0 + T.nn;
     if (T.nq_off != off || T.NQ % 32 || T.NQ < T.nquad || T.NQ > VS_MAX_QUADS) ++bad;
+    if (off + T.NQ > V.total_nq) return bad + 1;
     if (T.u0 != P.uniq_ptr[t] || T.nuq != P.uniq_ptr[t + 1] - P.uniq_ptr[t]) ++bad;
-    const uint32_t* m = V.meta.data() + (size_t)off * 4;
+    if (T.nn >= (int)VS_PAD_NODE || T.nuq > VS_MAX_UNIQ || (size_t)T.u0 + T.nuq > V.uniq_slot.size()) { ++bad; off += T.NQ; continue; }
+    std::vector<int> pos_of(VS_MAX_UNIQ, -1);
+    for (int i = 0; i < T.nuq; ++i) {
+      const int s = V.uniq_slot[T.u0 + i];
+      if (s >= VS_MAX_UNIQ || pos_of[s] >= 0) ++bad;
+      else pos_of[s] = i;
+    }
+    const uint32_t* m = V.meta.data() + (size_t)off * 2;
+    const uint32_t* pk = V.qpack.data() + off;
     int q = 0;
     std::vector<int> qstart(1, 0);
     for (int a = 0; a < T.nn; ++a) {
       const int64_t k0 = S.nbr_ptr[T.n0 + a], k1 = S.nbr_ptr[T.n0 + a + 1];
       for (int64_t k = k0; k < k1; k += 4, ++q) {
-        const int cnt = (int)(m[4 * q + 3] >> 16), first = (int)(m[4 * q + 3] & 0xffffu);
-        if ((int)m[4 * q + 2] != a || first != (int)(k - k0) || cnt != (int)std::min<int64_t>(4, k1 - k)) ++bad;
+        const int cnt = (int)(pk[q] >> 16), first = (int)(pk[q] & 0xffffu);
+        if ((int)(m[2 * q + 1] >> VS_SLOT_BITS) != a || first != (int)(k - k0) || cnt != (int)std::min<int64_t>(4, k1 - k)) ++bad;
+        if (m[2 * q] >> (3 * VS_SLOT_BITS)) ++bad;
         for (int e = 0; e < 4; ++e) {
-          const int loc = (int)((m[4 * q + e / 2] >> (16 * (e & 1))) & 0xffffu);
-          if (loc >= T.nuq) { ++bad; continue; }
-          if (e < cnt && P.uniq_xoff[T.u0 + loc] != (int)S.node_xoff(S.nbr[k + e])) ++bad;
+          const int s = (int)((e < 3 ? m[2 * q] >> (VS_SLOT_BITS * e) : m[2 * q + 1]) & VS_SLOT_MASK);
+          if (s >= VS_MAX_UNIQ || pos_of[s] < 0) { ++bad; continue; }
+          if (e < cnt && P.uniq_xoff[T.u0 + pos_of[s]] != (int)S.node_xoff(S.nbr[k + e])) ++bad;
         }
       }
       qstart.push_back(q);
     }
     if (q != T.nquad) ++bad;
-    for (; q < T.NQ; ++q) if (m[4 * q + 2] != 0xffffu) ++bad;
+    for (; q < T.NQ; ++q) if (m[2 * q + 1] >> VS_SLOT_BITS != VS_PAD_NODE) ++bad;
     if (T.split[0] != 0 || T.split[VS_CONSUMERS] != T.nquad) ++bad;
     for (int w = 0; w < VS_CONSUMERS; ++w) {
       if (T.split[w] > T.split[w + 1]) ++bad;
diff --git a/navier-stokes_equations_b200/csrc/structure.hpp b/navier-stokes_equations_b200/csrc/structure.hpp
--- a/navier-stokes_equations_b200/csrc/structure.hpp
+++ b/navier-stokes_equations_b200/csrc/structure.hpp
@@ -74,6 +74,10 @@
 constexpr int VS_CONSUMERS = 8;
 constexpr int VS_MAX_BLOCKS = 2048;
 constexpr int VS_MAX_QUADS = VS_MAX_BLOCKS / 4;
+constexpr int VS_MAX_UNIQ = 768;
+constexpr int VS_SLOT_BITS = 10;
+constexpr uint32_t VS_SLOT_MASK = (1u << VS_SLOT_BITS) - 1;
+constexpr uint32_t VS_PAD_NODE = 0x7f;
 struct alignas(16) VsTile {
   int n0, nn;
   int nquad, NQ;
@@ -87,10 +91,13 @@
 struct VsPlan {
   std::vector<VsTile> tiles;
   std::vector<uint32_t> meta;
+  std::vector<uint32_t> qpack;
+  std::vector<uint16_t> uniq_slot;
   int64_t total_nq = 0;
 };
-std::string build_vel_stream(const Structure& S, const TilePlan& P, VsPlan& V);
+std::string build_vel_stream(const Structure& S, const TilePlan& P, VsPlan& V, bool bank_aware = true);
 int64_t verify_vel_stream(const Structure& S, const TilePlan& P, const VsPlan& V);
+double vel_stream_x_wavefronts(const Structure& S, const VsPlan& V);
 
 struct CoarseLevel {
   Structure Sc;
diff --git a/navier-stokes_equations_b200/csrc/twolevel.cuh b/navier-stokes_equations_b200/csrc/twolevel.cuh
--- a/navier-stokes_equations_b200/csrc/twolevel.cuh
+++ b/navier-stokes_equations_b200/csrc/twolevel.cuh
@@ -103,12 +103,13 @@
 
 template <int DIM, typename VT>
 __global__ void __launch_bounds__(256)
-k_coarse_pack(const VsTile* __restrict__ tiles, const uint32_t* __restrict__ meta, const long long* __restrict__ cnbr_ptr,
+k_coarse_pack(const VsTile* __restrict__ tiles, const uint32_t* __restrict__ meta, const uint32_t* __restrict__ qpack,
+              const long long* __restrict__ cnbr_ptr,
               const double* __restrict__ cvals, const double* __restrict__ cdinv, VT* __restrict__ out) {
   constexpr int PL = DIM * DIM;
   const VsTile hd = tiles[blockIdx.x];
   VT* o = out + (long long)PL * 4 * hd.nq_off;
-  const uint4* mt = reinterpret_cast<const uint4*>(meta) + hd.nq_off;
+  const uint2* mt = reinterpret_cast<const uint2*>(meta) + hd.nq_off;
   for (int jb = threadIdx.x; jb < 4 * hd.NQ; jb += blockDim.x) {
     const int q = jb >> 2, e = jb & 3;
     double b[DIM][DIM];
@@ -116,10 +117,10 @@
     for (int r = 0; r < DIM; ++r)
 #pragma unroll
       for (int c = 0; c < DIM; ++c) b[r][c] = 0.0;
-    const uint4 m = __ldg(mt + q);
-    if (m.z != 0xffffu && e < (int)(m.w >> 16)) {
-      const int P = hd.n0 + (int)m.z;
-      const long long blk = cnbr_ptr[P] + (int)(m.w & 0xffffu) + e;
+    const uint32_t node = __ldg(&mt[q].y) >> VS_SLOT_BITS, pk = __ldg(qpack + hd.nq_off + q);
+    if (node != VS_PAD_NODE && e < (int)(pk >> 16)) {
+      const int P = hd.n0 + (int)node;
+      const long long blk = cnbr_ptr[P] + (int)(pk & 0xffffu) + e;
 #pragma unroll
       for (int r = 0; r < DIM; ++r)
 #pragma unroll
diff --git a/navier-stokes_equations_b200/csrc/velstream.cuh b/navier-stokes_equations_b200/csrc/velstream.cuh
--- a/navier-stokes_equations_b200/csrc/velstream.cuh
+++ b/navier-stokes_equations_b200/csrc/velstream.cuh
@@ -9,12 +9,14 @@
 
 constexpr int VS_GROUPS = 2;
 constexpr int VS_THREADS = (VS_GROUPS * VS_CONSUMERS + 1) * 32;
-constexpr int VS_MAX_UNIQ = TILE_MAX_UNIQ;
+static_assert(VS_MAX_UNIQ == TILE_MAX_UNIQ && VS_MAX_UNIQ % 16 == 0, "every unique neighbour of a tile has an x slot");
+static_assert(VS_MAX_UNIQ <= (1 << VS_SLOT_BITS), "x slots fit the 10-bit fields of the quad descriptor");
+static_assert(TILE_MAX_NODES < (int)VS_PAD_NODE, "node indices fit the 7-bit field of the quad descriptor below the padding mark");
 
 template <int DIM, typename VT> struct VsLayout {
   static constexpr int PL = DIM * DIM;
   static constexpr int VAL_BYTES = PL * VS_MAX_BLOCKS * (int)sizeof(VT);
-  static constexpr int META_BYTES = VS_MAX_QUADS * 16;
+  static constexpr int META_BYTES = VS_MAX_QUADS * 8;
   static constexpr int XS_BYTES = VS_MAX_UNIQ * DIM * 8;
   static constexpr int YS_BYTES = TILE_MAX_NODES * DIM * 8;
   static constexpr int HDR_BYTES = 64;
@@ -92,7 +94,8 @@
 template <int DIM, typename VT, int MODE, bool HALO>
 __global__ void __launch_bounds__(VS_THREADS, 1)
 k_vel_stream(const VsTile* __restrict__ tiles, int n_tiles, const int* __restrict__ tile_list, const VT* __restrict__ vals,
-             const uint32_t* __restrict__ meta, const int* __restrict__ uniq_xoff, const double* __restrict__ x,
+             const uint32_t* __restrict__ meta, const int* __restrict__ uniq_xoff, const uint16_t* __restrict__ uniq_slot,
+             const double* __restrict__ x,
              double* __restrict__ y, const double* __restrict__ u, double* __restrict__ poly, PolyCoef pc, VsHalo hx) {
   using L = VsLayout<DIM, VT>;
   constexpr int PL = L::PL;
@@ -136,19 +139,20 @@
       const int NQ = __ldg(&hd->NQ), nq_off = __ldg(&hd->nq_off), u0 = __ldg(&hd->u0), nuq = __ldg(&hd->nuq);
       unsigned char* st = vs_smem + s * L::STAGE_BYTES;
       if (lane == 0) {
-        const uint32_t vb = (uint32_t)(PL * 4 * NQ * (int)sizeof(VT)), mb = (uint32_t)(NQ * 16);
+        const uint32_t vb = (uint32_t)(PL * 4 * NQ * (int)sizeof(VT)), mb = (uint32_t)(NQ * 8);
         mbar_expect_tx(full + s, vb + mb + (uint32_t)L::HDR_BYTES);
         tma_bulk_g2s(st + L::OFF_HDR, hd, L::HDR_BYTES, full + s);
         tma_bulk_g2s(st + L::OFF_VAL, vals + (long long)PL * 4 * nq_off, vb, full + s);
-        tma_bulk_g2s(st + L::OFF_META, meta + (long long)4 * nq_off, mb, full + s);
+        tma_bulk_g2s(st + L::OFF_META, meta + (long long)2 * nq_off, mb, full + s);
       }
       double* xs = reinterpret_cast<double*>(st + L::OFF_XS);
       constexpr int PER_LANE = VS_MAX_UNIQ / 32;
-      int xo[PER_LANE];
+      int xo[PER_LANE], sl[PER_LANE];
 #pragma unroll
       for (int q = 0; q < PER_LANE; ++q) {
         const int i = lane + 32 * q;
         xo[q] = i < nuq ? __ldg(uniq_xoff + u0 + i) : -1;
+        sl[q] = i < nuq ? (int)__ldg(uniq_slot + u0 + i) : 0;
       }
       if (HALO && ghosts) {
 #pragma unroll
@@ -162,13 +166,12 @@
             }
 #pragma unroll
           for (int q = q0; q < q0 + 4; ++q) {
-            const int i = lane + 32 * q;
             if (xo[q] >= hx.ghost_start) {
 #pragma unroll
-              for (int c = 0; c < DIM; ++c) xs[i * DIM + c] = gv[q - q0][c];
+              for (int c = 0; c < DIM; ++c) xs[sl[q] * DIM + c] = gv[q - q0][c];
             } else if (xo[q] >= 0) {
 #pragma unroll
-              for (int c = 0; c < DIM; ++c) cp_async_8(xs + i * DIM + c, x + xo[q] + c);
+              for (int c = 0; c < DIM; ++c) cp_async_8(xs + sl[q] * DIM + c, x + xo[q] + c);
             }
           }
         }
@@ -178,9 +181,8 @@
 #pragma unroll
         for (int q = 0; q < PER_LANE; ++q) {
           if (xo[q] >= 0) {
-            const int i = lane + 32 * q;
-#pragma unroll
-            for (int c = 0; c < DIM; ++c) cp_async_8(xs + i * DIM + c, x + xo[q] + c);
+#pragma unroll
+            for (int c = 0; c < DIM; ++c) cp_async_8(xs + sl[q] * DIM + c, x + xo[q] + c);
           }
         }
         cp_async_arrive_noinc(full + s);
@@ -198,13 +200,13 @@
     unsigned char* st = vs_smem + s * L::STAGE_BYTES;
     const VsTile* hd = reinterpret_cast<const VsTile*>(st + L::OFF_HDR);
     const VT* sv = reinterpret_cast<const VT*>(st + L::OFF_VAL);
-    const uint4* sm = reinterpret_cast<const uint4*>(st + L::OFF_META);
+    const uint2* sm = reinterpret_cast<const uint2*>(st + L::OFF_META);
     const double* xs = reinterpret_cast<const double*>(st + L::OFF_XS);
     double* ys = reinterpret_cast<double*>(st + L::OFF_YS);
     const int NQ = hd->NQ, nn = hd->nn, n0 = hd->n0, nquad = hd->nquad;
     const int b0 = hd->split[cw], b1 = hd->split[cw + 1];
-    const int na = b0 < b1 ? (int)sm[b0].z : 0;
-    const int nb_ = b0 < b1 ? (b1 < nquad ? (int)sm[b1].z : nn) : 0;
+    const int na = b0 < b1 ? (int)(sm[b0].y >> VS_SLOT_BITS) : 0;
+    const int nb_ = b0 < b1 ? (b1 < nquad ? (int)(sm[b1].y >> VS_SLOT_BITS) : nn) : 0;
     const int r0 = DIM * na, r1 = DIM * nb_;
     const long long rowg0 = (long long)DIM * n0;
     double pu[2], pp[2];
@@ -226,12 +228,12 @@
       for (int r = 0; r < DIM; ++r) acc[r] = 0.0;
       int row = 0xffff;
       if (ok) {
-        const uint4 m = sm[j];
-        row = (int)m.z;
+        const uint2 m = sm[j];
+        row = (int)(m.y >> VS_SLOT_BITS);
         double xv[4][DIM];
 #pragma unroll
         for (int e = 0; e < 4; ++e) {
-          const int loc = (int)(((e < 2 ? m.x : m.y) >> (16 * (e & 1))) & 0xffffu);
+          const int loc = (int)((e < 3 ? m.x >> (VS_SLOT_BITS * e) : m.y) & VS_SLOT_MASK);
 #pragma unroll
           for (int c = 0; c < DIM; ++c) xv[e][c] = xs[loc * DIM + c];
         }
@@ -258,8 +260,10 @@
       const int prev = __shfl_up_sync(NSB_FULL, row, 1);
       const unsigned heads = __ballot_sync(NSB_FULL, lane == 0 || prev != row);
       const int pos = lane - (31 - __clz(heads & (0xffffffffu >> (31 - lane))));
+      const int maxpos = (int)__reduce_max_sync(NSB_FULL, (unsigned)pos);
 #pragma unroll
       for (int d = 1; d < 32; d <<= 1) {
+        if (d > maxpos) break;
 #pragma unroll
         for (int r = 0; r < DIM; ++r) {
           const double o = __shfl_up_sync(NSB_FULL, acc[r], d);
@@ -332,12 +336,13 @@
 
 template <int DIM, typename VT>
 __global__ void __launch_bounds__(256)
-k_vel_pack(DevMesh M, const VsTile* __restrict__ tiles, const uint32_t* __restrict__ meta, const double* __restrict__ vals,
+k_vel_pack(DevMesh M, const VsTile* __restrict__ tiles, const uint32_t* __restrict__ meta, const uint32_t* __restrict__ qpack,
+           const double* __restrict__ vals,
            const double* __restrict__ dinv, VT* __restrict__ out) {
   constexpr int PL = DIM * DIM;
   const VsTile hd = tiles[blockIdx.x];
   VT* o = out + (long long)PL * 4 * hd.nq_off;
-  const uint4* mt = reinterpret_cast<const uint4*>(meta) + hd.nq_off;
+  const uint2* mt = reinterpret_cast<const uint2*>(meta) + hd.nq_off;
   for (int jb = threadIdx.x; jb < 4 * hd.NQ; jb += blockDim.x) {
     const int q = jb >> 2, e = jb & 3;
     double b[DIM][DIM];
@@ -345,11 +350,11 @@
     for (int r = 0; r < DIM; ++r)
 #pragma unroll
       for (int c = 0; c < DIM; ++c) b[r][c] = 0.0;
-    const uint4 m = __ldg(mt + q);
-    if (m.z != 0xffffu && e < (int)(m.w >> 16)) {
-      const int A = hd.n0 + (int)m.z;
+    const uint32_t node = __ldg(&mt[q].y) >> VS_SLOT_BITS, pk = __ldg(qpack + hd.nq_off + q);
+    if (node != VS_PAD_NODE && e < (int)(pk >> 16)) {
+      const int A = hd.n0 + (int)node;
       const NodeDesc d = load_desc(M.nd + A);
-      const int k = (int)(m.w & 0xffffu) + e, len = DIM * d.nb + d.np;
+      const int k = (int)(pk & 0xffffu) + e, len = DIM * d.nb + d.np;
       double f[DIM][DIM], di[DIM][DIM];
 #pragma unroll
       for (int r = 0; r < DIM; ++r)
```
